# Kotstantinovskiy/SonicDiffusionBayesLab

Hardware: AMD Instinct MI355X
Metric: 512x512 images/sec at 50 DDIM steps (higher is better)
Workload: dtype bf16; 1 GPU; SD-1.5 512x512 DDIM 50 steps, CFG 7.5, batch=8/GPU (BASELINE configs[1]); global_batch=8, sample_size=64, parallelism=batch-shard x1, weights=SD-1.5-shaped synthetic seed 1234

## Files before the change

include/sd_hip.h:

```cpp
#ifndef SD_HIP_H
#define SD_HIP_H

#ifdef __cplusplus
extern "C" {
#endif

typedef struct sd_unet sd_unet;

typedef struct sd_unet_config {
    int sample_size;
    int in_channels;
    int out_channels;
    int num_levels;
    int block_out_channels[8];
    int layers_per_block;
    int attn_levels[8];
    int cross_attention_dim;
    int num_heads;
    int norm_num_groups;
    float norm_eps;
    int context_len;
    int weight_dtype;
    float fp8_act_scale_norm;
    float fp8_act_scale_ff;
// ... 277 lines not shown
int sd_op_softmax_rows(void* stream, void* S, long long rows, int cols, float scale);
int sd_op_conv3x3_upsample_subpixel(void* stream, const void* X, const void* W4, const float* bias, void* Y, int B, int Hin,
                                    int Win, int Cin, int Cout);
int sd_op_conv3x3_upsample_subpixel_groupnorm(void* stream, const void* X, const void* W4, const float* bias, void* Y, int B,
                                              int Hin, int Win, int Cin, int Cout, const float* gamma, const float* beta,
                                              void* Yn, int groups, float eps, int silu);
int sd_op_groupnorm(void* stream, const void* x1, int C1, const void* x2, int C2, const float* gamma,
                    const float* beta, void* y, int B, int HW, int groups, float eps, int silu);
int sd_op_conv3x3_groupnorm(void* stream, const void* X, const void* W, const float* bias, const float* bias2,
                            const void* R, void* Y, int B, int Hin, int Win, int Cin, int Cout, const float* gamma,
                            const float* beta, void* Yn, int groups, float eps, int silu);
int sd_op_conv3x3_splitk(int M, int Cout, int Cin, int Hin, int Win, int stride, int upsample);
int sd_op_layernorm(void* stream, const void* x, const float* gamma, const float* beta, void* y, int rows, int C,
                    float eps);
int sd_op_tome_match(void* stream, const void* x, const unsigned char* choice, int B, int h, int w, int C, float* node_max,
                     int* node_idx, int* tok);
int sd_op_tome_select(void* stream, const float* node_max, const int* node_idx, int B, int num_src, int r, int* kept, int* merged,
                      int* dst_idx);
int sd_op_tome_merge(void* stream, const void* x, const int* tok, const int* kept, const int* merged, const int* dst_idx, void* out,
                     long long ldo, int B, int h, int w, int C, int r);
int sd_op_tome_unmerge(void* stream, const void* y, long long ldy, const void* residual, const int* tok, const int* kept,
                       const int* merged, const int* dst_idx, void* out, int B, int h, int w, int C, int r);
int sd_op_tgate_capture(void* stream, const void* y, const void* res, void* h2, void* cache, float* rowstats, long long rows, int C,
                        int pair);
int sd_op_tgate_apply(void* stream, const void* h1, const void* cache, void* h2, float* rowstats, long long rows, int C);
int sd_op_freeu(void* stream, const void* hidden, const void* skip, void* hidden_out, void* skip_out, int B, int H, int W,
                int C_hidden, int C_skip, float b, float s);
int sd_hypertile_check(int B, int rh, int rw, int C, int nh, int nw, long long pitch);
int sd_op_hypertile_gather(void* stream, const void* x, long long pitch, void* out, int B, int rh, int rw, int C, int nh, int nw);
int sd_op_hypertile_scatter(void* stream, const void* y, void* out, long long pitch, int B, int rh, int rw, int C, int nh, int nw);
int sd_pag_identity_check(long long rows_total, long long row0, long long rows, int C, int heads, long long ldv, int tok);
int sd_op_pag_identity(void* stream, const void* V, long long ldv, int tok, void* out, long long rows_total, long long row0,
                       long long rows, int C, int heads);
int sd_sag_mass_check(int B, int heads, int N, int D, long long ld, int head_major);
int sd_op_sag_attn_mass(void* stream, const void* Q, const void* K, long long ld, float* mass, int B, int heads, int N, int D,
                        int exp2_units);
int sd_op_sag_degrade(void* stream, const float* x, const float* m, const float* mass, int mh, int mw, int pred_type,
                      const float coef[6], float* out, int LB, int H, int W);
int sd_op_attention(void* stream, const void* Q, long long ldq, const void* K, long long ldk, const void* V,
                    long long ldv, void* O, long long ldo, int B, int heads, int Nq, int Nk, int D, float scale);
int sd_op_gemm_qkv_headmajor(void* stream, const void* X, long long ldx, const void* W, void* Q, void* KV, int M, int C,
                             int tokens, int K);
int sd_op_attention_headmajor(void* stream, const void* Q, long long ldq, const void* K, const void* V, void* O,
                              long long ldo, int B, int heads, int Nq, int Nk, int D, float scale);
int sd_op_clip_attention(void* stream, const void* qkv, void* out, int B, int L, int H, int heads);
int sd_op_vit_attention(void* stream, const void* qkv, void* out, int B, int L, int H, int heads);
int sd_op_clip_embed(void* stream, const int* ids, const void* tok, const void* pos, void* out, int rows, int L, int H,
                     int vocab);
int sd_op_activation(void* stream, void* x, long long n, int kind);
int sd_op_pool_rows(void* stream, const void* src, const int* ids, int B, int L, int H, int eos_id, void* dst);
int sd_op_vit_embed(void* stream, const void* patch_rows, const float* cls, const void* pos, void* out, int B, int Np, int H);
int sd_op_bert_attention(void* stream, const void* q, long long ldq, const void* k, const void* v, long long ldkv,
                         const int* mask, void* out, long long ldo, int B, int heads, int Lq, int Lk);
int sd_op_reward_head(void* stream, const void* hidden, long long row_stride, const float* w, const float* bias, float mean,
                      float std, int B, int H, float* rewards, float* features);
int sd_op_clip_preprocess(void* stream, const unsigned char* images, int B, int H, int W, int S, int P, unsigned char* crop,
                          void* patches);
int sd_op_conv_in(void* stream, const float* x, int Bsrc, const float* Wt, const float* bias, void* y, int B, int H,
                  int W, int Cin, int Cout);
int sd_op_conv_in_cond(void* stream, const float* x, int Bsrc, const float* cond, int Bcond, const float* Wt,
                       const float* bias, void* y, int B, int H, int W, int Cout);
int sd_op_conv_in_add(void* stream, const float* x, int Bsrc, const void* addend, int Badd, const float* Wt, const float* bias,
                      void* y, int B, int H, int W, int Cout);
int sd_op_residual_add(void* stream, void* x, const long long* dst_off, const void* r, const long long* src_off,
                       const long long* count, int nseg, float scale);
int sd_op_conv_out(void* stream, const void* x, const void* Wp, const float* bias, float* y, int B, int H, int W,
                   int Cin, int Cout);
int sd_op_time_embedding(void* stream, float t, const void* W1, const float* b1, const void* W2, const float* b2,
                         float* scratch, float* temb, int dim_in, int dim);
int sd_op_timestep_cond(void* stream, float t, const float* cond, const void* Wc, float* row, float* emb, int cond_dim,
                        int dim);

int sd_op_ln_partials(int kind, int M, int N);
int sd_op_gemm_rowstats(void* stream, const void* X, long long ldx, const void* W, const float* bias, const void* R,
                        long long ldr, void* C, long long ldc, int M, int N, int K, float* rowstats);
int sd_op_gemm_ln(void* stream, const void* X, long long ldx, const void* Wg, const float* c1, const float* c2,
                  const float* rowstats, int parts, float eps, void* C, long long ldc, int M, int N, int K, int epi);
int sd_op_gemm_plan(void* stream, const void* X, long long ldx, const void* X2, long long ldx2, int K1, const void* W,
                    const float* bias, const float* bias2, const void* R, long long ldr, void* C, long long ldc, int M, int N,
                    int K, float* rowstats, float* stats, const float* ln_rs, int ln_parts, const float* ln_c1, float ln_eps,
                    void* KV, int hm_tokens);
int sd_op_xattn_fused_rowstats(void* stream, const void* X, const void* R, void* Y, const void* At, const void* Bw,
                               const float* bias, int M, int C, int rows_per_sample, int L, float* rowstats);
int sd_op_ip_xattn(void* stream, const void* R, void* Rout, const void* A, const void* Bt, const float* gamma, const float* beta,
                   float eps, long long M, int C, int rows_per_sample, int heads, int T);
int sd_op_xattn_expand(void* stream, const void* kv, void* out, int B, int L, int C, int heads, int slots, int col_off, float scale);
int sd_op_transpose_bf16(void* stream, const void* src, void* dst, int B, int R, int Cc, int perm16);
int sd_op_retile32(void* stream, const void* src, void* dst, int B, int R, int K, int RT);
int sd_op_xattn_fold(void* stream, const void* kv, const void* wqT, const void* wo, const float* lnu, const float* ones, void* at,
                     void* bw, float* c1, float* c2, void* scratch, int UB, int L, int C, int heads, int perm);
int sd_op_ip_fold(void* stream, const void* ip_kv, const void* wqT, const void* wo, void* at, void* bt, void* scratch, int UB, int T,
                  int C, int heads, float scale);
int sd_op_xattn_fused(void* stream, const void* X, const void* R, void* Y, const void* At, const void* Bw,
                      const float* bias, int M, int C, int rows_per_sample, int L);
int sd_op_xattn_fused_ln(void* stream, const void* X, const void* R, void* Y, const void* At, const void* Bw,
                         const float* bias, int M, int C, int rows_per_sample, int L, const float* ln_rowstats, int ln_parts,
                         long long ln_rows, const float* c2, float eps, float* rowstats);
int sd_op_conv3x3_ablate(void* stream, const void* X, const void* W, void* Y, int B, int Hin, int Win, int Cin, int Cout,
                         int ablate);
int sd_op_xattn_fused_stamps(void* stream, const void* X, const void* R, void* Y, const void* At, const void* Bw,
                             const float* bias, int M, int C, int rows_per_sample, int L, unsigned long long* stamps);

int sd_op_gemm_fp8(void* stream, const void* X, long long ldx, const void* W, const float* wscale, float xscale,
                   const float* bias, const void* R, long long ldr, void* C, long long ldc, int M, int N, int K, int epi,
                   int out_fp8, float oscale);
int sd_op_conv3x3_fp8(void* stream, const void* X, const void* W, const float* wscale, float xscale, const float* bias,
                      const float* bias2, const void* R, void* Y, int B, int Hin, int Win, int Cin, int Cout, int stride,
                      int upsample);
int sd_op_groupnorm_fp8(void* stream, const void* x1, int C1, const void* x2, int C2, const float* gamma,
                        const float* beta, void* y, int B, int HW, int groups, float eps, int silu, int Cpad, float oscale);
int sd_op_layernorm_fp8(void* stream, const void* x, const float* gamma, const float* beta, void* y, int rows, int C,
                        int Cpad, float eps, float oscale);
int sd_op_quantize_fp8(void* stream, const void* x_bf16, void* y_fp8, long long rows, int C, int Cpad, float scale);
int sd_op_amax_e4m3(void* stream, const void* codes, long long nbytes, unsigned* out_code);

#ifdef __cplusplus
}
#endif
#endif
```

sonicdiffusionbayeslab_amd/_lib.py:

```python
from __future__ import annotations

import ctypes as C
import os
import re
from typing import Optional

HERE = os.path.dirname(os.path.abspath(__file__))
LIB_PATH = os.environ.get("SD_AMD_LIB", os.path.join(HERE, "lib", "libsdhip.so"))
HEADER_PATH = os.path.normpath(os.path.join(HERE, "..", "include", "sd_hip.h"))

ABLATE_LIB_PATH = os.path.join(HERE, "lib", "libsdhip_ablate.so")

_lib: Optional[C.CDLL] = None
_ablate: Optional[C.CDLL] = None


class SdUnetConfig(C.Structure):
    _fields_ = [
        ("sample_size", C.c_int), ("in_channels", C.c_int), ("out_channels", C.c_int),
        ("num_levels", C.c_int), ("block_out_channels", C.c_int * 8), ("layers_per_block", C.c_int),
        ("attn_levels", C.c_int * 8), ("cross_attention_dim", C.c_int), ("num_heads", C.c_int),
        ("norm_num_groups", C.c_int), ("norm_eps", C.c_float), ("context_len", C.c_int),
        ("weight_dtype", C.c_int), ("fp8_act_scale_norm", C.c_float), ("fp8_act_scale_ff", C.c_float),
        ("time_cond_proj_dim", C.c_int),
# ... 147 lines not shown
    "sd_op_conv_in_add": (_i, [_vp, _vp, _i, _vp, _i, _vp, _vp, _vp, _i, _i, _i, _i]),
    "sd_op_residual_add": (_i, [_vp, _vp, _vp, _vp, _vp, _vp, _i, _f]),
    "sd_op_conv_in_cond": (_i, [_vp, _vp, _i, _vp, _i, _vp, _vp, _vp, _i, _i, _i, _i]),
    "sd_op_gemm": (_i, [_vp, _vp, _ll, _vp, _ll, _i, _vp, _vp, _vp, _vp, _ll, _vp, _ll, _i, _i, _i, _i]),
    "sd_op_gemm_tile_rows": (_i, [_i, _i, _i]),
    "sd_op_gemm_splitk": (_i, [_i, _i, _i, _i]),
    "sd_op_gemm_batched": (_i, [_vp, _vp, _ll, _vp, _ll, _i, _vp, _vp, _ll, _vp, _ll, _i, _i, _i, _i, _i]),
    "sd_op_gemm_batched_softmax_ln": (_i, [_vp, _vp, _ll, _vp, _ll, _i, _vp, _ll, _i, _i, _i, _i, _vp, _i, _vp, _vp, _f]),
    "sd_op_conv3x3": (_i, [_vp, _vp, _vp, _vp, _vp, _vp, _vp, _i, _i, _i, _i, _i, _i, _i]),
    "sd_op_conv3x3_shortcut": (_i, [_vp, _vp, _vp, _vp, _vp, _i, _vp, _i, _vp, _vp, _i, _i, _i, _i, _i]),
    "sd_op_conv3x3_shortcut_groupnorm": (_i, [_vp, _vp, _vp, _vp, _vp, _i, _vp, _i, _vp, _vp, _i, _i, _i, _i, _i,
                                              _vp, _vp, _vp, _i, _f, _i]),
    "sd_op_conv3x3_down_asym": (_i, [_vp, _vp, _vp, _vp, _vp, _i, _i, _i, _i, _i]),
    "sd_op_conv3x3_ablate": (_i, [_vp, _vp, _vp, _vp, _i, _i, _i, _i, _i, _i]),
    "sd_op_conv3x3_upsample_subpixel": (_i, [_vp, _vp, _vp, _vp, _vp, _i, _i, _i, _i, _i]),
    "sd_op_conv3x3_upsample_subpixel_groupnorm": (_i, [_vp, _vp, _vp, _vp, _vp, _i, _i, _i, _i, _i, _vp, _vp, _vp, _i, _f, _i]),
    "sd_op_groupnorm": (_i, [_vp, _vp, _i, _vp, _i, _vp, _vp, _vp, _i, _i, _i, _f, _i]),
    "sd_op_conv3x3_groupnorm": (_i, [_vp, _vp, _vp, _vp, _vp, _vp, _vp, _i, _i, _i, _i, _i, _vp, _vp, _vp, _i, _f, _i]),
    "sd_op_conv3x3_splitk": (_i, [_i, _i, _i, _i, _i, _i, _i]),
    "sd_op_conv3x3_kernel": (_i, [_i, _i, _i, _i, _i, _i, _i, _i]),
    "sd_op_softmax_rows": (_i, [_vp, _vp, _ll, _i, _f]),
    "sd_op_layernorm": (_i, [_vp, _vp, _vp, _vp, _vp, _i, _i, _f]),
    "sd_op_attention": (_i, [_vp, _vp, _ll, _vp, _ll, _vp, _ll, _vp, _ll, _i, _i, _i, _i, _i, _f]),
    "sd_op_gemm_qkv_headmajor": (_i, [_vp, _vp, _ll, _vp, _vp, _vp, _i, _i, _i, _i]),
    "sd_op_attention_headmajor": (_i, [_vp, _vp, _ll, _vp, _vp, _vp, _ll, _i, _i, _i, _i, _i, _f]),
    "sd_op_clip_attention": (_i, [_vp, _vp, _vp, _i, _i, _i, _i]),
    "sd_op_conv_in": (_i, [_vp, _vp, _i, _vp, _vp, _vp, _i, _i, _i, _i, _i]),
    "sd_op_conv_out": (_i, [_vp, _vp, _vp, _vp, _vp, _i, _i, _i, _i, _i]),
    "sd_op_time_embedding": (_i, [_vp, _f, _vp, _vp, _vp, _vp, _vp, _vp, _i, _i]),
    "sd_op_timestep_cond": (_i, [_vp, _f, _vp, _vp, _vp, _vp, _i, _i]),
    "sd_op_ln_partials": (_i, [_i, _i, _i]),
    "sd_op_gemm_rowstats": (_i, [_vp, _vp, _ll, _vp, _vp, _vp, _ll, _vp, _ll, _i, _i, _i, _vp]),
    "sd_op_gemm_plan": (_i, [_vp, _vp, _ll, _vp, _ll, _i, _vp, _vp, _vp, _vp, _ll, _vp, _ll, _i, _i, _i, _vp, _vp, _vp, _i, _vp, _f,
                            _vp, _i]),
    "sd_op_gemm_ln": (_i, [_vp, _vp, _ll, _vp, _vp, _vp, _vp, _i, _f, _vp, _ll, _i, _i, _i, _i]),
    "sd_op_xattn_fused_rowstats": (_i, [_vp, _vp, _vp, _vp, _vp, _vp, _vp, _i, _i, _i, _i, _vp]),
    "sd_op_xattn_fused": (_i, [_vp, _vp, _vp, _vp, _vp, _vp, _vp, _i, _i, _i, _i]),
    "sd_op_xattn_fused_ln": (_i, [_vp, _vp, _vp, _vp, _vp, _vp, _vp, _i, _i, _i, _i, _vp, _i, _ll, _vp, _f, _vp]),
    "sd_op_xattn_fused_stamps": (_i, [_vp, _vp, _vp, _vp, _vp, _vp, _vp, _i, _i, _i, _i, _vp]),
    "sd_op_gemm_fp8": (_i, [_vp, _vp, _ll, _vp, _vp, _f, _vp, _vp, _ll, _vp, _ll, _i, _i, _i, _i, _i, _f]),
    "sd_op_conv3x3_fp8": (_i, [_vp, _vp, _vp, _vp, _f, _vp, _vp, _vp, _vp, _i, _i, _i, _i, _i, _i, _i]),
    "sd_op_groupnorm_fp8": (_i, [_vp, _vp, _i, _vp, _i, _vp, _vp, _vp, _i, _i, _i, _f, _i, _i, _f]),
    "sd_op_layernorm_fp8": (_i, [_vp, _vp, _vp, _vp, _vp, _i, _i, _i, _f, _f]),
    "sd_op_quantize_fp8": (_i, [_vp, _vp, _vp, _ll, _i, _i, _f]),
    "sd_op_amax_e4m3": (_i, [_vp, _vp, _ll, _vp]),
    "sd_unet_set_tome": (_i, [_vp, C.c_double, _i]),
    "sd_unet_tome_block_count_hw": (_i, [_vp, _i, _i]),
    "sd_unet_tome_block_info_hw": (_i, [_vp, _i, _i, _i, C.POINTER(_i), C.POINTER(_i), C.POINTER(_i), C.POINTER(_ll)]),
    "sd_unet_set_tome_choice_hw": (_i, [_vp, _vp, _vp, _ll, _i, _i]),
    "sd_unet_tome_matching_hw": (_i, [_vp, _vp, _i, _i, _i, _vp, _vp, _vp, _vp, _vp, C.POINTER(_i), C.POINTER(_i)]),
    "sd_op_tome_match": (_i, [_vp, _vp, _vp, _i, _i, _i, _i, _vp, _vp, _vp]),
    "sd_op_tome_select": (_i, [_vp, _vp, _vp, _i, _i, _i, _vp, _vp, _vp]),
    "sd_op_tome_merge": (_i, [_vp, _vp, _vp, _vp, _vp, _vp, _vp, _ll, _i, _i, _i, _i, _i]),
    "sd_op_tome_unmerge": (_i, [_vp, _vp, _ll, _vp, _vp, _vp, _vp, _vp, _vp, _i, _i, _i, _i, _i]),
    "sd_unet_set_freeu": (_i, [_vp, _f, _f, _f, _f]),
    "sd_unet_disable_freeu": (_i, [_vp]),
    "sd_unet_plan_count": (_i, [_vp]),
    "sd_op_freeu": (_i, [_vp, _vp, _vp, _vp, _vp, _i, _i, _i, _i, _i, _f, _f]),
    "sd_unet_tgate_bytes_hw": (_ll, [_vp, _i, _i, _i]),
    "sd_unet_tgate_block_info_hw": (_i, [_vp, _i, _i, _i, _i, C.POINTER(_ll), C.POINTER(_ll), C.POINTER(_i)]),
    "sd_unet_set_tgate_hw": (_i, [_vp, _i, _vp, _ll, _i, _i, _i]),
    "sd_op_tgate_capture": (_i, [_vp, _vp, _vp, _vp, _vp, _vp, _ll, _i, _i]),
    "sd_op_tgate_apply": (_i, [_vp, _vp, _vp, _vp, _vp, _ll, _i]),
    "sd_unet_set_hypertile": (_i, [_vp, _i, _i]),
    "sd_unet_hypertile_block_count_hw": (_i, [_vp, _i, _i]),
    "sd_unet_hypertile_block_info_hw": (_i, [_vp, _i, _i, _i, C.POINTER(_i), C.POINTER(_i), C.POINTER(_i), C.POINTER(_i)]),
    "sd_hypertile_check": (_i, [_i, _i, _i, _i, _i, _i, _ll]),
    "sd_op_hypertile_gather": (_i, [_vp, _vp, _ll, _vp, _i, _i, _i, _i, _i, _i]),
    "sd_op_hypertile_scatter": (_i, [_vp, _vp, _vp, _ll, _i, _i, _i, _i, _i, _i]),
    "sd_unet_set_pag": (_i, [_vp, _ll]),
    "sd_unet_pag_block_count": (_i, [_vp]),
    "sd_pag_identity_check": (_i, [_ll, _ll, _ll, _i, _i, _ll, _i]),
    "sd_op_pag_identity": (_i, [_vp, _vp, _ll, _i, _vp, _ll, _ll, _ll, _i, _i]),
    "sd_sched_step_pag": (_i, [_vp, _vp, _i, _f, _f] + [_vp] * 8 + [C.POINTER(_f), _ll, _vp, _ll, _vp, _vp, _vp, _f, _f, _ll]),
    "sd_sched_step_pc_pag": (_i, [_vp, _vp, _i, _f, _f] + [_vp] * 9 + [C.POINTER(_f), _ll, _vp, _ll, _vp, _vp, _vp, _f, _f, _ll]),
    "sd_cfg_rescale_factors_pag": (_i, [_vp, _vp, _i, _ll, _f, _f, _f, _vp]),
    "sd_unet_set_sag": (_i, [_vp, _i]),
    "sd_unet_set_sag_buffer": (_i, [_vp, _vp, _ll]),
    "sd_sag_mass_check": (_i, [_i, _i, _i, _i, _ll, _i]),
    "sd_op_sag_attn_mass": (_i, [_vp, _vp, _vp, _ll, _vp, _i, _i, _i, _i, _i]),
    "sd_op_sag_degrade": (_i, [_vp, _vp, _vp, _vp, _i, _i, _i, C.POINTER(_f), _vp, _i, _i, _i]),
    "sd_sched_step_sag": (_i, [_vp, _vp, _i, _f, _f] + [_vp] * 8 + [C.POINTER(_f), _ll, _vp, _ll, _vp, _vp, _vp, _f, _f, _ll]),
    "sd_sched_step_pc_sag": (_i, [_vp, _vp, _i, _f, _f] + [_vp] * 9 + [C.POINTER(_f), _ll, _vp, _ll, _vp, _vp, _vp, _f, _f, _ll]),
}


def _open(path: str, missing_message: str) -> C.CDLL:
    if not os.path.exists(path):
        raise SdHipError(missing_message)
    lib = C.CDLL(path)
    for name, (res, args) in _SIGS.items():
        fn = getattr(lib, name)
        fn.restype = res
        fn.argtypes = args
    return lib


def load() -> C.CDLL:
    global _lib
    if _lib is None:
        _lib = _open(LIB_PATH, f"{LIB_PATH} is missing: build it with `python -m sonicdiffusionbayeslab_amd.build` "
                               "(or __graft_entry__.build()).  There is no CPU/PyTorch fallback for the hot path.")
    return _lib


def load_ablate() -> C.CDLL:
    global _ablate
    if _ablate is None:
        _ablate = _open(ABLATE_LIB_PATH, f"{ABLATE_LIB_PATH} is missing: build it with `python -m sonicdiffusionbayeslab_amd.build`")
    return _ablate


def check(rc: int, what: str = "libsdhip call", lib: Optional[C.CDLL] = None) -> None:
    if rc != 0:
        msg = (lib or load()).sd_last_error()
        raise SdHipError(f"{what} failed (rc={rc}): {msg.decode() if msg else '?'}")


def ptr(t) -> Optional[int]:
    return None if t is None else t.data_ptr()


def current_stream() -> int:
    import torch
    return torch.cuda.current_stream().cuda_stream
```

sonicdiffusionbayeslab_amd/build.py:

```python
from __future__ import annotations

import os
import shutil
import subprocess
import sys
import tempfile
from concurrent.futures import ThreadPoolExecutor

HERE = os.path.dirname(os.path.abspath(__file__))
CSRC = os.path.join(HERE, "csrc")
LIB_DIR = os.path.join(HERE, "lib")
LIB_PATH = os.path.join(LIB_DIR, "libsdhip.so")
ABLATE_LIB_PATH = os.path.join(LIB_DIR, "libsdhip_ablate.so")
ABLATE_SOURCES = ("gemm_conv.hip", "conv_halo.hip")
SOURCES = ["gemm_conv.hip", "gemm_lean.hip", "conv_halo.hip", "conv64.hip", "norm.hip", "attention.hip", "xattn.hip", "ip_xattn.hip", "small.hip", "sched.hip", "clip.hip", "vit.hip", "bert.hip", "inception.hip", "unet.hip", "pack.hip", "plan.hip", "taesd.hip", "tome.hip", "freeu.hip", "tgate.hip", "hypertile.hip", "pag.hip", "sag.hip", "ops.hip"]
HEADERS = ["common.h", "kernels.h", "model.h",os.path.join("..", "..", "include", "sd_hip.h")]
FLAGS = ["--offload-arch=gfx950", "-O3", "-fPIC", "-std=c++17", "-Wall", "-Wno-unused-function"]
NO_PACKED_FP32 = ["-Xclang", "-target-feature", "-Xclang", "-packed-fp32-ops"]
EXTRA_FLAGS = {"attention.hip": ["-mllvm", "-amdgpu-mfma-vgpr-form", "-ffinite-math-only", *NO_PACKED_FP32],
               "xattn.hip": ["-mllvm", "-amdgpu-mfma-vgpr-form", "-fno-slp-vectorize"],
               "ip_xattn.hip": NO_PACKED_FP32,
               "small.hip": NO_PACKED_FP32, "sched.hip": NO_PACKED_FP32, "clip.hip": NO_PACKED_FP32, "vit.hip": NO_PACKED_FP32, "bert.hip": NO_PACKED_FP32, "norm.hip": NO_PACKED_FP32,
               "inception.hip": NO_PACKED_FP32,
               "conv64.hip": NO_PACKED_FP32,
               "tome.hip": NO_PACKED_FP32,
               "freeu.hip": NO_PACKED_FP32,
               "tgate.hip": NO_PACKED_FP32,
               "hypertile.hip": NO_PACKED_FP32,
               "pag.hip": NO_PACKED_FP32,
               "sag.hip": NO_PACKED_FP32,
               "gemm_conv.hip": ["-fno-slp-vectorize"], "gemm_lean.hip": ["-fno-slp-vectorize"]}
_HOST_NOISE = "is not a recognized feature for this target (ignoring feature)"


def _newer(a: str, b: str) -> bool:
    return (not os.path.exists(b)) or os.path.getmtime(a) > os.path.getmtime(b)


def asm_path(src: str, ablate: bool = False) -> str:
    return os.path.join(LIB_DIR, src.replace(".hip", ".ablate.s" if ablate else ".s"))


def lint_asm(path: str, unit: str, verbose: bool = True) -> None:
    from . import asm_lint
    bad = asm_lint.lint_file(path, unit, verbose=verbose)
    if bad:
        raise RuntimeError(f"{unit}: the assembly hipcc produced violates {len(bad)} rule(s) of asm_lint.py (first: {bad[0]}); "
                           "see the VIOLATION lines above and sonicdiffusionbayeslab_amd/asm_lint.py for what each rule guards")


def compile_unit(hipcc: str, src: str, obj: str, flags, verbose: bool = True) -> None:
    s = os.path.join(CSRC, src)
    tmp = tempfile.mkdtemp(prefix="sdhip_", dir=LIB_DIR)
    try:
        cmd = [hipcc, *flags, "-save-temps", "-c", s, "-o", os.path.join(tmp, "unit.o")]
        if verbose:
            print(" ".join(cmd), flush=True)
        r = subprocess.run(cmd, capture_output=True, text=True, cwd=tmp)
        err = "\n".join(l for l in r.stderr.splitlines() if _HOST_NOISE not in l and "argument unused during compilation" not in l)
        if r.returncode != 0:
            raise RuntimeError(f"hipcc failed:\n{' '.join(cmd)}\n{r.stdout}\n{err}")
        if verbose and err.strip():
            print(err, file=sys.stderr)
        dev = [f for f in os.listdir(tmp) if f.endswith("-gfx950.s")]
        if len(dev) != 1:
            raise RuntimeError(f"{src}: expected one device assembly file from -save-temps, found {dev}")
        asm = obj[:-2] + ".s"
        shutil.move(os.path.join(tmp, dev[0]), asm)
        try:
            lint_asm(asm, src.split(".")[0], verbose=verbose)
        except Exception:
            os.replace(asm, asm + ".rejected")
            raise
        shutil.move(os.path.join(tmp, "unit.o"), obj)
    finally:
        shutil.rmtree(tmp, ignore_errors=True)


def build_library(force: bool = False, verbose: bool = True) -> str:
    hipcc = os.environ.get("HIPCC", "/opt/rocm/bin/hipcc")
    if not os.path.exists(hipcc):
        hipcc = "hipcc"
    os.makedirs(LIB_DIR, exist_ok=True)
    hdrs = [os.path.normpath(os.path.join(CSRC, h)) for h in HEADERS]
    me = [os.path.abspath(__file__), os.path.join(HERE, "asm_lint.py")]
    objs, jobs = [], []
    for src in SOURCES:
        s = os.path.join(CSRC, src)
        o = os.path.join(LIB_DIR, src.replace(".hip", ".o"))
        objs.append(o)
        if force or _newer(s, o) or any(_newer(h, o) for h in hdrs + me) or not os.path.exists(o[:-2] + ".s"):
            jobs.append((src, o, [*FLAGS, *EXTRA_FLAGS.get(src, [])]))

    aobjs, ajobs = [], []
    for src in SOURCES:
        s = os.path.join(CSRC, src)
        if src in ABLATE_SOURCES:
            o = os.path.join(LIB_DIR, src.replace(".hip", ".ablate.o"))
            if force or _newer(s, o) or any(_newer(h, o) for h in hdrs + me) or not os.path.exists(o[:-2] + ".s"):
                ajobs.append((src, o, [*FLAGS, "-DSD_ABLATE", *EXTRA_FLAGS.get(src, [])]))
        else:
            o = os.path.join(LIB_DIR, src.replace(".hip", ".o"))
        aobjs.append(o)

    def run(cmd):
        if verbose:
            print(" ".join(cmd), flush=True)
        r = subprocess.run(cmd, capture_output=True, text=True)
        if r.returncode != 0:
            raise RuntimeError(f"hipcc failed:\n{' '.join(cmd)}\n{r.stdout}\n{r.stderr}")

    with ThreadPoolExecutor(max_workers=4) as ex:
        list(ex.map(lambda j: compile_unit(hipcc, j[0], j[1], j[2], verbose), jobs + ajobs))
    if force or jobs or not os.path.exists(LIB_PATH):
# ... 9 lines not shown
```

sonicdiffusionbayeslab_amd/csrc/common.h:

```cpp
#pragma once
#include <hip/hip_runtime.h>
#include <stdint.h>

typedef unsigned short bf16_t;

typedef __attribute__((ext_vector_type(8))) short bf16x8;
typedef __attribute__((ext_vector_type(4))) short bf16x4;
typedef __attribute__((ext_vector_type(4))) float f32x4;
typedef __attribute__((ext_vector_type(16))) float f32x16;
typedef __attribute__((ext_vector_type(2))) __bf16 bf16x2_t;
typedef __attribute__((ext_vector_type(2))) float f32x2_t;
typedef __attribute__((ext_vector_type(4))) unsigned u32x4;
typedef __attribute__((ext_vector_type(2))) unsigned u32x2;

typedef __attribute__((ext_vector_type(8))) int i32x8;
typedef __attribute__((ext_vector_type(8))) unsigned u32x8;
__device__ __forceinline__ i32x8 cat_u32x4(u32x4 lo, u32x4 hi) {
    const u32x8 r = __builtin_shufflevector(lo, hi, 0, 1, 2, 3, 4, 5, 6, 7);
    return __builtin_bit_cast(i32x8, r);
}

#define LDS_PTR(p) ((__attribute__((address_space(3))) void*)(p))
#define GLB_PTR(p) ((const __attribute__((address_space(1))) void*)(p))

// ... 55 lines not shown

template <int SHR>
__device__ __forceinline__ float row_shr_add(float v) {
    const int sh = __builtin_amdgcn_update_dpp(0, __builtin_bit_cast(int, v), 0x110 + SHR, 0xf, 0xf, true);
    return v + __builtin_bit_cast(float, sh);
}
template <int TN, int TM>
__device__ __forceinline__ void tile_channel_stats(const f32x4 (&acc)[TN][TM], float* __restrict__ stats, long block64, int C,
                                                   int n_base, int N, int m_base, int M, int lane, int b0 = 0, int nb = TM) {
    const int lrow = lane & 15, lq = lane >> 4;
#pragma unroll
    for (int a = 0; a < TN; ++a) {
        float sv[4] = {0.f, 0.f, 0.f, 0.f}, qv[4] = {0.f, 0.f, 0.f, 0.f};
#pragma unroll
        for (int b = 0; b < TM; ++b) {
            if (b < b0 || b >= b0 + nb) continue;
            const bool live = m_base + b * 16 + lrow < M;
            const unsigned p0 = pack2bf(acc[a][b][0], acc[a][b][1]), p1 = pack2bf(acc[a][b][2], acc[a][b][3]);
            const float v[4] = {bflo(p0), bfhi(p0), bflo(p1), bfhi(p1)};
#pragma unroll
            for (int j = 0; j < 4; ++j) {
                const float x = live ? v[j] : 0.f;
                sv[j] += x;
                qv[j] = __builtin_fmaf(x, x, qv[j]);
            }
        }
#pragma unroll
        for (int j = 0; j < 4; ++j) {
            sv[j] = row_shr_add<8>(row_shr_add<4>(row_shr_add<2>(row_shr_add<1>(sv[j]))));
            qv[j] = row_shr_add<8>(row_shr_add<4>(row_shr_add<2>(row_shr_add<1>(qv[j]))));
        }
        const int n = n_base + a * 16 + lq * 4;
        if (lrow == 15 && n < N) {
            float* o = stats + (block64 * C + n) * 2;
            *(f32x4*)o = f32x4{sv[0], qv[0], sv[1], qv[1]};
            *(f32x4*)(o + 4) = f32x4{sv[2], qv[2], sv[3], qv[3]};
        }
    }
}

template <int TN, int TM>
__device__ __forceinline__ void tile_row_stats(const f32x4 (&acc)[TN][TM], float* __restrict__ part, int n_base, int N,
                                               int m_base, int M, int lane) {
    const int lrow = lane & 15, lq = lane >> 4;
#pragma unroll
    for (int b = 0; b < TM; ++b) {
        float s = 0.f, q = 0.f;
#pragma unroll
        for (int a = 0; a < TN; ++a) {
            const bool live = n_base + a * 16 + lq * 4 < N;
            const unsigned p0 = pack2bf(acc[a][b][0], acc[a][b][1]), p1 = pack2bf(acc[a][b][2], acc[a][b][3]);
            const float v[4] = {bflo(p0), bfhi(p0), bflo(p1), bfhi(p1)};
#pragma unroll
            for (int j = 0; j < 4; ++j) {
                const float x = live ? v[j] : 0.f;
                s += x;
                q = __builtin_fmaf(x, x, q);
            }
        }
        s += __shfl_xor(s, 16); q += __shfl_xor(q, 16);
        s += __shfl_xor(s, 32); q += __shfl_xor(q, 32);
        const int m = m_base + b * 16 + lrow;
        if (lq == 0 && m < M) *(f32x2_t*)(part + (long)m * 2) = f32x2_t{s, q};
    }
}

__device__ __forceinline__ f32x2_t ln_mean_rstd(float s, float q, float inv_k, float eps) {
    const float mean = s * inv_k;
    const float var = __builtin_fmaf(q, inv_k, -(mean * mean));
    return f32x2_t{mean, __builtin_amdgcn_rsqf(fmaxf(var, 0.f) + eps)};
}
__device__ __forceinline__ f32x4 ln_fold(f32x4 acc, f32x4 c1, float mean, float rstd, f32x4 c2) {
#ifdef SD_DIAG_LN_PACKED
    const f32x4 nm = {-mean, -mean, -mean, -mean}, rs = {rstd, rstd, rstd, rstd};
    return __builtin_elementwise_fma(__builtin_elementwise_fma(c1, nm, acc), rs, c2);
#else
    f32x4 r;
#pragma unroll
    for (int j = 0; j < 4; ++j) r[j] = __builtin_fmaf(__builtin_fmaf(c1[j], -mean, acc[j]), rstd, c2[j]);
    return r;
#endif
}

__device__ __forceinline__ float wave_sum(float v) {
#pragma unroll
    for (int o = 32; o > 0; o >>= 1) v += __shfl_xor(v, o);
    return v;
}

extern "C" const char* sd_last_error(void);
void sd_set_error(const char* fmt, ...);
#define SD_CHECK_HIP(expr)                                                              \
    do {                                                                                \
        hipError_t _e = (expr);                                                         \
        if (_e != hipSuccess) {                                                         \
            sd_set_error("%s failed: %s (%s:%d)", #expr, hipGetErrorString(_e), __FILE__, __LINE__); \
            return -2;                                                                  \
        }                                                                               \
    } while (0)
#define SD_REQUIRE(cond, ...)          \
    do {                               \
        if (!(cond)) {                 \
            sd_set_error(__VA_ARGS__); \
            return -1;                 \
        }                              \
    } while (0)
```

sonicdiffusionbayeslab_amd/csrc/kernels.h:

```cpp
#pragma once
#include <vector>

#include "common.h"

struct GemmArgs {
    const bf16_t* X = nullptr;
    long ldx = 0;
    const bf16_t* X2 = nullptr;
    long ldx2 = 0;
    int K1 = 0;
    const bf16_t* W = nullptr;
    long ldw = 0;
    const float* bias = nullptr;
    const float* bias2 = nullptr;
    const bf16_t* R = nullptr;
    long ldr = 0;
    bf16_t* C = nullptr;
    long ldc = 0;
    int M = 0, N = 0, K = 0;
    int Hin = 0, Win = 0, Cin = 0, Hout = 0, Wout = 0, stride = 1, up = 0;
    int asym = 0;
    int splitk = 1;
    float* slab = nullptr;
    int defer_reduce = 0;
    const void* zero_page = nullptr;
    long w_batch_stride = 0;
    int rows_per_batch = 0;
    int sm_valid = 0;
    int tiles_m = 0, tiles_n = 0;
    int tune = 0;
    float* stats = nullptr;
    float* rowstats = nullptr;
    bf16_t* KV = nullptr;
    int hm_C = 0, hm_tok = 0;
    int subpix = 0;
    const float* ln_rs = nullptr;
    const float* ln_c1 = nullptr;
    int ln_np = 0;
    float ln_eps = 1e-5f;
    int ln_per_sample = 0;
    int dt = 0;
    const float* wscale = nullptr;
    float xscale_inv = 1.0f;
    int out_fp8 = 0;
    float oscale = 1.0f;
    const bf16_t* Xs1 = nullptr;
    const bf16_t* Xs2 = nullptr;
    const bf16_t* Wsc = nullptr;
    long ldwsc = 0;
    int Csc1 = 0, Csc2 = 0;
};

int sd_gemm_tile_rows(int M, int N, int K = 0);
int sd_gemm_splitk(int M, int N, int K, int rows = 0);
int sd_launch_gemm(const GemmArgs& a, int epi , hipStream_t stream);
int sd_launch_conv3x3(const GemmArgs& a, hipStream_t stream);
bool sd_gemm_lean_applicable(const GemmArgs& a, int epi);
int sd_launch_gemm_lean(const GemmArgs& a, int epi, int rows, hipStream_t stream);
void sd_launch_splitk_reduce(const GemmArgs& a, hipStream_t stream);
bool sd_conv_halo_applicable(const GemmArgs& a);
int sd_conv_halo_mode(const GemmArgs& a);
int sd_conv3x3_splitk(int M, int N, int Cin, int Hin, int Win, int stride, int up, int dt = 0);
bool sd_conv_halo_subpix_applicable(const GemmArgs& a);
int sd_launch_conv3x3_halo(const GemmArgs& a, hipStream_t stream);
bool sd_conv_halo_shortcut_applicable(const GemmArgs& a);

constexpr int SD_CONV64_PACKED_BYTES = 9 * 2 * 4 * 1024;
struct Conv64Args {
    const bf16_t* X = nullptr;
    const bf16_t* Wp = nullptr;
    const float* bias = nullptr;
    const bf16_t* R = nullptr;
    bf16_t* Y = nullptr;
    int B = 0, Hin = 0, Win = 0;
    int mode = 0;
    int relu = 0;
    int Hout = 0, Wout = 0, tiles_y = 0, tiles_x = 0, ntiles = 0;
    unsigned xbytes = 0;
};
int sd_conv64_out_size(int in, int mode);
void sd_conv64_pack(const float* w_oihw , bf16_t* out);
int sd_launch_conv64(const Conv64Args& a, hipStream_t stream);
int sd_launch_taesd_entry(const float* x, const float* Wt, const float* bias, bf16_t* y, int B, int H, int W, int Cin, int decoder,
                          hipStream_t stream);
int sd_launch_taesd_exit(const bf16_t* x, const bf16_t* Wp, const float* bias, float* y, int B, int H, int W, int Cout, int out_mode,
                         hipStream_t stream);

struct GroupNormArgs {
    const bf16_t* x1 = nullptr; int C1 = 0;
    const bf16_t* x2 = nullptr; int C2 = 0;
    const float* gamma = nullptr; const float* beta = nullptr;
    bf16_t* y = nullptr;
    int out_fp8 = 0, Cpad = 0;
    float oscale = 1.0f;
    const float* stats1 = nullptr; const float* stats2 = nullptr;
    const float* slab = nullptr; int splitk = 0;
    const float* sbias = nullptr; const float* sbias2 = nullptr;
    const bf16_t* sR = nullptr; long sldr = 0;
    bf16_t* x1w = nullptr;
    float* partial = nullptr;
    int B = 0, HW = 0, groups = 32, nsplit = 0;
    float eps = 1e-5f;
    int silu = 0;
};
int sd_groupnorm_nsplit(int B, int HW);
bool sd_groupnorm_uses_small(int B, int HW, int C1, int C2, int groups);
bool sd_groupnorm_slab_ok(int B, int HW, int C1, int C2, int groups);
size_t sd_groupnorm_scratch_bytes(int B, int HW, int groups);
int sd_launch_groupnorm(const GroupNormArgs& a, hipStream_t stream);

int sd_launch_softmax_rows(bf16_t* s, long rows, int cols, float scale, hipStream_t stream);
int sd_launch_softmax_rows_long(bf16_t* s, long rows, int cols, float scale, hipStream_t stream);
int sd_launch_pqconv(const float* x, const float* W, const float* bias, float* y, int B, int HW, float in_scale,
                     hipStream_t stream);

int sd_launch_layernorm(const bf16_t* x, const float* gamma, const float* beta, bf16_t* y, int rows, int C,
                        float eps, hipStream_t stream);
int sd_launch_layernorm_fp8(const bf16_t* x, const float* gamma, const float* beta, void* y, int rows, int C, int Cpad,
                            float eps, float oscale, hipStream_t stream);
int sd_launch_amax_e4m3(const void* y, long nbytes, unsigned* out, hipStream_t stream);
int sd_launch_quantize_fp8(const bf16_t* x, void* y, long rows, int C, int Cpad, float scale, hipStream_t stream);

struct AttnArgs {
    const bf16_t* Q = nullptr; long ldq = 0;
    const bf16_t* K = nullptr; long ldk = 0;
    const bf16_t* V = nullptr; long ldv = 0;
    bf16_t* O = nullptr; long ldo = 0;
    int B = 0, heads = 0, Nq = 0, Nk = 0, D = 0;
    float scale = 0.f;
    const void* consts = nullptr;
    int kv_head_major = 0;
    int q_prescaled = 0;
    int xcd_order = 1;
};
int sd_launch_attention(const AttnArgs& a, hipStream_t stream);

int sd_launch_gemv(const float* x, const bf16_t* W, const float* b, float* y, int N, int K, int silu_in,
                   hipStream_t stream);
int sd_launch_timestep_sinusoid(float t, float* out, int dim, hipStream_t stream);
int sd_launch_timestep_sinusoid_row(float t, const float* row, float* out, int dim, hipStream_t stream);
int sd_launch_f32_to_bf16(const float* src, bf16_t* dst, long n, hipStream_t stream);
int sd_launch_transpose_bf16(const bf16_t* src, bf16_t* dst, int B, int R, int Cc, hipStream_t stream, int perm16 = 0);

int sd_launch_retile32(const bf16_t* src, bf16_t* dst, int B, int R, int K, int RT, hipStream_t stream);
int sd_launch_replicate(const void* src, void* dst, long bytes, int rep, hipStream_t stream);

int sd_tome_check(int h, int w, int C, const char* who);
int sd_launch_tome_partition(const unsigned char* choice, int h, int w, int* tok, hipStream_t stream);
int sd_launch_tome_match(const bf16_t* x, const unsigned char* choice, int B, int h, int w, int C, float* node_max, int* node_idx,
                         int* tok, float* inv, hipStream_t stream);
int sd_launch_tome_select(const float* node_max, const int* node_idx, int B, int num_src, int r, int* kept, int* merged, int* dst_idx,
                          hipStream_t stream);
int sd_launch_tome_merge(const bf16_t* x, const int* tok, const int* kept, const int* merged, const int* dst_idx, bf16_t* out,
                         long ldo, int B, int h, int w, int C, int r, hipStream_t stream);
int sd_launch_tome_unmerge(const bf16_t* y, long ldy, const bf16_t* residual, const int* tok, const int* kept, const int* merged,
                           const int* dst_idx, bf16_t* out, int B, int h, int w, int C, int r, hipStream_t stream);

int sd_freeu_check(int B, int H, int W, int C_hidden, int C_skip, const char* who);
int sd_launch_freeu(const bf16_t* hidden, const bf16_t* skip, bf16_t* hidden_out, bf16_t* skip_out, int B, int H, int W, int C_hidden,
                    int C_skip, float b, float s, hipStream_t stream);

constexpr int SD_TGATE_PARTS = 2;
int sd_tgate_check(long rows, int C, const char* who);
int sd_launch_tgate_capture(const bf16_t* y, const bf16_t* res, bf16_t* h2, bf16_t* cache, float* rowstats, long rows, int C, int pair,
                            hipStream_t stream);
int sd_launch_tgate_apply(const bf16_t* h1, const bf16_t* cache, bf16_t* h2, float* rowstats, long rows, int C, hipStream_t stream);

int sd_hypertile_shape_ok(int B, int rh, int rw, int C, int nh, int nw, long pitch, const char* who);
int sd_launch_hypertile_gather(const bf16_t* x, long pitch, bf16_t* out, int B, int rh, int rw, int C, int nh, int nw, hipStream_t stream);
int sd_launch_hypertile_scatter(const bf16_t* y, bf16_t* out, long pitch, int B, int rh, int rw, int C, int nh, int nw, hipStream_t stream);

int sd_pag_identity_shape_ok(long rows_total, long row0, long rows, int C, int heads, long ldv, int tok, const char* who);
int sd_launch_pag_identity(const bf16_t* V, long ldv, int tok, bf16_t* out, long rows_total, long row0, long rows, int C, int heads,
                           hipStream_t stream);

int sd_sag_mass_shape_ok(int B, int heads, int N, int D, long ld, int head_major, const char* who);
int sd_launch_sag_attn_mass(const bf16_t* Q, const bf16_t* K, long ld, float* mass, int B, int heads, int N, int D, int exp2_units,
                            hipStream_t stream);
int sd_sag_degrade_shape_ok(int LB, int H, int W, int mh, int mw, int pred, const char* who);
int sd_launch_sag_degrade(const float* x, const float* m, const float* mass, int mh, int mw, int pred, const float coef[6], float* out,
                          int LB, int H, int W, hipStream_t stream);

struct XattnArgs {
    const bf16_t* X = nullptr;
    const bf16_t* R = nullptr;
    bf16_t* Y = nullptr;
    const bf16_t* At = nullptr;
    const bf16_t* Bw = nullptr;
    const float* bias = nullptr;
    int M = 0, C = 0, rows_per_sample = 0, L = 0;
    float* rowstats = nullptr;
    const float* ln_rs = nullptr; int ln_np = 0; long ln_rows = 0;
// ... 97 lines not shown
```

sonicdiffusionbayeslab_amd/csrc/model.h:

```cpp
#pragma once
#include "../../include/sd_hip.h"
#include "common.h"
#include "kernels.h"

#include <stdlib.h>
#include <string.h>
#include <sys/mman.h>

#include <algorithm>
#include <map>
#include <new>
#include <set>
#include <string>
#include <tuple>
#include <unordered_map>
#include <vector>

namespace sdhip {

constexpr size_t NOFF = (size_t)-1;
constexpr int T_LATENTS = -2, T_EPS = -3;
constexpr int MAX_CONTROL_RES = SD_MAX_RES_SEGMENTS;

struct ParamSpec {
    std::string name;
    std::vector<long long> shape;
    std::vector<float> data;
    bool loaded = false;
    long long numel() const {
        long long n = 1;
        for (auto s : shape) n *= s;
        return n;
    }
};

struct Wrap {
    int type;
    int block_i, layer_i;
};

enum OpKind { OP_SINUSOID, OP_GEMV, OP_CONV_IN, OP_GN, OP_CONV3, OP_GEMM, OP_LN, OP_ATTN, OP_CONV_OUT, OP_SOFTMAX, OP_PQCONV,
              OP_CLIP_EMBED, OP_CLIP_ATTN, OP_QGELU, OP_TO_F32, OP_XATTN, OP_REPLICATE,
              OP_VIT_PREP, OP_VIT_EMBED, OP_VIT_ATTN, OP_POOL, OP_CONV_IN_IMG, OP_ENC_OUT, OP_IP_XATTN, OP_RES_ADD,
              OP_BERT_ATTN, OP_REWARD_HEAD,
              OP_TOME_MATCH, OP_TOME_SELECT, OP_TOME_MERGE, OP_TOME_UNMERGE,
              OP_FREEU,
              OP_TGATE_CAPTURE, OP_TGATE_APPLY, OP_TGATE_ZERO,
              OP_HT_GATHER, OP_HT_SCATTER,
              OP_PAG_IDENTITY,
              OP_SAG_MASS };

constexpr int TGATE_OFF = 0, TGATE_CAPTURE = 1, TGATE_REUSE = 2;

constexpr int REP_TEXT_POOLED = 2;

struct Op {
    int kind = 0;
    int x1 = -1, x2 = -1, r = -1, out = -1, aux = -1, b2t = -1;
    size_t w = NOFF, b = NOFF, g = NOFF, be = NOFF;
    long b2idx = 0;
    int M = 0, N = 0, K = 0, K1 = 0, epi = 0;
    int B = 0, Hin = 0, Win = 0, Cin = 0, Hout = 0, Wout = 0, stride = 1, up = 0;
    int C1 = 0, C2 = 0, HW = 0, silu = 0, nsplit = 0;
    float eps = 0.f;
    int heads = 0, D = 0, Nq = 0, Nk = 0;
    long ldq = 0, ldk = 0, ldv = 0, ldo = 0, qoff = 0, koff = 0, voff = 0;
    int silu_in = 0, splitk = 1;
    int pool_by_ids = 0;
    int key_mask = 0;
    int defer = 0, slab_t = -1, slab_k = 0, slab_r = -1, slab_b2t = -1;
    size_t slab_b = NOFF;
    long slab_b2idx = 0;
    int wt = -1;
    size_t wx = NOFF;
    long xoff = 0, woff_el = 0, coff = 0, ldx_o = 0, ldw_o = 0, ldc_o = 0;
    float scale = 0.f;
    long wbs = 0;
    int rpb = 0, sm_valid = 0;
    int dt = 0, out_fp8 = 0, Cpad = 0, Kalg = 0;
    int sname = -1;
    int stats = -1, s1 = -1, s2 = -1;
    int subpix = 0;
    int asym = 0;
    int hm = 0;
    int qps = 0;
    int rs = -1, lnrs = -1, lnnp = 0;
    size_t c1 = NOFF;
    size_t wsc = NOFF;
    float xs = 1.f, os = 1.f;
    int scx1 = -1, scx2 = -1, scc1 = 0, scc2 = 0;
    size_t scw = NOFF;
    int nres = 0;
    int res_t[MAX_CONTROL_RES];
    int nwrap = 0;
    Wrap wraps[3];
};

struct HostBlob {
    unsigned char* p = nullptr;
    size_t n = 0, cap = 0;
    unsigned char* data() { return p; }
    const unsigned char* data() const { return p; }
    size_t size() const { return n; }
    bool empty() const { return n == 0; }
    bool reserve(size_t bytes) {
        if (bytes <= cap) return true;
        void* q = mmap(nullptr, bytes, PROT_READ | PROT_WRITE, MAP_PRIVATE | MAP_ANONYMOUS | MAP_POPULATE, -1, 0);
        if (q == MAP_FAILED) return false;
        (void)madvise(q, bytes, MADV_HUGEPAGE);
        if (p) { memcpy(q, p, n); munmap(p, cap); }
        p = (unsigned char*)q; cap = bytes;
        return true;
    }
    void resize(size_t bytes) {
        if (bytes > cap && !reserve(std::max(bytes, cap * 2))) throw std::bad_alloc();
        n = bytes;
    }
    void release() { if (p) munmap(p, cap); p = nullptr; n = cap = 0; }
    ~HostBlob() { release(); }
    HostBlob() = default;
    HostBlob(const HostBlob&) = delete;
    HostBlob& operator=(const HostBlob&) = delete;
};

struct Tn {
    size_t bytes = 0;
    int def = -1, last = -1;
    bool persistent = false;
    bool ctx = false;
    bool ctx_ip = false;
    size_t off = NOFF;
};

struct Plan {
    int UB = 0, branch = -1;
    int rep = 1;
    int lh = 0, lw = 0;
    int ip = 0;
    struct IpFold { int at, bt, C; size_t wqT, wo, wkv; int heads; };
    std::vector<IpFold> ip_fold;
    int ip_e = -1, ip_proj = -1, ip_tok = -1, ip_kv = -1;
    int cn = 0;
    std::vector<size_t> cn_off;
    std::vector<long> cn_count;
    struct TomeBlock { int tok, kept, merged, dst_idx, B, h, w, r; long choice_off; };
    std::vector<TomeBlock> tome;
    long tome_choice_bytes = 0;
    struct HtBlock { int rh, rw, nh, nw; };
    std::vector<HtBlock> hypertile;
    int pag_lb = 0, pag_blocks = 0;
    int sag = 0;
    int freeu = 0;
    int tgate = 0, tg_pair = 1, tg_batch = 0;
    std::vector<size_t> tg_off;
    std::vector<long> tg_rows;
    std::vector<int> tg_ch;
    int tg_blocks = 0;
    std::vector<Tn> tensors;
    std::vector<Op> ops;
    std::vector<char> skipped;
    std::vector<int> ctx_kv;
    std::vector<size_t> ctx_w;
    std::vector<int> ctx_c;
    int ctx_bf16 = -1;
    struct Fold { int kv, at, bw, C, heads; size_t wqT, wo; bool perm; int c2 = -1; size_t lnu = NOFF; int c1 = -1; size_t ones = NOFF; };
    std::vector<Fold> ctx_fold;
    int ctx_fold_scratch = -1;
    std::map<std::string, int> taps;
    size_t total_bytes = 0;
    ClipPrepGeom geom;
    std::vector<int> prep_tab;
    const int* dtab = nullptr;
};

}

// ... 124 lines not shown
```

sonicdiffusionbayeslab_amd/csrc/norm.hip:

```cpp
#include "common.h"
#include "kernels.h"

#include <stdlib.h>

#include <algorithm>
#include <type_traits>

namespace {

struct GnGeom {
    int nchunks, rows_par, threads, cpg, C;
};

__host__ __device__ inline GnGeom gn_geom(int C, int groups) {
    GnGeom g;
    g.C = C;
    g.nchunks = C / 8;
    g.rows_par = g.nchunks >= 256 ? 1 : 256 / g.nchunks;
    const int act = g.rows_par * g.nchunks;
    g.threads = (act + 63) / 64 * 64;
    g.cpg = C / groups;
    return g;
}

// ... 58 lines not shown
            else                        { s += v.z; q += v.w; }
        }
        float* out = a.partial + (((long)b * a.nsplit + split) * a.groups + tid) * 2;
        out[0] = s;
        out[1] = q;
    }
}

__global__ __launch_bounds__(256) void gn_finalize_kernel(const GroupNormArgs a) {
    const int lane = threadIdx.x & 63;
    const int idx = blockIdx.x * 4 + (threadIdx.x >> 6);
    if (idx >= a.B * a.groups) return;
    const int b = idx / a.groups, gi = idx - b * a.groups;
    float s = 0.f, q = 0.f;
    for (int i = lane; i < a.nsplit; i += 64) {
        const float* pp = a.partial + (((long)b * a.nsplit + i) * a.groups + gi) * 2;
        s += pp[0];
        q += pp[1];
    }
    s = wave_sum(s);
    q = wave_sum(q);
    if (lane == 0) {
        const float cnt = (float)a.HW * (float)((a.C1 + a.C2) / a.groups);
        const float mean = s / cnt;
        const float var = fmaxf(q / cnt - mean * mean, 0.f);
        float* st = a.partial + (long)a.B * a.nsplit * a.groups * 2 + (long)idx * 2;
        st[0] = mean;
        st[1] = rsqrtf(var + a.eps);
    }
}

__global__ __launch_bounds__(256) void gn_finalize_stats_kernel(const GroupNormArgs a) {
    __shared__ float red[8];
    const int tid = threadIdx.x, lane = tid & 63, wave = tid >> 6;
    const int idx = blockIdx.x;
    const int b = idx / a.groups, gi = idx - b * a.groups;
    const int C = a.C1 + a.C2, cpg = C / a.groups, nblk = a.HW >> 6;
    const int total = nblk * cpg;
    float s = 0.f, q = 0.f;
    for (int i = tid; i < total; i += 256) {
        const int blk = i / cpg, c = gi * cpg + (i - blk * cpg);
        const long gb = (long)b * nblk + blk;
        const f32x2_t v = *(const f32x2_t*)(c < a.C1 ? a.stats1 + (gb * a.C1 + c) * 2 : a.stats2 + (gb * a.C2 + (c - a.C1)) * 2);
        s += v[0];
        q += v[1];
    }
    s = wave_sum(s);
    q = wave_sum(q);
    if (lane == 0) { red[wave * 2] = s; red[wave * 2 + 1] = q; }
    __syncthreads();
    if (tid == 0) {
        s = (red[0] + red[2]) + (red[4] + red[6]);
        q = (red[1] + red[3]) + (red[5] + red[7]);
        const float cnt = (float)a.HW * (float)cpg;
        const float mean = s / cnt;
        const float var = fmaxf(q / cnt - mean * mean, 0.f);
        float* st = a.partial + (long)a.B * a.nsplit * a.groups * 2 + (long)idx * 2;
        st[0] = mean;
        st[1] = rsqrtf(var + a.eps);
    }
}

template <bool SILU, bool FP8>
__global__ void gn_apply_kernel(const GroupNormArgs a) {
    const GnGeom g = gn_geom(a.C1 + a.C2, a.groups);
    const int tid = threadIdx.x;
    const int split = blockIdx.x, b = blockIdx.y;
    const bool active = tid < g.rows_par * g.nchunks;
    if (!active) return;
    const int prow = tid / g.nchunks, ch = tid - prow * g.nchunks;
    const int c0 = ch * 8;
    const float* st = a.partial + (long)a.B * a.nsplit * a.groups * 2 + (long)b * a.groups * 2;
    const int g0 = c0 / g.cpg, g1 = (c0 + 7) / g.cpg;
    const int nb = min(8, (g0 + 1) * g.cpg - c0);
    const float m0 = st[g0 * 2], r0 = st[g0 * 2 + 1], m1 = st[g1 * 2], r1 = st[g1 * 2 + 1];
    float sc[8], sf[8];
    {
        const f32x4 ga = *(const f32x4*)(a.gamma + c0), gb = *(const f32x4*)(a.gamma + c0 + 4);
        const f32x4 ba = *(const f32x4*)(a.beta + c0), bb = *(const f32x4*)(a.beta + c0 + 4);
#pragma unroll
        for (int j = 0; j < 8; ++j) {
            const float gm = j < 4 ? ga[j & 3] : gb[j & 3], bt = j < 4 ? ba[j & 3] : bb[j & 3];
            const float mean = j < nb ? m0 : m1, rstd = j < nb ? r0 : r1;
            sc[j] = rstd * gm;
            sf[j] = bt - mean * sc[j];
        }
    }
    const int per = (a.HW + a.nsplit - 1) / a.nsplit;
    const int pbeg = split * per, pend = min(a.HW, pbeg + per);
    auto apply = [&](const u32x4 v, long pix) {
        float f[8] = {bflo(v[0]), bfhi(v[0]), bflo(v[1]), bfhi(v[1]),
                      bflo(v[2]), bfhi(v[2]), bflo(v[3]), bfhi(v[3])};
#pragma unroll
        for (int j = 0; j < 8; ++j) {
            f[j] = f[j] * sc[j] + sf[j];
            if (SILU) f[j] = silu_f(f[j]);
        }
        if (FP8) {
            char* yr = (char*)a.y + pix * a.Cpad;
            const u32x2 o = {pack4fp8(f[0] * a.oscale, f[1] * a.oscale, f[2] * a.oscale, f[3] * a.oscale),
                             pack4fp8(f[4] * a.oscale, f[5] * a.oscale, f[6] * a.oscale, f[7] * a.oscale)};
            *(u32x2*)(yr + c0) = o;
            if (ch == g.nchunks - 1)
                for (int k = g.C; k < a.Cpad; k += 16) *(u32x4*)(yr + k) = u32x4{0u, 0u, 0u, 0u};
            return;
        }
        u32x4 o = {pack2bf(f[0], f[1]), pack2bf(f[2], f[3]), pack2bf(f[4], f[5]), pack2bf(f[6], f[7])};
        *(u32x4*)(a.y + pix * g.C + c0) = o;
    };
    const long base = (long)b * a.HW;
    const int rp = g.rows_par;
    int p = pbeg + prow;
    for (; p + 3 * rp < pend; p += 4 * rp) {
        const u32x4 v0 = *(const u32x4*)gn_src(a, base + p, c0);
        const u32x4 v1 = *(const u32x4*)gn_src(a, base + p + rp, c0);
        const u32x4 v2 = *(const u32x4*)gn_src(a, base + p + 2 * rp, c0);
        const u32x4 v3 = *(const u32x4*)gn_src(a, base + p + 3 * rp, c0);
        apply(v0, base + p); apply(v1, base + p + rp); apply(v2, base + p + 2 * rp); apply(v3, base + p + 3 * rp);
    }
    for (; p < pend; p += rp) apply(*(const u32x4*)gn_src(a, base + p, c0), base + p);
}

__device__ __forceinline__ float2 gn_unit_sums(const u32x2 v) {
    const float f0 = bflo(v[0]), f1 = bfhi(v[0]), f2 = bflo(v[1]), f3 = bfhi(v[1]);
    return make_float2((f0 + f1) + (f2 + f3), (f0 * f0 + f1 * f1) + (f2 * f2 + f3 * f3));
}
__device__ __forceinline__ void gn_mean_rstd(float ts, float tq, float cnt, float eps, float& mean, float& rstd) {
    mean = ts / cnt;
    rstd = rsqrtf(fmaxf(tq / cnt - mean * mean, 0.f) + eps);
}
template <bool SILU, bool FP8>
__device__ __forceinline__ void gn_unit_store(const GroupNormArgs& a, const u32x2 v, float mean, float rstd, long pix, int c, int C) {
    const f32x4 gm = *(const f32x4*)(a.gamma + c), bt = *(const f32x4*)(a.beta + c);
    float f[4] = {bflo(v[0]), bfhi(v[0]), bflo(v[1]), bfhi(v[1])};
#pragma unroll
    for (int jj = 0; jj < 4; ++jj) {
        f[jj] = (f[jj] - mean) * rstd * gm[jj] + bt[jj];
        if (SILU) f[jj] = silu_f(f[jj]);
    }
    if (FP8) {
        *(unsigned*)((char*)a.y + pix * a.Cpad + c) = pack4fp8(f[0] * a.oscale, f[1] * a.oscale, f[2] * a.oscale, f[3] * a.oscale);
    } else {
        u32x2 o = {pack2bf(f[0], f[1]), pack2bf(f[2], f[3])};
        *(u32x2*)(a.y + pix * C + c) = o;
    }
}

template <bool SILU, bool FP8, int MAXU>
__global__ __launch_bounds__(256) void gn_small_kernel(const GroupNormArgs a) {
    __shared__ float2 red[4];
    const int C = a.C1 + a.C2, cpg = C / a.groups, upp = cpg >> 2;
    const int grp = blockIdx.x, b = blockIdx.y;
    const int tid = threadIdx.x, lane = tid & 63, wave = tid >> 6;
    const int total = a.HW * upp;
    const long base = (long)b * a.HW;
    auto src = [&](int p, int c) -> const bf16_t* {
        return c < a.C1 ? a.x1 + (base + p) * a.C1 + c : a.x2 + (base + p) * a.C2 + (c - a.C1);
    };
    const int p0 = tid / upp, k0 = tid - p0 * upp, dp = 256 / upp, dk = 256 - dp * upp;
    u32x2 vals[MAXU];
    int pj[MAXU], kj[MAXU];
    {
        int p = p0, k = k0;
#pragma unroll
        for (int j = 0; j < MAXU; ++j) {
            const bool live = tid + 256 * j < total;
            pj[j] = live ? p : 0; kj[j] = live ? k : 0;
            vals[j] = *(const u32x2*)src(pj[j], grp * cpg + kj[j] * 4);
            p += dp; k += dk;
            if (k >= upp) { k -= upp; ++p; }
        }
    }
    float s = 0.f, q = 0.f;
#pragma unroll
    for (int j = 0; j < MAXU; ++j) {
        const bool live = tid + 256 * j < total;
        const float2 u = gn_unit_sums(vals[j]);
        s += live ? u.x : 0.f;
// ... 353 lines not shown

int sd_launch_softmax_rows_long(bf16_t* s, long rows, int cols, float scale, hipStream_t stream) {
    SD_REQUIRE(s && rows > 0 && rows <= 0x7fffffffL, "softmax_rows_long: %ld rows", rows);
    SD_REQUIRE(cols % 8 == 0 && cols > 0, "softmax_rows_long: cols=%d must be a positive multiple of 8", cols);
    hipLaunchKernelGGL(softmax_rows_long_kernel, dim3((unsigned)rows), dim3(256), 0, stream, s, cols, scale);
    SD_CHECK_HIP(hipGetLastError());
    return 0;
}

int sd_launch_softmax_rows(bf16_t* s, long rows, int cols, float scale, hipStream_t stream) {
    SD_REQUIRE(s && rows > 0, "softmax_rows: empty");
    SD_REQUIRE(cols % 8 == 0 && cols > 0 && cols <= 4096, "softmax_rows: cols=%d must be a multiple of 8 and <= 4096", cols);
    hipLaunchKernelGGL(softmax_rows_kernel, dim3((unsigned)((rows + 3) / 4)), dim3(256), 0, stream, s, rows, cols, scale);
    SD_CHECK_HIP(hipGetLastError());
    return 0;
}

size_t sd_groupnorm_scratch_bytes(int B, int HW, int groups) {
    return ((size_t)B * sd_groupnorm_nsplit(B, HW) * groups * 2 + (size_t)B * groups * 2) * sizeof(float);
}

int sd_groupnorm_nsplit(int B, int HW) {
    int n = (2048 + B - 1) / B;
    if (n > HW / 8) n = HW / 8;
    if (n < 1) n = 1;
    if (n > 256) n = 256;
    return n;
}

bool sd_groupnorm_uses_small(int B, int HW, int C1, int C2, int groups) {
    static const bool no_small = getenv("SD_GN_NO_SMALL") != nullptr;
    const int C = C1 + C2;
    return !no_small && HW <= 256 && (long)HW * (C / groups) <= 10240 && (C / groups) % 4 == 0 && C1 % 4 == 0 && B <= 65535;
}

bool sd_groupnorm_slab_ok(int B, int HW, int C1, int C2, int groups) {
    if (!sd_groupnorm_uses_small(B, HW, C1, C2, groups)) return false;
    const int cpg = (C1 + C2) / groups, G = cpg >= 80 ? 1 : 80 / cpg;
    return cpg >= 20 && cpg <= 80 && groups % G == 0 && C2 % 4 == 0 && (long)B * HW * C1 < (1L << 29);
}

int sd_launch_groupnorm(const GroupNormArgs& a, hipStream_t stream) {
    const int C = a.C1 + a.C2;
    SD_REQUIRE(a.x1 && a.y && a.gamma && a.beta && a.partial, "groupnorm: null operand");
    SD_REQUIRE(!a.out_fp8 || (a.Cpad >= C && a.Cpad % 128 == 0 && C % 16 == 0 && a.oscale > 0.f),
               "groupnorm fp8 out: Cpad=%d must be a multiple of 128 >= C=%d (C a multiple of 16)", a.Cpad, C);
    SD_REQUIRE(a.C1 % 8 == 0 && a.C2 % 8 == 0 && (a.C2 == 0 || a.x2), "groupnorm: C1=%d C2=%d must be multiples of 8", a.C1, a.C2);
    SD_REQUIRE(a.groups > 0 && a.groups <= 64 && C % a.groups == 0 && (C / a.groups >= 8 || C / a.groups == 4),
               "groupnorm: C=%d groups=%d needs C/groups >= 8 (or == 4)", C, a.groups);
    SD_REQUIRE(a.nsplit >= 1 && a.nsplit <= a.HW && a.B > 0 && a.HW > 0, "groupnorm: bad split %d for HW=%d", a.nsplit, a.HW);
    const GnGeom g = gn_geom(C, a.groups);
    SD_REQUIRE(g.threads <= 1024, "groupnorm: C=%d too wide", C);
    if (a.slab) {
        const int cpg = C / a.groups, G = cpg >= 80 ? 1 : 80 / cpg, ncol = G * (cpg / 4);
        SD_REQUIRE(a.splitk > 1 && a.splitk <= 64 && a.x1w && !a.out_fp8 && (!a.sR || a.sldr >= a.C1) && (a.C2 == 0 || a.x2),
                   "groupnorm with a deferred split-K reduce: splitk=%d, bf16 output, x1w and a residual stride >= C1", a.splitk);
        SD_REQUIRE(sd_groupnorm_slab_ok(a.B, a.HW, a.C1, a.C2, a.groups), "groupnorm with a deferred split-K reduce: HW=%d C=%d+%d "
                   "is not a shape gn_slab_kernel takes", a.HW, a.C1, a.C2);
        const dim3 grid(a.groups / G, a.B), blk((32 * ncol + 63) / 64 * 64);
        const size_t smem = ((size_t)G * a.HW * (cpg / 4) + 4 * G) * sizeof(float2);
        auto go = [&](auto kern) { hipLaunchKernelGGL(kern, grid, blk, smem, stream, a); };
        auto pick = [&](auto mi, auto un) {
            constexpr int MI = decltype(mi)::value, UN = decltype(un)::value;
            if (a.silu) go(gn_slab_kernel<true, MI, UN>); else go(gn_slab_kernel<false, MI, UN>);
        };
        using std::integral_constant;
        const int iters = (a.HW + 31) / 32, k = a.splitk;
        if (iters <= 2) {
            if (k % 8 == 0) pick(integral_constant<int, 2>{}, integral_constant<int, 8>{});
            else if (k % 4 == 0) pick(integral_constant<int, 2>{}, integral_constant<int, 4>{});
            else if (k % 2 == 0) pick(integral_constant<int, 2>{}, integral_constant<int, 2>{});
            else pick(integral_constant<int, 2>{}, integral_constant<int, 1>{});
        } else if (iters <= 4) {
            if (k % 4 == 0) pick(integral_constant<int, 4>{}, integral_constant<int, 4>{});
            else if (k % 2 == 0) pick(integral_constant<int, 4>{}, integral_constant<int, 2>{});
            else pick(integral_constant<int, 4>{}, integral_constant<int, 1>{});
        } else {
            if (k % 2 == 0) pick(integral_constant<int, 8>{}, integral_constant<int, 2>{});
            else pick(integral_constant<int, 8>{}, integral_constant<int, 1>{});
        }
        SD_CHECK_HIP(hipGetLastError());
        return 0;
    }
    if (sd_groupnorm_uses_small(a.B, a.HW, a.C1, a.C2, a.groups)) {
        const int units = (a.HW * (C / a.groups / 4) + 255) / 256;
        const dim3 grid(a.groups, a.B);
        auto go = [&](auto kern) { hipLaunchKernelGGL(kern, grid, dim3(256), 0, stream, a); };
        auto pick = [&](auto mu) {
            constexpr int MU = decltype(mu)::value;
            if (a.out_fp8) { if (a.silu) go(gn_small_kernel<true, true, MU>); else go(gn_small_kernel<false, true, MU>); }
            else { if (a.silu) go(gn_small_kernel<true, false, MU>); else go(gn_small_kernel<false, false, MU>); }
        };
        if (units <= 3) pick(std::integral_constant<int, 3>{});
        else if (units <= 5) pick(std::integral_constant<int, 5>{});
        else pick(std::integral_constant<int, 10>{});
        SD_CHECK_HIP(hipGetLastError());
        return 0;
    }
    dim3 grid(a.nsplit, a.B);
    if (a.stats1 != nullptr) {
        SD_REQUIRE(a.HW % 64 == 0 && (a.C2 == 0 || a.stats2 != nullptr), "groupnorm: producer statistics need HW %% 64 == 0 and both sources");
        hipLaunchKernelGGL(gn_finalize_stats_kernel, dim3(a.B * a.groups), dim3(256), 0, stream, a);
    } else {
        hipLaunchKernelGGL(gn_stats_kernel, grid, dim3(g.threads), (g.threads + g.nchunks) * sizeof(float4), stream, a);
        hipLaunchKernelGGL(gn_finalize_kernel, dim3((a.B * a.groups + 3) / 4), dim3(256), 0, stream, a);
    }
    if (a.out_fp8) {
        if (a.silu) hipLaunchKernelGGL((gn_apply_kernel<true, true>), grid, dim3(g.threads), 0, stream, a);
        else hipLaunchKernelGGL((gn_apply_kernel<false, true>), grid, dim3(g.threads), 0, stream, a);
    } else {
        if (a.silu) hipLaunchKernelGGL((gn_apply_kernel<true, false>), grid, dim3(g.threads), 0, stream, a);
        else hipLaunchKernelGGL((gn_apply_kernel<false, false>), grid, dim3(g.threads), 0, stream, a);
    }
    SD_CHECK_HIP(hipGetLastError());
    return 0;
}

static int launch_layernorm(const bf16_t* x, const float* gamma, const float* beta, bf16_t* y, int rows, int C, float eps,
                            bool fp8, int Cpad, float oscale, hipStream_t stream) {
    SD_REQUIRE(x && y && gamma && beta, "layernorm: null operand");
    SD_REQUIRE(C % 8 == 0 && C > 0 && C <= 1536, "layernorm: C=%d must be a multiple of 8 and <= 1536", C);
    SD_REQUIRE(rows > 0, "layernorm: no rows");
    SD_REQUIRE(!fp8 || (Cpad == (C + 127) / 128 * 128 && C % 16 == 0 && oscale > 0.f && Cpad - C <= 64 * 16),
               "layernorm fp8 out: Cpad=%d must be C=%d rounded up to 128 (C a multiple of 16)", Cpad, C);
    auto grouped = [&](auto kern, int lpr) {
        const int rows_per_block = 4 * (64 / lpr);
        hipLaunchKernelGGL(kern, dim3((rows + rows_per_block - 1) / rows_per_block), dim3(256), 0, stream, x, gamma, beta, y,
                           rows, eps, oscale);
    };
    if (fp8) {
        if (C == 320) grouped(layernorm_grouped_kernel<8, true>, 8);
        else if (C == 640) grouped(layernorm_grouped_kernel<16, true>, 16);
        else if (C == 1280) grouped(layernorm_grouped_kernel<32, true>, 32);
        else
            hipLaunchKernelGGL(layernorm_kernel<true>, dim3((rows + 3) / 4), dim3(256), 0, stream, x, gamma, beta, y, rows, C,
                               eps, Cpad, oscale);
    } else {
        if (C == 320) grouped(layernorm_grouped_kernel<8, false>, 8);
        else if (C == 640) grouped(layernorm_grouped_kernel<16, false>, 16);
        else if (C == 1280) grouped(layernorm_grouped_kernel<32, false>, 32);
        else
            hipLaunchKernelGGL(layernorm_kernel<false>, dim3((rows + 3) / 4), dim3(256), 0, stream, x, gamma, beta, y, rows, C,
                               eps, C, 1.0f);
    }
    SD_CHECK_HIP(hipGetLastError());
    return 0;
}

int sd_launch_layernorm(const bf16_t* x, const float* gamma, const float* beta, bf16_t* y, int rows, int C,
                        float eps, hipStream_t stream) {
    return launch_layernorm(x, gamma, beta, y, rows, C, eps, false, C, 1.0f, stream);
}

int sd_launch_layernorm_fp8(const bf16_t* x, const float* gamma, const float* beta, void* y, int rows, int C, int Cpad,
                            float eps, float oscale, hipStream_t stream) {
    return launch_layernorm(x, gamma, beta, (bf16_t*)y, rows, C, eps, true, Cpad, oscale, stream);
}

int sd_launch_quantize_fp8(const bf16_t* x, void* y, long rows, int C, int Cpad, float scale, hipStream_t stream) {
    SD_REQUIRE(x && y && rows > 0, "quantize_fp8: null operand");
    SD_REQUIRE(C % 8 == 0 && Cpad % 8 == 0 && Cpad >= C && scale > 0.f, "quantize_fp8: C=%d Cpad=%d", C, Cpad);
    const long n = rows * (Cpad >> 3);
    hipLaunchKernelGGL(quantize_fp8_kernel, dim3((unsigned)((n + 255) / 256)), dim3(256), 0, stream, x, (char*)y, rows, C,
                       Cpad, scale);
    SD_CHECK_HIP(hipGetLastError());
    return 0;
}

int sd_launch_amax_e4m3(const void* y, long nbytes, unsigned* out, hipStream_t stream) {
    SD_REQUIRE(y && out && nbytes > 0 && nbytes % 16 == 0 && ((uintptr_t)y & 15) == 0, "amax_e4m3: %ld bytes, 16-byte granules", nbytes);
    const long n16 = nbytes / 16;
    const unsigned grid = (unsigned)std::min<long>((n16 + 255) / 256, 2048);
    hipLaunchKernelGGL(amax_e4m3_kernel, dim3(grid), dim3(256), 0, stream, (const u32x4*)y, n16, out);
    SD_CHECK_HIP(hipGetLastError());
    return 0;
}
```

sonicdiffusionbayeslab_amd/csrc/ops.hip:

```cpp
#include "model.h"

#include <stdlib.h>

namespace sdhip {

static void* g_scratch = nullptr;
static size_t g_scratch_bytes = 0;
void* op_scratch(size_t bytes) {
    if (bytes > g_scratch_bytes) {
        (void)hipDeviceSynchronize();
        if (g_scratch) (void)hipFree(g_scratch);
        g_scratch = nullptr;
        g_scratch_bytes = 0;
        if (hipMalloc(&g_scratch, bytes) != hipSuccess) return nullptr;
        g_scratch_bytes = bytes;
    }
    return g_scratch;
}

}

using namespace sdhip;

static void conv3x3_args(GemmArgs& a, const void* X, const void* W, const float* bias, const float* bias2, const void* R, void* Y,
// ... 538 lines not shown
    if (splitk_slab(a, "sd_op_gemm_fp8")) return -1;
    return sd_launch_gemm(a, epi, (hipStream_t)stream);
}

extern "C" int sd_op_conv3x3_fp8(void* stream, const void* X, const void* W, const float* wscale, float xscale,
                                 const float* bias, const float* bias2, const void* R, void* Y, int B, int Hin, int Win,
                                 int Cin, int Cout, int stride, int upsample) {
    if (ensure_zero_page()) return -2;
    SD_REQUIRE(stride == 1 || stride == 2, "conv3x3 fp8: stride %d", stride);
    SD_REQUIRE(xscale > 0.f, "conv3x3 fp8: activation scale");
    GemmArgs a;
    conv3x3_args(a, X, W, bias, bias2, R, Y, B, Hin, Win, Cin, Cout, stride, upsample ? 1 : 0);
    a.dt = 1; a.wscale = wscale; a.xscale_inv = 1.0f / xscale;
    a.splitk = sd_conv3x3_splitk(a.M, a.N, Cin, Hin, Win, stride, a.up, 1);
    if (splitk_slab(a, "sd_op_conv3x3_fp8")) return -1;
    return sd_launch_conv3x3(a, (hipStream_t)stream);
}

extern "C" int sd_op_groupnorm_fp8(void* stream, const void* x1, int C1, const void* x2, int C2, const float* gamma,
                                   const float* beta, void* y, int B, int HW, int groups, float eps, int silu, int Cpad,
                                   float oscale) {
    GroupNormArgs a;
    a.x1 = (const bf16_t*)x1; a.C1 = C1; a.x2 = (const bf16_t*)x2; a.C2 = C2; a.gamma = gamma; a.beta = beta;
    a.y = (bf16_t*)y; a.B = B; a.HW = HW; a.groups = groups; a.eps = eps; a.silu = silu;
    a.out_fp8 = 1; a.Cpad = Cpad; a.oscale = oscale;
    a.nsplit = sd_groupnorm_nsplit(B, HW);
    a.partial = (float*)op_scratch(sd_groupnorm_scratch_bytes(B, HW, groups));
    SD_REQUIRE(a.partial, "sd_op_groupnorm_fp8: cannot allocate scratch");
    return sd_launch_groupnorm(a, (hipStream_t)stream);
}

extern "C" int sd_op_layernorm_fp8(void* stream, const void* x, const float* gamma, const float* beta, void* y, int rows,
                                   int C, int Cpad, float eps, float oscale) {
    return sd_launch_layernorm_fp8((const bf16_t*)x, gamma, beta, y, rows, C, Cpad, eps, oscale, (hipStream_t)stream);
}

extern "C" int sd_op_quantize_fp8(void* stream, const void* x_bf16, void* y_fp8, long long rows, int C, int Cpad, float scale) {
    return sd_launch_quantize_fp8((const bf16_t*)x_bf16, y_fp8, (long)rows, C, Cpad, scale, (hipStream_t)stream);
}

extern "C" int sd_op_amax_e4m3(void* stream, const void* codes, long long nbytes, unsigned* out_code) {
    SD_REQUIRE(out_code, "sd_op_amax_e4m3: null output");
    SD_CHECK_HIP(hipMemsetAsync(out_code, 0, sizeof(unsigned), (hipStream_t)stream));
    return sd_launch_amax_e4m3(codes, (long)nbytes, out_code, (hipStream_t)stream);
}

extern "C" int sd_op_ln_partials(int kind, int M, int N) { return kind == 0 ? (N + 159) / 160 * 2 : 2 * sd_xattn_slices(M, N); }
extern "C" int sd_op_gemm_rowstats(void* stream, const void* X, long long ldx, const void* W, const float* bias, const void* R,
                                   long long ldr, void* C, long long ldc, int M, int N, int K, float* rowstats) {
    if (ensure_zero_page()) return -2;
    SD_REQUIRE(rowstats, "sd_op_gemm_rowstats: null partials buffer");
    GemmArgs a;
    a.X = (const bf16_t*)X; a.ldx = ldx; a.K1 = K; a.W = (const bf16_t*)W; a.bias = bias; a.R = (const bf16_t*)R; a.ldr = ldr;
    a.C = (bf16_t*)C; a.ldc = ldc; a.M = M; a.N = N; a.K = K; a.zero_page = zero_page(); a.splitk = 1; a.rowstats = rowstats;
    return sd_launch_gemm(a, 0, (hipStream_t)stream);
}
extern "C" int sd_op_gemm_plan(void* stream, const void* X, long long ldx, const void* X2, long long ldx2, int K1, const void* W,
                               const float* bias, const float* bias2, const void* R, long long ldr, void* C, long long ldc,
                               int M, int N, int K, float* rowstats, float* stats, const float* ln_rs, int ln_parts,
                               const float* ln_c1, float ln_eps, void* KV, int hm_tokens) {
    if (ensure_zero_page()) return -2;
    GemmArgs a;
    a.X = (const bf16_t*)X; a.ldx = ldx; a.X2 = (const bf16_t*)X2; a.ldx2 = ldx2; a.K1 = K1; a.W = (const bf16_t*)W;
    a.bias = bias; a.bias2 = bias2; a.R = (const bf16_t*)R; a.ldr = ldr; a.C = (bf16_t*)C; a.ldc = ldc; a.M = M; a.N = N; a.K = K;
    a.zero_page = zero_page(); a.splitk = 1; a.rowstats = rowstats; a.stats = stats;
    a.ln_rs = ln_rs; a.ln_np = ln_parts; a.ln_c1 = ln_c1; a.ln_eps = ln_eps;
    if (hm_tokens > 0) {
        SD_REQUIRE(N % 3 == 0 && KV, "sd_op_gemm_plan: head-major K / V needs N = 3 C and a KV buffer");
        a.KV = (bf16_t*)KV; a.hm_C = N / 3; a.hm_tok = hm_tokens;
    }
    return sd_launch_gemm(a, 0, (hipStream_t)stream);
}
extern "C" int sd_op_gemm_ln(void* stream, const void* X, long long ldx, const void* Wg, const float* c1, const float* c2,
                             const float* rowstats, int parts, float eps, void* C, long long ldc, int M, int N, int K, int epi) {
    if (ensure_zero_page()) return -2;
    SD_REQUIRE(epi == 0 || epi == 1, "sd_op_gemm_ln: epi %d (0 = plain, 1 = GEGLU)", epi);
    GemmArgs a;
    a.X = (const bf16_t*)X; a.ldx = ldx; a.K1 = K; a.W = (const bf16_t*)Wg; a.bias = c2;
    a.C = (bf16_t*)C; a.ldc = ldc; a.M = M; a.N = N; a.K = K; a.zero_page = zero_page(); a.splitk = 1;
    a.ln_rs = rowstats; a.ln_np = parts; a.ln_c1 = c1; a.ln_eps = eps;
    return sd_launch_gemm(a, epi, (hipStream_t)stream);
}

extern "C" int sd_op_xattn_fused_rowstats(void* stream, const void* X, const void* R, void* Y, const void* At, const void* Bw,
                                          const float* bias, int M, int C, int rows_per_sample, int L, float* rowstats) {
    SD_REQUIRE(sd_xattn_fused_applicable(rows_per_sample, C, 8, L), "sd_op_xattn_fused_rowstats: shape not supported");
    XattnArgs a = xattn_args(X, R, Y, At, Bw, bias, M, C, rows_per_sample, L);
    a.rowstats = rowstats;
    return sd_launch_xattn_fused(a, (hipStream_t)stream);
}

extern "C" int sd_op_ip_xattn(void* stream, const void* R, void* Rout, const void* A, const void* Bt, const float* gamma,
                              const float* beta, float eps, long long M, int C, int rows_per_sample, int heads, int T) {
    return sd_launch_ip_xattn((const bf16_t*)R, (bf16_t*)Rout, (const bf16_t*)A, (const bf16_t*)Bt, gamma, beta, eps, (long)M, C,
                              rows_per_sample, heads, T, (hipStream_t)stream);
}

extern "C" int sd_op_xattn_expand(void* stream, const void* kv, void* out, int B, int L, int C, int heads, int slots, int col_off,
                                  float scale) {
    SD_REQUIRE(col_off == 0 || col_off == C, "sd_op_xattn_expand: col_off %d (0 = the K half, C = the V half of a row)", col_off);
    return sd_launch_xattn_expand((const bf16_t*)kv, (bf16_t*)out, B, L, C, heads, col_off, scale, (hipStream_t)stream, slots);
}

extern "C" int sd_op_transpose_bf16(void* stream, const void* src, void* dst, int B, int R, int Cc, int perm16) {
    return sd_launch_transpose_bf16((const bf16_t*)src, (bf16_t*)dst, B, R, Cc, (hipStream_t)stream, perm16);
}

extern "C" int sd_op_retile32(void* stream, const void* src, void* dst, int B, int R, int K, int RT) {
    SD_REQUIRE(R > 0 && K > 0, "sd_op_retile32: R=%d K=%d", R, K);
    SD_REQUIRE(((((uintptr_t)src) | (uintptr_t)dst) & 15) == 0, "sd_op_retile32: operands must be 16-byte aligned");
    return sd_launch_retile32((const bf16_t*)src, (bf16_t*)dst, B, R, K, RT, (hipStream_t)stream);
}

extern "C" int sd_op_xattn_fold(void* stream, const void* kv, const void* wqT, const void* wo, const float* lnu, const float* ones,
                                void* at, void* bw, float* c1, float* c2, void* scratch, int UB, int L, int C, int heads, int perm) {
    if (ensure_zero_page()) return -2;
    return sd_launch_xattn_fold((const bf16_t*)kv, (const bf16_t*)wqT, (const bf16_t*)wo, lnu, ones, (bf16_t*)at, (bf16_t*)bw, c1, c2,
                                (bf16_t*)scratch, UB, L, C, heads, perm, (hipStream_t)stream);
}

extern "C" int sd_op_ip_fold(void* stream, const void* ip_kv, const void* wqT, const void* wo, void* at, void* bt, void* scratch,
                             int UB, int T, int C, int heads, float scale) {
    if (ensure_zero_page()) return -2;
    return sd_launch_ip_fold((const bf16_t*)ip_kv, (const bf16_t*)wqT, (const bf16_t*)wo, (bf16_t*)at, (bf16_t*)bt, (bf16_t*)scratch,
                             UB, T, C, heads, scale, (hipStream_t)stream);
}

extern "C" int sd_op_xattn_fused(void* stream, const void* X, const void* R, void* Y, const void* At, const void* Bw,
                                 const float* bias, int M, int C, int rows_per_sample, int L) {
    SD_REQUIRE(sd_xattn_fused_applicable(rows_per_sample, C, 8, L) || getenv("SD_XATTN_FUSED"),
               "sd_op_xattn_fused: shape not supported (8 heads x 80 key slots, 64 < L <= 80, C %% 32 == 0, tokens per sample %% 128 == 0)");
    return sd_launch_xattn_fused(xattn_args(X, R, Y, At, Bw, bias, M, C, rows_per_sample, L), (hipStream_t)stream);
}

extern "C" int sd_op_xattn_fused_ln(void* stream, const void* X, const void* R, void* Y, const void* At, const void* Bw,
                                    const float* bias, int M, int C, int rows_per_sample, int L, const float* ln_rowstats,
                                    int ln_parts, long long ln_rows, const float* c2, float eps, float* rowstats) {
    SD_REQUIRE(sd_xattn_fused_applicable(rows_per_sample, C, 8, L), "sd_op_xattn_fused_ln: shape not supported");
    SD_REQUIRE(ln_rowstats && c2, "sd_op_xattn_fused_ln: null operand");
    XattnArgs a = xattn_args(X, R, Y, At, Bw, bias, M, C, rows_per_sample, L);
    a.rowstats = rowstats;
    a.ln_rs = ln_rowstats; a.ln_np = ln_parts; a.ln_rows = ln_rows; a.ln_c2 = c2; a.ln_eps = eps;
    return sd_launch_xattn_fused(a, (hipStream_t)stream);
}

extern "C" int sd_op_xattn_fused_stamps(void* stream, const void* X, const void* R, void* Y, const void* At, const void* Bw,
                                        const float* bias, int M, int C, int rows_per_sample, int L, unsigned long long* stamps) {
    SD_REQUIRE(stamps, "sd_op_xattn_fused_stamps: null stamp buffer");
    SD_REQUIRE(sd_xattn_fused_applicable(rows_per_sample, C, 8, L), "sd_op_xattn_fused_stamps: shape not supported");
    XattnArgs a = xattn_args(X, R, Y, At, Bw, bias, M, C, rows_per_sample, L);
    a.stamps = stamps;
    return sd_launch_xattn_fused(a, (hipStream_t)stream);
}
```

sonicdiffusionbayeslab_amd/csrc/plan.hip:

```cpp
#include "model.h"

#include <stdlib.h>

namespace sdhip {

namespace {

struct Builder {
    sd_unet* u;
    Plan& pl;
    int UB;
    std::vector<Wrap> wrapstack;
    std::map<int, int> stats_of;
    std::map<int, float> tscale;
    static std::string stem(const std::string& key) {
        const size_t n = key.rfind(".weight");
        return n == std::string::npos ? key : key.substr(0, n);
    }
    std::string error;
    float xscale(int t) {
        auto it = tscale.find(t);
        if (it == tscale.end()) {
            if (error.empty()) error = "fp8 consumer of a tensor without a scale";
            return 1.0f;
// ... 72 lines not shown
    }
    static int pad128(int c) { return (c + 127) / 128 * 128; }
    int gn(int x1, int c1, int x2, int c2, int hw, const std::string& g, const std::string& b, float eps, int silu,
           bool fq = false) {
        Op o; o.kind = OP_GN; o.x1 = x1; o.C1 = c1; o.x2 = x2; o.C2 = c2; o.HW = hw; o.B = UB;
        o.g = W(g); o.be = W(b); o.eps = eps; o.silu = silu;
        o.nsplit = sd_groupnorm_nsplit(UB, hw);
        o.aux = tensor(sd_groupnorm_scratch_bytes(UB, hw, u->cfg.norm_num_groups));
        if (hw % 64 == 0 && !sd_groupnorm_uses_small(UB, hw, c1, c2, u->cfg.norm_num_groups) && stats_of.count(x1) &&
            (x2 < 0 || stats_of.count(x2))) {
            o.s1 = stats_of[x1];
            o.s2 = x2 >= 0 ? stats_of[x2] : -1;
        }
        if (fq) {
            o.out_fp8 = 1; o.Cpad = pad128(c1 + c2); o.sname = u->act_id(stem(g), u->s_norm); o.os = u->act_scale[o.sname];
            o.out = tensor((size_t)UB * hw * o.Cpad); tscale[o.out] = o.os;
        } else o.out = tensor((size_t)UB * hw * (c1 + c2) * 2);
        push(o);
        return o.out;
    }
    int conv3(int x, int hin, int win, int cin, int cout, int stride, int up, const std::string& w, const std::string& b,
              long b2idx, int b2t, int r, bool fq = false) {
        Op o; o.kind = OP_CONV3; o.x1 = x; o.B = UB; o.Hin = hin; o.Win = win; o.Cin = cin; o.N = cout;
        o.stride = stride; o.up = up;
        o.Hout = ((hin << up) + 2 - 3) / stride + 1;
        o.Wout = ((win << up) + 2 - 3) / stride + 1;
        o.M = UB * o.Hout * o.Wout; o.K = 9 * cin; o.Kalg = o.K;
        o.b = W(b); o.b2t = b2t; o.b2idx = b2idx; o.r = r;
        if (fq) { o.dt = 1; o.Cin = pad128(cin); o.K = 9 * o.Cin; o.w = W(w + ".fp8"); o.wsc = W(w + ".scale"); o.xs = xscale(x); }
        else o.w = W(w);
        static const bool subpix_off = getenv("SD_CONV_SUBPIXEL") && atoi(getenv("SD_CONV_SUBPIXEL")) == 0;
        if (up && !fq && !subpix_off && u->kind == 0 && stride == 1 && r < 0 && b2t < 0 && (hin * win) % 64 == 0 &&
            u->woff.count(w + ".sub")) {
            o.subpix = 1; o.K = 4 * cin; o.Kalg = 4 * cin;
            o.w = W(w + ".sub"); o.splitk = 1;
            o.out = tensor((size_t)o.M * cout * 2);
            if ((hin * win) % 128 == 0) want_stats(o, o.M, cout);
            push(o);
            return o.out;
        }
        o.splitk = sd_conv3x3_splitk(o.M, o.N, o.Cin, hin, win, stride, up, o.dt);
        if (o.splitk > 1) o.aux = tensor((size_t)o.splitk * o.M * o.N * 4);
        o.out = tensor((size_t)o.M * cout * 2);
        GemmArgs g;
        g.M = o.M; g.N = o.N; g.Cin = o.Cin; g.K = o.K; g.ldw = o.K; g.Hin = hin; g.Win = win; g.Hout = o.Hout; g.Wout = o.Wout;
        g.stride = stride; g.up = up; g.dt = o.dt;
        if (sd_conv_halo_mode(g) != 2) want_stats(o, o.M, cout);
        push(o);
        return o.out;
    }
    int gemm(int x1, int k1, int x2, int k2, int M, int N, const std::string& w, const std::string& b, int r, int epi,
             bool fq = false, const std::string& oname = "") {
        Op o; o.kind = OP_GEMM; o.x1 = x1; o.x2 = x2; o.K1 = k1; o.K = k1 + k2; o.Kalg = o.K; o.M = M; o.N = N; o.epi = epi;
        o.b = b.empty() ? NOFF : W(b); o.r = r;
        if (fq) { o.dt = 1; o.K = o.K1 = pad128(k1); o.w = W(w + ".fp8"); o.wsc = W(w + ".scale"); o.xs = xscale(x1); }
        else o.w = W(w);
        o.splitk = epi ? 1 : sd_gemm_splitk(M, N, o.dt ? o.K / 2 : o.K, o.dt ? 128 : 0);
        if (o.splitk > 1) o.aux = tensor((size_t)o.splitk * M * N * 4);
        if (!oname.empty()) {
            o.out_fp8 = 1; o.sname = u->act_id(oname, u->s_ff); o.os = u->act_scale[o.sname]; o.Cpad = pad128(N / 2);
            o.out = tensor((size_t)M * o.Cpad); tscale[o.out] = o.os;
        } else o.out = tensor((size_t)M * (epi ? N / 2 : N) * 2);
        push(o);
        return o.out;
    }
    int ln(int x, int M, int C, const std::string& g, const std::string& b, bool fq = false, float eps = 1e-5f) {
        Op o; o.kind = OP_LN; o.x1 = x; o.M = M; o.N = C; o.g = W(g); o.be = W(b); o.eps = eps;
        if (fq) {
            o.out_fp8 = 1; o.Cpad = pad128(C); o.sname = u->act_id(stem(g), u->s_norm); o.os = u->act_scale[o.sname];
            o.out = tensor((size_t)M * o.Cpad); tscale[o.out] = o.os;
        } else o.out = tensor((size_t)M * C * 2);
        push(o);
        return o.out;
    }
    int attn(int q, long qoff, long ldq, int kv, long koff, long voff, long ldkv, int nq, int nk, int C, int heads, int B) {
        Op o; o.kind = OP_ATTN; o.x1 = q; o.x2 = kv; o.qoff = qoff; o.koff = koff; o.voff = voff;
        o.ldq = ldq; o.ldk = o.ldv = ldkv; o.ldo = C; o.B = B; o.heads = heads; o.D = C / heads;
        o.Nq = nq; o.Nk = nk;
        o.out = tensor((size_t)B * nq * C * 2);
        push(o);
        return o.out;
    }
    bool shortcut_fuse = !(getenv("SD_SHORTCUT_FUSE") && atoi(getenv("SD_SHORTCUT_FUSE")) == 0);
    int resnet(const std::string& p, int x1, int c1, int x2, int c2, int cout, int rh, int rw, int tproj_t) {
        const int hw = rh * rw, cin = c1 + c2, M = UB * hw;
        const bool fq = u->fp8;
        int t1 = gn(x1, c1, x2, c2, hw, p + "norm1.weight", p + "norm1.bias", u->cfg.norm_eps, 1, fq);
        int t2 = conv3(t1, rh, rw, cin, cout, 1, 0, p + "conv1.weight", p + "conv1.bias", u->tproj_off.at(p), tproj_t, -1, fq);
        int t3 = gn(t2, cout, -1, 0, hw, p + "norm2.weight", p + "norm2.bias", u->cfg.norm_eps, 1, fq);
        int sc = x1;
        if (cin != cout) {
            GemmArgs g;
            g.M = M; g.N = cout; g.Cin = cout; g.K = 9 * cout; g.ldw = g.K; g.Hin = g.Hout = rh; g.Win = g.Wout = rw;
            g.Csc1 = c1; g.Csc2 = x2 >= 0 ? c2 : 0;
            if (shortcut_fuse && !fq && u->unet_like() && u->woff.count(p + "conv2.bias+shortcut") && sd_conv_halo_shortcut_applicable(g)) {
                const int out = conv3(t3, rh, rw, cout, cout, 1, 0, p + "conv2.weight", p + "conv2.bias+shortcut", 0, -1, -1, fq);
                Op& o = pl.ops.back();
                o.scx1 = x1; o.scc1 = c1; o.scx2 = x2; o.scc2 = g.Csc2; o.scw = W(p + "conv_shortcut.weight");
                o.Kalg += cin;
                return out;
            }
            sc = gemm(x1, c1, x2, c2, M, cout, p + "conv_shortcut.weight", p + "conv_shortcut.bias", -1, 0);
        }
        return conv3(t3, rh, rw, cout, cout, 1, 0, p + "conv2.weight", p + "conv2.bias", 0, -1, sc, fq);
    }
    int tome_r(int rh, int rw, int C) {
        if (u->kind != 0 || u->fp8 || !(u->tome_ratio > 0.0) || rh <= 0 || pl.lh / rh > u->tome_max_downsample) return 0;
        const int N = rh * rw;
        if (rh % 2 || rw % 2 || N > 16384 || C % 64 || C > 1536) {
            if (error.empty()) error = "Token Merging needs even token-grid sides, at most 16384 tokens and C a multiple of 64 up to 1536 on "
                                       "every merging level (" + std::to_string(rh) + "x" + std::to_string(rw) + ", C = " + std::to_string(C) + ")";
            return 0;
        }
        return std::min(N - N / 4, (int)((double)N * u->tome_ratio));
    }
    static int ht_tile_side(int r, int T) {
        for (int d = std::min(T, r); d <= r; ++d)
            if (r % d == 0) return d;
        return r;
    }
    void hypertile_tiles(int rh, int rw, int* nh, int* nw) {
        *nh = *nw = 1;
        if (u->kind != 0 || u->fp8 || u->ht_tokens <= 0 || rh <= 0 || rw <= 0 || pl.lh / rh > (1 << u->ht_max_depth)) return;
        *nh = rh / ht_tile_side(rh, u->ht_tokens);
        *nw = rw / ht_tile_side(rw, u->ht_tokens);
    }
    int n_transformers = 0;
    int transformer(const std::string& p, int x, int C, int rh, int rw) {
        const int blk = pl.pag_blocks++;
        const bool pert = pl.pag_lb > 0 && ((u->pag_mask >> blk) & 1);
        if (pert && prefix_rep > 1) {
            x = replicate(x, (size_t)UB * rh * rw * C * 2, prefix_rep);
            UB *= prefix_rep;
            prefix_rep = 1;
        }
        int ht_nh, ht_nw;
        hypertile_tiles(rh, rw, &ht_nh, &ht_nw);
        if (ht_nh * ht_nw == 1) return transformer_block(p, x, C, rh, rw, 1, pert);
        if (u->tome_ratio > 0.0) { if (error.empty()) error = "HyperTile and Token Merging together are not built"; return x; }
        if (sd_hypertile_shape_ok(UB, rh, rw, C, ht_nh, ht_nw, C, "HyperTile")) { if (error.empty()) error = sd_last_error(); return x; }
        pl.hypertile.push_back(Plan::HtBlock{rh, rw, ht_nh, ht_nw});
        int xp;
        { Op o; o.kind = OP_HT_GATHER; o.x1 = x; o.B = UB; o.Hin = rh; o.Win = rw; o.N = C; o.K = ht_nh; o.K1 = ht_nw;
          o.out = xp = tensor((size_t)UB * rh * rw * C * 2); push(o); }
        if (stats_of.count(x)) stats_of[xp] = stats_of[x];
        const int yp = transformer_block(p, xp, C, rh, rw, ht_nh * ht_nw, pert);
        Op o; o.kind = OP_HT_SCATTER; o.x1 = yp; o.B = UB; o.Hin = rh; o.Win = rw; o.N = C; o.K = ht_nh; o.K1 = ht_nw;
        o.out = tensor((size_t)UB * rh * rw * C * 2); push(o);
        if (stats_of.count(yp)) stats_of[o.out] = stats_of[yp];
        return o.out;
    }
    int transformer_block(const std::string& p, int x, int C, int rh, int rw, int nt, bool pert) {
        const int hw = rh * rw, L = u->cfg.context_len;
        const int NH = block_heads(u->cfg, p), NP = NH * 80;
        int M = UB * hw;
        const std::string t = p + "transformer_blocks.0.";
        const bool fq = u->fp8;
        int g = gn(x, C, -1, 0, hw, p + "norm.weight", p + "norm.bias", 1e-6f, 0, fq);
        int h0 = gemm(g, C, -1, 0, M, C, p + "proj_in.weight", p + "proj_in.bias", -1, 0, fq);
        const int tr = tome_r(rh, rw, C);
        const int Nm = hw - tr, Mm = UB * Nm;
        int tome_i = -1;
        int qkv, rs = -1, np = 0;
        if (tr > 0) {
            const int num_dst = hw / 4, num_src = hw - num_dst;
            Plan::TomeBlock tb;
            tb.B = UB; tb.h = rh; tb.w = rw; tb.r = tr; tb.choice_off = pl.tome_choice_bytes;
            pl.tome_choice_bytes += num_dst;
            tb.tok = tensor((size_t)hw * 4, true);
            tb.kept = tensor((size_t)UB * std::max(num_src - tr, 1) * 4, true);
            tb.merged = tensor((size_t)UB * tr * 4, true);
            tb.dst_idx = tensor((size_t)UB * tr * 4, true);
            int n1 = ln(h0, M, C, t + "norm1.weight", t + "norm1.bias");
            int nmax, nidx;
            { Op o; o.kind = OP_TOME_MATCH; o.x1 = h0; o.B = UB; o.Hin = rh; o.Win = rw; o.N = C; o.b2idx = tb.choice_off;
              o.out = nmax = tensor((size_t)UB * num_src * 4); o.aux = nidx = tensor((size_t)UB * num_src * 4);
              o.stats = tb.tok; o.rs = tensor((size_t)UB * hw * 4); push(o); }
            { Op o; o.kind = OP_TOME_SELECT; o.x1 = nmax; o.x2 = nidx; o.B = UB; o.M = num_src; o.K = tr;
              o.out = tb.kept; o.aux = tb.merged; o.stats = tb.dst_idx; push(o); }
            int m;
            { Op o; o.kind = OP_TOME_MERGE; o.x1 = n1; o.x2 = tb.tok; o.r = tb.kept; o.wt = tb.merged; o.s1 = tb.dst_idx;
              o.B = UB; o.Hin = rh; o.Win = rw; o.N = C; o.K = tr; o.out = m = tensor((size_t)Mm * C * 2); push(o); }
            tome_i = (int)pl.tome.size();
            pl.tome.push_back(tb);
            qkv = gemm(m, C, -1, 0, Mm, 3 * C, t + "attn1.qkv.weight", "", -1, 0);
        } else if (!fq && (np = want_rowstats(pl.ops.back(), M, C, rs)) > 0) {
            qkv = gemm_ln(h0, rs, np, M, 3 * C, C, t + "attn1.qkv.weight", 0);
        } else {
            int n1 = ln(h0, M, C, t + "norm1.weight", t + "norm1.bias", fq);
            qkv = gemm(n1, C, -1, 0, M, 3 * C, t + "attn1.qkv.weight", "", -1, 0, fq);
        }
        static const bool hm_off = (getenv("SD_ATTN_HEADMAJOR") && atoi(getenv("SD_ATTN_HEADMAJOR")) == 0) ||
                                   getenv("SD_ATTN_NO_PIPE") || getenv("SD_ATTN_NO_DMA") || getenv("SD_GEMM_BIG");
        const int Na = Nm / nt;
        const bool hm = !hm_off && C / NH == 40 && C % 160 == 0 && Na % 128 == 0 && Na >= 256 &&
                        sd_gemm_tile_rows(Mm, 3 * C) == 128 && pl.ops.back().splitk == 1;
        if (pert && (tr > 0 || fq || pl.pag_lb >= UB)) {
            if (error.empty()) error = "PAG with Token Merging or fp8, or a batch without unperturbed samples, is not built";
            return x;
        }
        const int Ba = (pert ? UB - pl.pag_lb : UB) * nt;
        const int qkv_op = (int)pl.ops.size() - 1;
        if (pl.sag && p == "mid_block.attentions.0.") {
            if (nt != 1) { if (error.empty()) error = "SAG with a HyperTile setting that tiles the mid block is not built"; return x; }
            if (tr > 0 || fq || pert) { if (error.empty()) error = "SAG with Token Merging, fp8 or PAG is not built"; return x; }
            if (rh < 4 || rh > 16 || rw < 4 || rw > 16) {
                if (error.empty()) error = "SAG: the mid grid is " + std::to_string(rh) + "x" + std::to_string(rw) + " (4 .. 16 tokens per side)";
                return x;
            }
            if (sd_sag_mass_shape_ok(UB, NH, hw, C / NH, 3 * C, hm ? 1 : 0, "SAG")) { if (error.empty()) error = sd_last_error(); return x; }
            Op o; o.kind = OP_SAG_MASS; o.x1 = qkv; o.B = UB; o.heads = NH; o.D = C / NH; o.Nk = hw; o.Hin = rh; o.Win = rw;
            o.koff = C; o.ldk = 3 * C;
            push(o);
        }
        int a1;
        if (hm) {
            pl.ops[qkv_op].hm = 1;
            pl.ops[qkv_op].HW = Na;
            a1 = attn(qkv, 0, C, qkv, (long)Mm * C, 2l * Mm * C, C, Na, Na, C, NH, Ba);
            pl.ops.back().hm = 1;
        } else {
            a1 = attn(qkv, 0, 3 * C, qkv, C, 2 * C, 3 * C, Na, Na, C, NH, Ba);
        }
        pl.ops.back().qps = 1;
        if (pert) {
            const long row0 = (long)(UB - pl.pag_lb) * hw, rows = (long)pl.pag_lb * hw;
            if (sd_pag_identity_shape_ok(Mm, row0, rows, C, NH, 3 * C, hm ? Na : 0, "PAG")) { if (error.empty()) error = sd_last_error(); return x; }
            pl.tensors[a1].bytes = ((size_t)Mm * C * 2 + 255) / 256 * 256;
            Op o; o.kind = OP_PAG_IDENTITY; o.x1 = qkv; o.out = a1; o.M = Mm; o.N = C; o.heads = NH; o.qoff = row0; o.koff = rows;
            o.hm = hm ? 1 : 0; o.HW = hm ? Na : 0; o.voff = hm ? 2l * Mm * C : 2 * C; o.ldv = 3 * C;
            push(o);
        }
        int h1 = gemm(a1, C, -1, 0, Mm, C, t + "attn1.to_out.0.weight", t + "attn1.to_out.0.bias", tr > 0 ? -1 : h0, 0);
        const int to_out_op = (int)pl.ops.size() - 1;
        if (tr > 0) {
            const Plan::TomeBlock& tb = pl.tome[tome_i];
            Op o; o.kind = OP_TOME_UNMERGE; o.x1 = h1; o.r = h0; o.x2 = tb.tok; o.wt = tb.kept; o.s1 = tb.merged; o.s2 = tb.dst_idx;
            o.B = UB; o.Hin = rh; o.Win = rw; o.N = C; o.K = tr; o.out = tensor((size_t)M * C * 2); push(o);
            h1 = o.out;
        }
        if (prefix_rep > 1) {
            x = replicate(x, (size_t)M * C * 2, prefix_rep);
            h1 = replicate(h1, (size_t)M * C * 2, prefix_rep);
            UB *= prefix_rep;
            M = UB * hw;
            prefix_rep = 1;
        }
// ... 464 lines not shown
                }
                h = resnet(bp + "resnets." + std::to_string(j) + ".", hin, ch, sin, sc, co, rh, rw, t_proj);
                ch = co;
                if (c.attn_levels[lev]) h = transformer(bp + "attentions." + std::to_string(j) + ".", h, co, rh, rw);
                wrapstack.pop_back();
            }
            if (i < nl - 1) {
                wrapstack.push_back(Wrap{2, rb, 0});
                const std::string up = bp + "upsamplers.0.conv.";
                h = conv3(h, rh, rw, co, co, 1, 1, up + "weight", up + "bias", 0, -1, -1);
                wrapstack.pop_back();
                rh *= 2; rw *= 2;
            }
            wrapstack.pop_back();
            pl.taps["up" + std::to_string(i)] = h;
        }
        if (pl.tgate && pl.tg_blocks != (int)pl.tg_rows.size() && error.empty()) error = "T-GATE cache layout (block count)";
        int g = gn(h, ch, -1, 0, rh * rw, "conv_norm_out.weight", "conv_norm_out.bias", c.norm_eps, 1);
        { Op o; o.kind = OP_CONV_OUT; o.x1 = g; o.out = T_EPS; o.B = UB; o.Hin = rh; o.Win = rw; o.Cin = ch; o.N = c.out_channels;
          o.w = W("conv_out.weight"); o.b = W("conv_out.bias"); push(o); }
    }
};

bool wrap_skipped(const Wrap& w, int branch) {
    const int cache_layer_id = branch % 3, cache_block_id = branch / 3;
    if (w.block_i > cache_block_id || w.type == 1) return true;
    if (w.block_i < cache_block_id) return false;
    return w.type == 0 ? w.layer_i >= cache_layer_id : w.layer_i > cache_layer_id;
}

void op_tensors(const Op& o, int ins[32], int& nin) {
    nin = 0;
    for (int t : {o.x1, o.x2, o.r, o.b2t, o.wt, o.s1, o.s2, o.lnrs, o.slab_t, o.slab_r, o.slab_b2t, o.scx1, o.scx2})
        if (t >= 0) ins[nin++] = t;
    for (int k = 0; k < o.nres; ++k) ins[nin++] = o.res_t[k];
}

void fuse_deferred_reduce(sd_unet* u, Plan& pl) {
    if (getenv("SD_GN_SLAB") && atoi(getenv("SD_GN_SLAB")) == 0) return;
    const int nops = (int)pl.ops.size();
    auto skipped = [&](const Op& o) {
        if (pl.branch < 0) return false;
        for (int k = 0; k < o.nwrap; ++k)
            if (wrap_skipped(o.wraps[k], pl.branch)) return true;
        return false;
    };
    std::vector<int> producer(pl.tensors.size(), -1);
    for (int i = 0; i < nops; ++i)
        if (pl.ops[i].out >= 0) producer[pl.ops[i].out] = i;
    for (int g = 0; g < nops; ++g) {
        Op& G = pl.ops[g];
        if (G.kind != OP_GN || G.out_fp8 || G.x1 < 0 || !sd_groupnorm_slab_ok(G.B, G.HW, G.C1, G.C2, u->cfg.norm_num_groups)) continue;
        const int p = producer[G.x1];
        if (p < 0 || p >= g) continue;
        Op& P = pl.ops[p];
        if (P.kind != OP_CONV3 && !(P.kind == OP_GEMM && P.epi == 0)) continue;
        if (P.splitk <= 1 || P.splitk > 64 || P.aux < 0 || P.dt || P.out_fp8 || P.defer || P.subpix) continue;
        if (P.kind == OP_GEMM && (P.coff || P.ldc_o || P.hm || P.rs >= 0 || P.lnrs >= 0)) continue;
        if ((long)G.B * G.HW != P.M || G.C1 != P.N || skipped(P) != skipped(G)) continue;
        bool first_reader = true;
        for (int i = p + 1; i < g && first_reader; ++i) {
            int ins[32], nin;
            op_tensors(pl.ops[i], ins, nin);
            for (int k = 0; k < nin; ++k)
                if (ins[k] == P.out) first_reader = false;
        }
        if (!first_reader) continue;
        P.defer = 1;
        G.slab_t = P.aux; G.slab_k = P.splitk; G.slab_b = P.b; G.slab_r = P.r;
        G.slab_b2t = P.kind == OP_CONV3 ? P.b2t : -1; G.slab_b2idx = P.b2idx;
    }
}

void assign_memory(sd_unet* u, Plan& pl) {
    const int nops = (int)pl.ops.size();
    pl.skipped.assign(nops, 0);
    if (pl.branch >= 0) {
        for (int i = 0; i < nops; ++i)
            for (int k = 0; k < pl.ops[i].nwrap; ++k)
                if (wrap_skipped(pl.ops[i].wraps[k], pl.branch)) pl.skipped[i] = 1;
        std::vector<int> producer(pl.tensors.size(), -1);
        for (int i = 0; i < nops; ++i) {
            if (pl.ops[i].out >= 0) producer[pl.ops[i].out] = i;
            if (pl.ops[i].stats >= 0) producer[pl.ops[i].stats] = i;
            if (pl.ops[i].rs >= 0) producer[pl.ops[i].rs] = i;
        }
        for (int i = 0; i < nops; ++i) {
            if (pl.skipped[i]) continue;
            int ins[32], nin;
            op_tensors(pl.ops[i], ins, nin);
            for (int k = 0; k < nin; ++k) {
                const int p = producer[ins[k]];
                if (p >= 0 && pl.skipped[p]) pl.tensors[ins[k]].persistent = true;
            }
        }
    }
    if (u->debug_taps)
        for (auto& kv : pl.taps) pl.tensors[kv.second].persistent = true;
    for (int i = 0; i < nops; ++i) {
        const Op& o = pl.ops[i];
        int ins[32], nin;
        op_tensors(o, ins, nin);
        for (int k = 0; k < nin; ++k) pl.tensors[ins[k]].last = std::max(pl.tensors[ins[k]].last, i);
        for (int t : {o.out, o.aux, o.stats, o.rs})
            if (t >= 0) {
                if (pl.tensors[t].def < 0) pl.tensors[t].def = i;
                pl.tensors[t].last = std::max(pl.tensors[t].last, i);
            }
    }
    size_t off = 0;
    for (auto& t : pl.tensors)
        if (t.ctx && !t.ctx_ip) { t.off = off; off += t.bytes; }
    for (auto& t : pl.tensors)
        if (t.ctx_ip) { t.off = off; off += t.bytes; }
    for (auto& t : pl.tensors)
        if (t.persistent && !t.ctx) { t.off = off; off += t.bytes; }
    const size_t arena0 = off;
    struct Live { size_t off, bytes; int last; };
    std::vector<Live> live;
    size_t high = arena0;
    std::vector<std::vector<int>> def_at(nops);
    for (int t = 0; t < (int)pl.tensors.size(); ++t)
        if (!pl.tensors[t].persistent && pl.tensors[t].def >= 0) def_at[pl.tensors[t].def].push_back(t);
    for (int i = 0; i < nops; ++i) {
        for (int t : def_at[i]) {
            std::sort(live.begin(), live.end(), [](const Live& a, const Live& b) { return a.off < b.off; });
            size_t cur = arena0;
            for (const Live& l : live) {
                if (l.off >= cur + pl.tensors[t].bytes) break;
                cur = std::max(cur, l.off + l.bytes);
            }
            pl.tensors[t].off = cur;
            live.push_back(Live{cur, pl.tensors[t].bytes, pl.tensors[t].last});
            high = std::max(high, cur + pl.tensors[t].bytes);
        }
        live.erase(std::remove_if(live.begin(), live.end(), [i](const Live& l) { return l.last <= i; }), live.end());
    }
    pl.total_bytes = high + 4096;
}

}

int transformer_block_count(const sd_unet_config& c) {
    int n = 1;
    for (int i = 0; i < c.num_levels; ++i)
        if (c.attn_levels[i]) n += 2 * c.layers_per_block + 1;
    return n;
}

int plan_rep(const sd_unet* u, int latent_batch, int unet_batch) {
    if (u->kind == 0 && u->pag_mask)
        return (latent_batch > 0 && (unet_batch == 3 * latent_batch || unet_batch == 2 * latent_batch)) ? unet_batch / latent_batch : 1;
    static const bool off = getenv("SD_CFG_DEDUP") && atoi(getenv("SD_CFG_DEDUP")) == 0;
    return (!off && u->unet_like() && u->cfg.attn_levels[0] && latent_batch > 0 && unet_batch == 2 * latent_batch) ? 2 : 1;
}

int check_latent_size(const sd_unet* u, int lh, int lw, const char* who) {
    if (u->kind == 1 || u->kind == 4) {
        SD_REQUIRE(lh >= 8 && lw >= 8 && lh <= 128 && lw <= 128 && lh % 8 == 0 && lw % 8 == 0,
                   "%s: latent %dx%d (the VAE %s takes sides that are multiples of 8 in [8, 128])", who, lh, lw,
                   u->kind == 1 ? "decoder" : "encoder");
    } else if (u->unet_like()) {
        const int d = 1 << (u->cfg.num_levels - 1);
        SD_REQUIRE(lh >= d && lw >= d && lh <= 256 && lw <= 256 && lh % d == 0 && lw % d == 0,
                   "%s: latent %dx%d (both sides must be multiples of %d, at most 256)", who, lh, lw, d);
    }
    return 0;
}

size_t control_segments(const sd_unet_config& c, int UB, int lh, int lw, std::vector<size_t>* off, std::vector<long>* count) {
    off->clear(); count->clear();
    size_t bytes = 0;
    auto seg = [&](int C, int h, int w) {
        const long n = (long)UB * h * w * C;
        off->push_back(bytes); count->push_back(n);
        bytes = (bytes + (size_t)n * 2 + 255) / 256 * 256;
    };
    int h = lh, w = lw;
    seg(c.block_out_channels[0], h, w);
    for (int i = 0; i < c.num_levels; ++i) {
        for (int j = 0; j < c.layers_per_block; ++j) seg(c.block_out_channels[i], h, w);
        if (i < c.num_levels - 1) { h /= 2; w /= 2; seg(c.block_out_channels[i], h, w); }
    }
    seg(c.block_out_channels[c.num_levels - 1], h, w);
    return bytes;
}

// ... 101 lines not shown
```

sonicdiffusionbayeslab_amd/csrc/unet.hip:

```cpp
#include "model.h"

#include <stdarg.h>
#include <stdio.h>
#include <stdlib.h>

#include <chrono>

static thread_local char g_err[1024] = "";
void sd_set_error(const char* fmt, ...) {
    va_list ap;
    va_start(ap, fmt);
    vsnprintf(g_err, sizeof(g_err), fmt, ap);
    va_end(ap);
}
extern "C" const char* sd_last_error(void) { return g_err; }
extern "C" int sd_abi_version(void) { return 3; }

static void* g_zero_page = nullptr;

namespace sdhip {

int ensure_zero_page() {
    if (g_zero_page) return 0;
    SD_CHECK_HIP(hipMalloc(&g_zero_page, 4096));
// ... 15 lines not shown
        case OP_GEMV:
            return sd_launch_gemv((const float*)T(o.x1), (const bf16_t*)(wb + o.w), (const float*)(wb + o.b),
                                  (float*)T(o.out), o.N, o.K, o.silu_in, stream);
        case OP_CONV_IN:
            if (u->kind == 0 && o.Cin == 9) {
                SD_REQUIRE(u->inpaint_b > 0, "forward: this UNet has in_channels = 9 and no inpainting condition is set "
                                             "(sd_unet_set_inpaint_cond_hw: mask and masked-image latents)");
                SD_REQUIRE(u->inpaint_h == o.Hin && u->inpaint_w == o.Win && o.B % u->inpaint_b == 0,
                           "forward: the inpainting condition was set for batch %d at %dx%d, the forward runs batch %d at %dx%d",
                           u->inpaint_b, u->inpaint_h, u->inpaint_w, o.B, o.Hin, o.Win);
                return sd_launch_conv_in_cond(latents, latent_batch, u->dinpaint, u->inpaint_b, (const float*)(wb + o.w),
                                              (const float*)(wb + o.b), (bf16_t*)T(o.out), o.B, o.Hin, o.Win, o.N, stream);
            }
            if (u->kind == 5) {
                SD_REQUIRE(u->cn_b > 0, "controlnet_forward: no conditioning image is set (sd_controlnet_set_cond_hw)");
                SD_REQUIRE(u->cn_h == o.Hin && u->cn_w == o.Win && o.B % u->cn_b == 0,
                           "controlnet_forward: the conditioning image was set for batch %d at %dx%d, the forward runs batch %d at %dx%d",
                           u->cn_b, u->cn_h, u->cn_w, o.B, o.Hin, o.Win);
                return sd_launch_conv_in_add(latents, latent_batch, u->cn_embed, u->cn_b, (const float*)(wb + o.w),
                                             (const float*)(wb + o.b), (bf16_t*)T(o.out), o.B, o.Hin, o.Win, o.N, stream);
            }
            return sd_launch_conv_in(o.x1 >= 0 ? (const float*)T(o.x1) : latents, o.x1 >= 0 ? o.B : latent_batch,
                                     (const float*)(wb + o.w), (const float*)(wb + o.b), (bf16_t*)T(o.out), o.B, o.Hin,
                                     o.Win, o.Cin, o.N, stream);
        case OP_PQCONV:
            return sd_launch_pqconv(latents, (const float*)(wb + o.w), (const float*)(wb + o.b), (float*)T(o.out), o.B,
                                    o.HW, timestep , stream);
        case OP_SOFTMAX:
            if (o.N > 4096) return sd_launch_softmax_rows_long((bf16_t*)T(o.x1), o.M, o.N, o.scale, stream);
            return sd_launch_softmax_rows((bf16_t*)T(o.x1), o.M, o.N, o.scale, stream);
        case OP_GN: {
            GroupNormArgs a;
            a.x1 = (const bf16_t*)T(o.x1); a.C1 = o.C1; a.x2 = (const bf16_t*)T(o.x2); a.C2 = o.C2;
            a.gamma = (const float*)(wb + o.g); a.beta = (const float*)(wb + o.be);
            a.y = (bf16_t*)T(o.out); a.partial = (float*)T(o.aux);
            a.B = o.B; a.HW = o.HW; a.groups = u->cfg.norm_num_groups; a.nsplit = o.nsplit; a.eps = o.eps; a.silu = o.silu;
            a.out_fp8 = o.out_fp8; a.Cpad = o.Cpad; a.oscale = o.os;
            a.stats1 = (const float*)T(o.s1); a.stats2 = (const float*)T(o.s2);
            if (o.slab_t >= 0) {
                a.slab = (const float*)T(o.slab_t); a.splitk = o.slab_k; a.x1w = (bf16_t*)T(o.x1);
                a.sbias = o.slab_b != NOFF ? (const float*)(wb + o.slab_b) : nullptr;
                a.sbias2 = o.slab_b2t >= 0 ? (const float*)T(o.slab_b2t) + o.slab_b2idx : nullptr;
                a.sR = (const bf16_t*)T(o.slab_r); a.sldr = o.C1;
            }
            return sd_launch_groupnorm(a, stream);
        }
        case OP_CONV3: {
            GemmArgs a;
            a.X = (const bf16_t*)T(o.x1); a.W = (const bf16_t*)(wb + o.w); a.bias = (const float*)(wb + o.b);
            a.bias2 = o.b2t >= 0 ? (const float*)T(o.b2t) + o.b2idx : nullptr;
            a.R = (const bf16_t*)T(o.r); a.ldr = o.N; a.C = (bf16_t*)T(o.out); a.ldc = o.N;
            a.M = o.M; a.N = o.N; a.K = o.K; a.K1 = o.K;
            a.Hin = o.Hin; a.Win = o.Win; a.Cin = o.Cin; a.Hout = o.Hout; a.Wout = o.Wout; a.stride = o.stride; a.up = o.up;
            a.zero_page = g_zero_page; a.splitk = o.splitk; a.slab = (float*)T(o.aux); a.defer_reduce = o.defer;
            if (o.dt) { a.dt = 1; a.wscale = (const float*)(wb + o.wsc); a.xscale_inv = 1.0f / o.xs; }
            a.stats = (float*)T(o.stats);
            a.asym = o.asym;
            if (o.subpix) { a.subpix = 1; a.up = 0; a.w_batch_stride = (long)o.N * 4 * o.Cin; }
            if (o.scw != NOFF) {
                a.Xs1 = (const bf16_t*)T(o.scx1); a.Csc1 = o.scc1; a.Xs2 = (const bf16_t*)T(o.scx2); a.Csc2 = o.scc2;
                a.Wsc = (const bf16_t*)(wb + o.scw); a.ldwsc = o.scc1 + o.scc2;
            }
            return sd_launch_conv3x3(a, stream);
        }
        case OP_GEMM: {
            GemmArgs a;
            a.X = o.wx != NOFF ? (const bf16_t*)(wb + o.wx) : (const bf16_t*)T(o.x1) + o.xoff;
            a.ldx = o.ldx_o ? o.ldx_o : o.K1; a.X2 = (const bf16_t*)T(o.x2); a.ldx2 = o.K - o.K1; a.K1 = o.K1;
            a.W = o.wt >= 0 ? (const bf16_t*)T(o.wt) + o.woff_el : (const bf16_t*)(wb + o.w); a.ldw = o.ldw_o;
            a.bias = o.b != NOFF ? (const float*)(wb + o.b) : nullptr;
            a.R = (const bf16_t*)T(o.r); a.ldr = o.N; a.C = (bf16_t*)T(o.out) + o.coff;
            a.ldc = o.ldc_o ? o.ldc_o : (o.epi == 1 ? o.N / 2 : o.N);
            a.M = o.M; a.N = o.N; a.K = o.K; a.zero_page = g_zero_page; a.splitk = o.splitk; a.slab = (float*)T(o.aux);
            a.defer_reduce = o.defer;
            a.w_batch_stride = o.wbs; a.rows_per_batch = o.rpb; a.sm_valid = o.sm_valid;
            if (o.dt) { a.dt = 1; a.wscale = (const float*)(wb + o.wsc); a.xscale_inv = 1.0f / o.xs; }
            if (o.out_fp8) { a.out_fp8 = 1; a.oscale = o.os; a.ldc = o.Cpad; }
            a.stats = (float*)T(o.stats);
            a.rowstats = (float*)T(o.rs);
            if (o.hm) { a.hm_C = o.N / 3; a.hm_tok = o.HW; a.ldc = a.hm_C; a.KV = (bf16_t*)T(o.out) + (long)o.M * a.hm_C; }
            if (o.lnrs >= 0) { a.ln_rs = (const float*)T(o.lnrs); a.ln_np = o.lnnp; a.ln_c1 = (const float*)(wb + o.c1); a.ln_eps = 1e-5f; }
            if (o.lnrs >= 0 && o.s1 >= 0) { a.ln_c1 = (const float*)T(o.s1); a.bias = (const float*)T(o.s2); a.ln_per_sample = 1; }
            return sd_launch_gemm(a, o.epi, stream);
        }
        case OP_LN:
            if (o.out_fp8)
                return sd_launch_layernorm_fp8((const bf16_t*)T(o.x1), (const float*)(wb + o.g), (const float*)(wb + o.be),
                                               T(o.out), o.M, o.N, o.Cpad, o.eps, o.os, stream);
            return sd_launch_layernorm((const bf16_t*)T(o.x1), (const float*)(wb + o.g), (const float*)(wb + o.be),
                                       (bf16_t*)T(o.out), o.M, o.N, o.eps, stream);
        case OP_ATTN: {
            AttnArgs a;
            a.Q = (const bf16_t*)T(o.x1) + o.qoff; a.ldq = o.ldq;
            a.K = (const bf16_t*)T(o.x2) + o.koff; a.ldk = o.ldk;
            a.V = (const bf16_t*)T(o.x2) + o.voff; a.ldv = o.ldv;
            a.O = (bf16_t*)T(o.out); a.ldo = o.ldo;
            a.B = o.B; a.heads = o.heads; a.Nq = o.Nq; a.Nk = o.Nk; a.D = o.D;
            a.scale = 1.0f / sqrtf((float)o.D);
            a.q_prescaled = o.qps;
            a.consts = g_zero_page;
            a.kv_head_major = o.hm;
            return sd_launch_attention(a, stream);
        }
        case OP_XATTN: {
            XattnArgs a;
            a.X = (const bf16_t*)T(o.x1); a.R = (const bf16_t*)T(o.r); a.Y = (bf16_t*)T(o.out);
            a.At = (const bf16_t*)T(o.wt); a.Bw = (const bf16_t*)T(o.x2); a.bias = (const float*)(wb + o.b);
            a.M = o.M; a.C = o.N; a.rows_per_sample = o.rpb; a.L = o.sm_valid;
            a.rowstats = (float*)T(o.rs);
            if (o.lnrs >= 0) {
                a.ln_rs = (const float*)T(o.lnrs); a.ln_np = o.lnnp; a.ln_rows = o.ldx_o; a.ln_c2 = (const float*)T(o.s1); a.ln_eps = 1e-5f;
            }
            return sd_launch_xattn_fused(a, stream);
        }
        case OP_IP_XATTN:
            return sd_launch_ip_xattn((const bf16_t*)T(o.x1), (bf16_t*)T(o.out), (const bf16_t*)T(o.wt), (const bf16_t*)T(o.x2),
                                      (const float*)(wb + o.g), (const float*)(wb + o.be), o.eps, o.M, o.N, o.rpb, o.heads,
                                      u->cfg.ip_adapter_tokens, stream);
        case OP_RES_ADD: {
            SD_REQUIRE(u->ctrl_res && o.nres == (int)pl.cn_off.size() && o.nres <= MAX_CONTROL_RES, "forward: no ControlNet residuals are set");
            bf16_t* x[MAX_CONTROL_RES];
            const bf16_t* r[MAX_CONTROL_RES];
            long n[MAX_CONTROL_RES];
            for (int k = 0; k < o.nres; ++k) {
                x[k] = (bf16_t*)T(o.res_t[k]); r[k] = (const bf16_t*)(u->ctrl_res + pl.cn_off[k]); n[k] = pl.cn_count[k];
                SD_REQUIRE((size_t)n[k] * 2 <= pl.tensors[o.res_t[k]].bytes, "forward: ControlNet residual %d exceeds its tensor", k);
            }
            return sd_launch_residual_add(x, r, n, o.nres, u->ctrl_scale, stream);
        }
        case OP_FREEU:
            SD_REQUIRE(u->freeu_on && (o.epi == 0 || o.epi == 1), "forward: FreeU is off (sd_unet_set_freeu)");
            return sd_launch_freeu((const bf16_t*)T(o.x1), (const bf16_t*)T(o.x2), (bf16_t*)T(o.out), (bf16_t*)T(o.aux), o.B, o.Hin, o.Win,
                                   o.C1, o.C2, u->freeu_b[o.epi], u->freeu_s[o.epi], stream);
        case OP_TGATE_ZERO:
            SD_CHECK_HIP(hipMemsetAsync(T(o.out), 0, pl.tensors[o.out].bytes, stream));
            return 0;
        case OP_TGATE_CAPTURE:
        case OP_TGATE_APPLY: {
            SD_REQUIRE(u->tg_cache && o.b2idx >= 0 && o.b2idx < (long)pl.tg_off.size() &&
                           pl.tg_off[o.b2idx] + (size_t)pl.tg_rows[o.b2idx] * o.N * 2 <= (size_t)u->tg_bytes,
                       "forward: no T-GATE cache for block %ld (sd_unet_set_tgate_hw)", o.b2idx);
            bf16_t* slice = (bf16_t*)(u->tg_cache + pl.tg_off[o.b2idx]);
            if (o.kind == OP_TGATE_APPLY)
                return sd_launch_tgate_apply((const bf16_t*)T(o.x1), slice, (bf16_t*)T(o.out), (float*)T(o.rs), o.M, o.N, stream);
            return sd_launch_tgate_capture((const bf16_t*)T(o.x1), (const bf16_t*)T(o.r), (bf16_t*)T(o.out), slice, (float*)T(o.rs),
                                           o.M / o.K, o.N, o.K, stream);
        }
        case OP_REPLICATE:
            return sd_launch_replicate(T(o.x1), T(o.out), (long)o.M * 16, o.N, stream);
        case OP_HT_GATHER:
            return sd_launch_hypertile_gather((const bf16_t*)T(o.x1), o.N, (bf16_t*)T(o.out), o.B, o.Hin, o.Win, o.N, o.K, o.K1, stream);
        case OP_HT_SCATTER:
            return sd_launch_hypertile_scatter((const bf16_t*)T(o.x1), (bf16_t*)T(o.out), o.N, o.B, o.Hin, o.Win, o.N, o.K, o.K1, stream);
        case OP_PAG_IDENTITY:
            return sd_launch_pag_identity((const bf16_t*)T(o.x1) + o.voff, o.ldv, o.HW, (bf16_t*)T(o.out), o.M, o.qoff, o.koff, o.N, o.heads, stream);
        case OP_SAG_MASS:
            SD_REQUIRE(u->sag_mass && (long long)o.B * o.Nk <= u->sag_mass_floats, "forward: SAG capture is on and the mass buffer holds %lld "
                       "floats, batch %d at a %dx%d mid grid takes %lld (sd_unet_set_sag_buffer)", u->sag_mass ? u->sag_mass_floats : 0ll, o.B,
                       o.Hin, o.Win, (long long)o.B * o.Nk);
            return sd_launch_sag_attn_mass((const bf16_t*)T(o.x1), (const bf16_t*)T(o.x1) + o.koff, o.ldk, u->sag_mass, o.B, o.heads, o.Nk, o.D, 1, stream);
        case OP_TOME_MATCH:
            SD_REQUIRE(u->tome_choice && o.b2idx + (long)(o.Hin / 2) * (o.Win / 2) <= u->tome_choice_n, "forward: no Token Merging choice array");
            return sd_launch_tome_match((const bf16_t*)T(o.x1), u->tome_choice + o.b2idx, o.B, o.Hin, o.Win, o.N, (float*)T(o.out),
                                        (int*)T(o.aux), (int*)T(o.stats), (float*)T(o.rs), stream);
        case OP_TOME_SELECT:
            return sd_launch_tome_select((const float*)T(o.x1), (const int*)T(o.x2), o.B, o.M, o.K, (int*)T(o.out), (int*)T(o.aux),
// ... 1220 lines not shown
    if (check_workspace(*plp, "calibrate_fp8", workspace, workspace_bytes)) return -1;
    u->ip_keys.clear();
    hipStream_t st = (hipStream_t)stream;
    unsigned* dmax = (unsigned*)op_scratch(256);
    SD_REQUIRE(dmax, "calibrate_fp8: cannot allocate scratch");
    std::vector<float> eps((size_t)unet_batch * u->cfg.out_channels * u->cfg.sample_size * u->cfg.sample_size);
    float* deps = nullptr;
    SD_CHECK_HIP(hipMalloc((void**)&deps, eps.size() * 4));
    std::map<int, float> cur;
    const Plan& pl = *plp;
    auto measure = [&](const Op& o, float probe, float* amax) -> int {
        Op t = o; t.os = probe;
        int r = run_op(u, pl, t, (char*)workspace, latents, latent_batch, deps, timestep, st);
        if (r) return r;
        SD_CHECK_HIP(hipMemsetAsync(dmax, 0, 4, st));
        const Tn& tn = pl.tensors[o.out];
        const long rows = o.kind == OP_GN ? (long)o.B * o.HW : (long)o.M;
        if ((r = sd_launch_amax_e4m3((char*)workspace + tn.off, rows * o.Cpad, dmax, st))) return r;
        unsigned code = 0;
        SD_CHECK_HIP(hipMemcpyAsync(&code, dmax, 4, hipMemcpyDeviceToHost, st));
        SD_CHECK_HIP(hipStreamSynchronize(st));
        *amax = code >= 0x7e ? -1.f : e4m3_code_value(code) / probe;
        return 0;
    };
    for (size_t i = 0; i < pl.ops.size() && !rc; ++i) {
        Op o = pl.ops[i];
        if (o.dt) {
            auto it = cur.find(o.x1);
            if (it != cur.end()) o.xs = it->second;
        }
        if (o.out_fp8 && o.sname >= 0) {
            float amax = 0.f;
            rc = measure(o, 448.f / 4096.f, &amax);
            if (!rc && amax < 0.f) rc = measure(o, 448.f / 1048576.f, &amax);
            if (rc) break;
            if (amax < 0.f) amax = 1048576.f;
            float& seen = u->act_amax[o.sname];
            seen = std::max(seen, amax);
            const float want = 448.f / (margin * std::max(seen, 1e-6f));
            const float sc = ldexpf(1.f, (int)floorf(log2f(want)));
            u->act_scale[o.sname] = std::min(std::max(sc, ldexpf(1.f, -20)), ldexpf(1.f, 20));
            o.os = u->act_scale[o.sname];
            cur[o.out] = o.os;
        }
        rc = run_op(u, pl, o, (char*)workspace, latents, latent_batch, deps, timestep, st);
    }
    (void)hipStreamSynchronize(st);
    (void)hipFree(deps);
    if (rc) return rc;
    u->plans.clear();
    return 0;
}

extern "C" int sd_unet_fp8_scale_count(const sd_unet* u) { return u ? (int)u->act_names.size() : -1; }

extern "C" int sd_unet_fp8_scale_info(const sd_unet* u, int index, char* name, int name_cap, float* scale, float* amax) {
    SD_REQUIRE(u && index >= 0 && index < (int)u->act_names.size(), "fp8_scale_info: bad index %d", index);
    if (name && name_cap > 0) snprintf(name, name_cap, "%s", u->act_names[index].c_str());
    if (scale) *scale = u->act_scale[index];
    if (amax) *amax = u->act_amax[index];
    return 0;
}

extern "C" int sd_unet_set_fp8_scale(sd_unet* u, const char* name, float scale) {
    SD_REQUIRE(u && u->kind == 0 && u->fp8 && name, "set_fp8_scale: not an fp8 UNet handle");
    SD_REQUIRE(scale > 0.f && scale == scale, "set_fp8_scale: scale %g", scale);
    auto it = u->act_index.find(name);
    SD_REQUIRE(it != u->act_index.end(), "set_fp8_scale: no e4m3 activation tensor '%s' (build a plan first: sd_unet_workspace_bytes)", name);
    u->act_scale[it->second] = scale;
    u->plans.clear();
    return 0;
}

static void op_work(const Op& o, double* flops, double* bytes) {
    *flops = 0; *bytes = 0;
    switch (o.kind) {
        case OP_CONV3:
        case OP_GEMM: {
            const double K = o.Kalg ? o.Kalg : o.K, esz = o.dt ? 1.0 : 2.0;
            *flops = 2.0 * o.M * o.N * K;
            *bytes = esz * ((double)o.M * K + (double)o.N * K) + (o.out_fp8 ? 1.0 : 2.0) * (double)o.M * (o.epi == 1 ? o.N / 2 : o.N);
            break;
        }
        case OP_XATTN:
            *flops = 4.0 * o.M * (double)o.N * o.N + 4.0 * o.M * (double)o.sm_valid * o.N;
            *bytes = 3.0 * 2.0 * o.M * o.N;
            break;
        case OP_ATTN:
            *flops = 4.0 * o.B * o.heads * (double)o.Nq * o.Nk * o.D;
            *bytes = 2.0 * o.B * o.heads * o.D * (2.0 * o.Nq + 2.0 * o.Nk);
            break;
        case OP_GN:
            *bytes = 2.0 * 2.0 * o.B * (double)o.HW * (o.C1 + o.C2);
            break;
        case OP_LN:
            *bytes = 2.0 * 2.0 * (double)o.M * o.N;
            break;
        case OP_REPLICATE:
            *bytes = 16.0 * o.M * (1.0 + o.N);
            break;
        case OP_TOME_MATCH: {
            const double N = (double)o.Hin * o.Win;
            *flops = 2.0 * o.B * (0.75 * N) * (0.25 * N) * o.N;
            *bytes = 2.0 * o.B * N * o.N;
            break;
        }
        case OP_TOME_MERGE:
        case OP_TOME_UNMERGE:
            *bytes = 2.0 * o.B * (2.0 * o.Hin * o.Win - o.K) * (double)o.N;
            break;
        case OP_FREEU:
            *flops = 2.0 * 14.0 * o.B * (double)o.Hin * o.Win * o.C2;
            *bytes = 2.0 * o.B * (double)o.Hin * o.Win * (2.0 * o.C1 + 3.0 * o.C2);
            break;
        case OP_SAG_MASS:
            *flops = 2.0 * o.B * o.heads * (double)o.Nk * o.Nk * o.D;
            *bytes = 2.0 * 2.0 * o.B * (double)o.Nk * o.heads * o.D + 4.0 * o.B * o.Nk;
            break;
        case OP_PAG_IDENTITY:
            *bytes = 2.0 * 2.0 * (double)o.koff * o.N;
            break;
        case OP_HT_GATHER:
        case OP_HT_SCATTER:
            *bytes = 2.0 * 2.0 * o.B * (double)o.Hin * o.Win * o.N;
            break;
        case OP_RES_ADD:
            *bytes = 3.0 * 2.0 * (double)o.M;
            break;
        case OP_TGATE_CAPTURE:
            *bytes = 2.0 * (double)o.M * o.N * (3.0 + 1.0 / o.K);
            break;
        case OP_TGATE_APPLY:
            *bytes = 3.0 * 2.0 * (double)o.M * o.N;
            break;
        case OP_IP_XATTN:
            *flops = 4.0 * o.M * 32.0 * o.N;
            *bytes = 2.0 * 2.0 * o.M * o.N;
            break;
        default:
            break;
    }
}

static int profiled_run(sd_unet* u, void* stream, const float* latents, int latent_batch, int unet_batch, float timestep,
                        float* eps_out, void* workspace, long long workspace_bytes, int cache_mode, int cache_branch_id,
                        Plan** plan, std::vector<std::pair<int, float>>* per_op) {
    SD_REQUIRE(latents && eps_out && workspace, "forward_profiled: null argument");
    SD_REQUIRE(latent_batch > 0 && unet_batch % latent_batch == 0, "forward_profiled: bad batch");
    Plan* pl;
    const int rep = plan_rep(u, latent_batch, unet_batch);
    const int ip = u->ip_keys.empty() ? 0 : 1;
    if (ip && check_ip_set(u, "forward_profiled", unet_batch, cache_branch_id, u->cfg.sample_size, u->cfg.sample_size)) return -1;
    const int cn = u->ctrl_res ? 1 : 0;
    if (cn && check_control_set(u, "forward_profiled", unet_batch, u->cfg.sample_size, u->cfg.sample_size, cache_mode, cache_branch_id)) return -1;
    if (u->tg_mode && check_tgate_forward(u, "forward_profiled", latent_batch, unet_batch, u->cfg.sample_size, u->cfg.sample_size, cache_mode,
                                          cache_branch_id, ip, cn)) return -1;
    if (u->pag_mask && check_pag_forward(u, "forward_profiled", latent_batch, unet_batch, cache_mode, cache_branch_id, ip, cn)) return -1;
    if (u->sag_on && check_sag_forward(u, "forward_profiled", cache_mode, cache_branch_id, ip, cn)) return -1;
    u->last_rep = rep; u->last_ip = ip; u->last_cn = cn;
    u->last_h = u->last_w = u->cfg.sample_size;
    int rc = get_plan(u, unet_batch, cache_branch_id, &pl, rep, -1, -1, ip, cn);
    if (rc) return rc;
    *plan = pl;
    if ((rc = ensure_tome_choice(u, pl->tome_choice_bytes, stream))) return rc;
    SD_REQUIRE((long long)pl->total_bytes <= workspace_bytes, "forward_profiled: workspace too small");
    hipStream_t st = (hipStream_t)stream;
    std::vector<hipEvent_t> ev;
    std::vector<int> which;
    auto mark = [&]() -> int {
        hipEvent_t e;
        SD_CHECK_HIP(hipEventCreate(&e));
        SD_CHECK_HIP(hipEventRecord(e, st));
        ev.push_back(e);
        return 0;
    };
    if (mark()) return -2;
    for (size_t i = 0; i < pl->ops.size(); ++i) {
        if (cache_mode == SD_CACHE_SKIP && pl->skipped[i]) continue;
        rc = run_op(u, *pl, pl->ops[i], (char*)workspace, latents, latent_batch, eps_out, timestep, st);
        if (mark()) return -2;
        which.push_back((int)i);
        if (rc) break;
    }
    SD_CHECK_HIP(hipStreamSynchronize(st));
    if (u->tg_mode == TGATE_CAPTURE) u->tg_captured = rc == 0;
    for (size_t j = 0; j < which.size(); ++j) {
        float ms = 0.f;
        (void)hipEventElapsedTime(&ms, ev[j], ev[j + 1]);
        per_op->push_back({which[j], ms});
    }
    for (auto e : ev) (void)hipEventDestroy(e);
    return rc;
}

extern "C" int sd_unet_forward_profiled(sd_unet* u, void* stream, const float* latents, int latent_batch, int unet_batch,
                                        float timestep, float* eps_out, void* workspace, long long workspace_bytes,
                                        int cache_mode, int cache_branch_id, double kind_ms[SD_PROFILE_KINDS],
                                        long long kind_launches[SD_PROFILE_KINDS], double kind_flops[SD_PROFILE_KINDS],
                                        double kind_bytes[SD_PROFILE_KINDS]) {
    SD_REQUIRE(kind_ms && kind_launches && kind_flops && kind_bytes, "forward_profiled: null argument");
    Plan* pl = nullptr;
    std::vector<std::pair<int, float>> per_op;
    const int rc = profiled_run(u, stream, latents, latent_batch, unet_batch, timestep, eps_out, workspace, workspace_bytes,
                                cache_mode, cache_branch_id, &pl, &per_op);
    if (!pl) return rc;
    for (int k = 0; k < SD_PROFILE_KINDS; ++k) { kind_ms[k] = 0; kind_launches[k] = 0; kind_flops[k] = 0; kind_bytes[k] = 0; }
    for (auto& [i, ms] : per_op) {
        const Op& o = pl->ops[i];
        double fl, by;
        op_work(o, &fl, &by);
        bool halo4 = false;
        if (o.kind == OP_CONV3 && !o.dt && o.subpix) {
            GemmArgs a;
            a.M = o.M; a.N = o.N; a.K = o.K; a.K1 = o.K; a.Hin = o.Hin; a.Win = o.Win; a.Cin = o.Cin; a.Hout = o.Hout; a.Wout = o.Wout;
            a.stride = o.stride; a.up = 0; a.subpix = 1; a.splitk = o.splitk; a.slab = (float*)(o.aux >= 0 ? (void*)1 : nullptr);
            a.w_batch_stride = (long)o.N * 4 * o.Cin;
            halo4 = sd_conv_halo_subpix_applicable(a);
        }
        const int kd = o.kind == OP_SAG_MASS ? 12 : o.kind == OP_PAG_IDENTITY ? 11 : o.kind == OP_HT_GATHER ? 9 : o.kind == OP_HT_SCATTER ? 10 : o.kind == OP_TGATE_CAPTURE ? 24 : o.kind == OP_TGATE_APPLY ? 25 : o.kind == OP_TGATE_ZERO ? 26 : o.kind == OP_XATTN ? 18 : o.kind == OP_REPLICATE ? 19 : o.kind == OP_IP_XATTN ? 22 : o.kind == OP_RES_ADD ? 23 : halo4 ? 21 :
                       (o.kind == OP_CONV3 && !o.dt && (o.subpix || o.stride != 1)) ? 20 :
                       (o.dt ? (o.kind == OP_CONV3 ? 16 : 17) : o.kind);
        kind_ms[kd] += ms; kind_launches[kd] += 1; kind_flops[kd] += fl; kind_bytes[kd] += by;
    }
    return rc;
}

extern "C" long long sd_unet_forward_op_times(sd_unet* u, void* stream, const float* latents, int latent_batch, int unet_batch,
                                              float timestep, float* eps_out, void* workspace, long long workspace_bytes,
                                              int cache_mode, int cache_branch_id, char* text, long long cap) {
    SD_REQUIRE(text && cap > 0, "forward_op_times: null argument");
    Plan* pl = nullptr;
    std::vector<std::pair<int, float>> per_op;
    const int rc = profiled_run(u, stream, latents, latent_batch, unet_batch, timestep, eps_out, workspace, workspace_bytes,
                                cache_mode, cache_branch_id, &pl, &per_op);
    if (rc) return rc;
    long long n = 0;
    for (auto& [i, ms] : per_op) {
        const Op& o = pl->ops[i];
        double fl, by;
        op_work(o, &fl, &by);
        const int w = snprintf(text + n, (size_t)(cap - n), "%d %d %d %d %d %.5f %.3f %.3f\n", i, (int)o.kind, o.M, o.N,
                               o.kind == OP_GN ? o.slab_k : o.K, ms, fl * 1e-9, by * 1e-6);
        if (w < 0 || n + w >= cap) break;
        n += w;
    }
    return n;
}

extern "C" int sd_unet_debug_tensor(sd_unet* u, void* stream, const char* name, float* host_out, long long numel,
                                    void* workspace, int unet_batch, int cache_branch_id) {
    SD_REQUIRE(u && u->debug_taps, "debug_tensor: create the handle with SD_DEBUG_TAPS=1 in the environment");
    if (u->kind == 5 && name && !strcmp(name, "cond_embedding")) {
        SD_REQUIRE(u->cn_b > 0, "debug_tensor: no conditioning image is set");
        const size_t have = (size_t)u->cn_b * u->cn_h * u->cn_w * u->cfg.block_out_channels[0];
        SD_REQUIRE(numel >= 0 && (size_t)numel <= have, "debug_tensor: 'cond_embedding' holds %zu elements", have);
        std::vector<unsigned short> tmp(numel);
        SD_CHECK_HIP(hipStreamSynchronize((hipStream_t)stream));
        SD_CHECK_HIP(hipMemcpy(tmp.data(), u->cn_embed, (size_t)numel * 2, hipMemcpyDeviceToHost));
        for (long long i = 0; i < numel; ++i) {
            unsigned v = (unsigned)tmp[i] << 16;
            memcpy(&host_out[i], &v, 4);
        }
        return 0;
    }
    Plan* pl;
    int rc = get_plan(u, unet_batch, cache_branch_id, &pl, u->last_rep, u->last_h > 0 ? u->last_h : -1, u->last_w > 0 ? u->last_w : -1, u->last_ip, u->last_cn);
    if (rc) return rc;
    auto it = pl->taps.find(name);
    SD_REQUIRE(it != pl->taps.end(), "debug_tensor: unknown tap '%s'", name);
    const Tn& t = pl->tensors[it->second];
    SD_REQUIRE((size_t)numel * 2 <= t.bytes, "debug_tensor: '%s' holds at most %zu elements", name, t.bytes / 2);
    std::vector<unsigned short> tmp(numel);
    SD_CHECK_HIP(hipStreamSynchronize((hipStream_t)stream));
    SD_CHECK_HIP(hipMemcpy(tmp.data(), (char*)workspace + t.off, (size_t)numel * 2, hipMemcpyDeviceToHost));
    for (long long i = 0; i < numel; ++i) {
        unsigned v = (unsigned)tmp[i] << 16;
        memcpy(&host_out[i], &v, 4);
    }
    return 0;
}

extern "C" int sd_inpaint_prepare(void* stream, const float* image, const float* mask, float* masked_image, float* latent_mask,
                                  int batch, int height, int width) {
    return sd_launch_inpaint_prepare(image, mask, masked_image, latent_mask, batch, height, width, (hipStream_t)stream);
}
```

sonicdiffusionbayeslab_amd/unet.py:

```python
from __future__ import annotations

import ctypes as C
import math
from typing import Dict, Optional

import torch

from . import _lib
from .handle import ALIGN, HipHandle, Workspace, load_params as _load_params
from .weights import UNetConfig, param_shapes

CACHE_OFF, CACHE_FULL_AND_STORE, CACHE_SKIP = 0, 1, 2
LATENT_CHANNELS = 4


def _c_config(cfg: UNetConfig, weight_dtype: str = "bf16", fp8_act_scales=(0.0, 0.0)) -> _lib.SdUnetConfigFull:
    c = _lib.SdUnetConfigFull()
    if weight_dtype not in _lib.DTYPES:
        raise ValueError(f"weight_dtype {weight_dtype!r}: one of {sorted(_lib.DTYPES)}")
    c.weight_dtype = _lib.DTYPES[weight_dtype]
    c.fp8_act_scale_norm, c.fp8_act_scale_ff = float(fp8_act_scales[0]), float(fp8_act_scales[1])
    c.sample_size, c.in_channels, c.out_channels = cfg.sample_size, cfg.in_channels, cfg.out_channels
    c.num_levels = len(cfg.block_out_channels)
    for i, v in enumerate(cfg.block_out_channels):
# ... 535 lines not shown
        _lib.check(self._lib.sd_unet_set_tgate_hw(self._handle, int(mode), buf.ptr, buf.nbytes, int(latent_batch), h, w),
                   "sd_unet_set_tgate_hw")
        self._tgate = (int(mode), int(latent_batch), h, w)
        if mode == self.TGATE_CAPTURE and self._ws is not None and self._ws_key is not None and self._ws_key[2:] == (h, w):
            self._grow_workspace_for_control()

    def _tgate_workspace(self, unet_batch: int, h: int, w: int) -> Workspace:
        key = (unet_batch, h, w)
        if not self._tgate_ws.holds(key):
            self._tgate_ws.reserve(self._workspace_bytes(unet_batch, -1, h, w), key)
        return self._tgate_ws

    def plan_count(self) -> int:
        return int(self._lib.sd_unet_plan_count(self._handle))

    def forward_latents(self, latents: torch.Tensor, unet_batch: int, timestep: float,
                        out: Optional[torch.Tensor] = None, cache_mode: int = CACHE_OFF, sag_forward: bool = False) -> torch.Tensor:
        if latents.dim() != 4 or latents.shape[1] != LATENT_CHANNELS:
            raise ValueError(f"latents must be [B,{LATENT_CHANNELS},H,W], got {tuple(latents.shape)}")
        b, c, h, w = latents.shape
        if self.config.in_channels == 9 and (self._inpaint_key is None or self._inpaint_key[1:] != (h, w)
                                             or unet_batch % self._inpaint_key[0]):
            raise _lib.SdHipError(f"this UNet has in_channels = 9: set_inpaint_cond(mask, masked_latents) must be called for "
                                  f"this batch and size ({h}x{w}) first")
        gated = self._tgate is not None and self._tgate[0] == self.TGATE_REUSE
        if sag_forward:
            if self._sag or gated or cache_mode != CACHE_OFF:
                raise _lib.SdHipError("a SAG forward runs with capture off (set_sag(False)), without T-GATE and DeepCache")
            if self._sag_ctx_key != (unet_batch, h, w):
                raise _lib.SdHipError(f"set_sag_context(encoder_hidden_states, {h}, {w}) must be called for this batch and size first")
        elif not gated and (self._ctx_key is None or self._ctx_key[2:] != (unet_batch, h, w)):
            raise _lib.SdHipError(f"set_context(encoder_hidden_states, {h}, {w}) must be called for this batch and size first")
        if self._ip_on and (unet_batch, self.cache_branch_id, h, w) not in self._ip_keys:
            raise _lib.SdHipError(f"this UNet runs with an IP-Adapter image prompt: set_ip_adapter(image_embeds, scale, {h}, {w}) must "
                                  f"be called for this batch ({unet_batch}) and size after set_context (or clear_ip_adapter())")
        if self._control is not None and self._control[2:] != (unet_batch, h, w):
            raise _lib.SdHipError(f"the ControlNet residuals were set for batch {self._control[2]} at {self._control[3]}x{self._control[4]}: "
                                  f"set_control_residuals for this batch ({unet_batch}) and size ({h}x{w}), or clear_control_residuals()")
        if latents.dtype != torch.float32 or not latents.is_contiguous() or latents.device != self.device:
            latents = latents.to(self.device, torch.float32).contiguous()
        if out is None:
            out = torch.empty((unet_batch, self.config.out_channels, h, w), dtype=torch.float32, device=self.device)
        ws = self._sag_ws if sag_forward else self._tgate_workspace(unet_batch, h, w) if gated else self._reserve(unet_batch, h, w)
        _lib.check(self._lib.sd_unet_forward_hw(self._handle, _lib.current_stream(), latents.data_ptr(), b, unet_batch, h, w,
                                                float(timestep), out.data_ptr(), ws.ptr, ws.nbytes,
                                                cache_mode, self.cache_branch_id), "sd_unet_forward_hw")
        return out

    def calibrate_fp8(self, latents: torch.Tensor, unet_batch: int, timesteps, margin: float = 2.0) -> Dict[str, float]:
        if self.weight_dtype != "fp8_e4m3":
            raise _lib.SdHipError("calibrate_fp8: the handle was not created with weight_dtype='fp8'")
        if self.cache_branch_id != -1:
            raise _lib.SdHipError("calibrate_fp8: call set_deepcache(-1) and set_context(...) first (the calibration pass runs "
                                  "the plan without DeepCache)")
        s = self.config.sample_size
        if self._ctx_key is None or self._ctx_key[2:] != (unet_batch, s, s):
            raise _lib.SdHipError("set_context(encoder_hidden_states) must be called for this batch first (at sample_size)")
        latents = latents.to(self.device, torch.float32).contiguous()
        if tuple(latents.shape[1:]) != (LATENT_CHANNELS, s, s):
            raise ValueError(f"calibrate_fp8: latents must be [B,{LATENT_CHANNELS},{s},{s}] (sample_size), got {tuple(latents.shape)}")
        ws = self._reserve(unet_batch)
        for t in timesteps:
            _lib.check(self._lib.sd_unet_calibrate_fp8(self._handle, _lib.current_stream(), latents.data_ptr(), latents.shape[0],
                                                       unet_batch, float(t), float(margin), ws.ptr, ws.nbytes),
                       "sd_unet_calibrate_fp8")
        return self.fp8_scales()

    def fp8_scales(self, with_amax: bool = False) -> Dict[str, float]:
        out = {}
        name = C.create_string_buffer(256)
        sc, am = C.c_float(), C.c_float()
        for i in range(self._lib.sd_unet_fp8_scale_count(self._handle)):
            _lib.check(self._lib.sd_unet_fp8_scale_info(self._handle, i, name, 256, C.byref(sc), C.byref(am)), "sd_unet_fp8_scale_info")
            out[name.value.decode()] = (sc.value, am.value) if with_amax else sc.value
        return out

    def set_fp8_scales(self, scales: Dict[str, float]) -> None:
        if self._lib.sd_unet_workspace_bytes(self._handle, 1, -1) < 0:
            _lib.check(-1, "sd_unet_workspace_bytes")
        for k, v in scales.items():
            _lib.check(self._lib.sd_unet_set_fp8_scale(self._handle, k.encode(), float(v)), f"sd_unet_set_fp8_scale({k})")

    KIND_NAMES = {0: "sinusoid", 1: "gemv", 2: "conv_in", 3: "groupnorm", 4: "conv3x3", 5: "gemm", 6: "layernorm",
                  7: "attention", 8: "conv_out", 9: "hypertile_gather", 10: "hypertile_scatter", 11: "pag_identity", 12: "sag_mass", 16: "conv3x3_fp8", 17: "gemm_fp8", 18: "xattn_fused",
                  19: "replicate", 20: "conv3x3_gemm", 21: "conv3x3_halo_subpix", 22: "ip_xattn", 23: "residual_add",
                  24: "tgate_capture", 25: "tgate_apply", 26: "tgate_zero",
                  27: "tome_match", 28: "tome_select", 29: "tome_merge", 30: "tome_unmerge", 31: "freeu"}

    def forward_profiled(self, latents: torch.Tensor, unet_batch: int, timestep: float, cache_mode: int = CACHE_OFF):
        latents = latents.to(self.device, torch.float32).contiguous()
        s = self.config.sample_size
        if tuple(latents.shape[2:]) != (s, s):
            raise ValueError(f"forward_profiled: {s}x{s} latents only, got {tuple(latents.shape)}")
        out = torch.empty((unet_batch, self.config.out_channels, latents.shape[2], latents.shape[3]),
                          dtype=torch.float32, device=self.device)
        gated = self._tgate is not None and self._tgate[0] == self.TGATE_REUSE
        ws = self._tgate_workspace(unet_batch, s, s) if gated else self._reserve(unet_batch)
        ms, fl, by = (C.c_double * 32)(), (C.c_double * 32)(), (C.c_double * 32)()
        ln = (C.c_longlong * 32)()
        _lib.check(self._lib.sd_unet_forward_profiled(
            self._handle, _lib.current_stream(), latents.data_ptr(), latents.shape[0], unet_batch, float(timestep),
            out.data_ptr(), ws.ptr, ws.nbytes, cache_mode, self.cache_branch_id, ms, ln, fl, by),
            "sd_unet_forward_profiled")
        return {n: dict(ms=ms[i], launches=ln[i], flops=fl[i], bytes=by[i]) for i, n in self.KIND_NAMES.items()
                if ln[i] or i < 9}

    def __call__(self, sample: torch.Tensor, timestep, encoder_hidden_states: torch.Tensor = None,
                 timestep_cond=None, cross_attention_kwargs=None, added_cond_kwargs=None, return_dict: bool = False,
                 down_block_additional_residuals=None, mid_block_additional_residual=None, **kwargs):
        if (down_block_additional_residuals is None) != (mid_block_additional_residual is None):
            raise NotImplementedError("down_block_additional_residuals and mid_block_additional_residual go together (a ControlNet's "
                                      "outputs; a T2I-Adapter's down residuals alone are not built)")
        emb = None
        if added_cond_kwargs is not None:
            if self.config.ip_adapter_embed_dim is None:
                raise NotImplementedError("added_cond_kwargs is not part of the SD-1.5 hot path (this UNet has no IP-Adapter)")
            if set(added_cond_kwargs) != {"image_embeds"}:
                raise NotImplementedError(f"added_cond_kwargs {sorted(added_cond_kwargs)}: only {{'image_embeds': ...}} of one "
                                          "IP-Adapter is built")
            emb = self._call_image_embeds(added_cond_kwargs["image_embeds"], sample.shape[0])
        self._apply_timestep_cond(timestep_cond)
        h, w = sample.shape[2], sample.shape[3]
        key = (encoder_hidden_states.data_ptr(), encoder_hidden_states._version, sample.shape[0], h, w)
        if self._ctx_key != key:
            self.set_context(encoder_hidden_states, h, w)
        if emb is None:
            if self._ip_on:
                self.clear_ip_adapter()
        else:
            ip_call = (emb.data_ptr(), emb._version, float(self.ip_adapter_scale), sample.shape[0], self.cache_branch_id, h, w)
            if self._ip_call != ip_call or ip_call[3:] not in self._ip_keys:
                self.set_ip_adapter(emb, self.ip_adapter_scale, h, w)
                self._ip_call = ip_call
        t = float(timestep.item()) if torch.is_tensor(timestep) else float(timestep)
        if down_block_additional_residuals is not None:
            from .controlnet import pack_residuals
            buf = pack_residuals(down_block_additional_residuals, mid_block_additional_residual, self.config, self.device)
            self.set_control_residuals(buf, 1.0, sample.shape[0], h, w)
            try:
                eps = self.forward_latents(sample, sample.shape[0], t)
            finally:
                self.clear_control_residuals()
        else:
            eps = self.forward_latents(sample, sample.shape[0], t)
        return (eps.to(sample.dtype),)

    def _call_image_embeds(self, image_embeds, batch: int) -> torch.Tensor:
        if isinstance(image_embeds, (list, tuple)):
            if len(image_embeds) != 1:
                raise NotImplementedError(f"image_embeds: a list of {len(image_embeds)} (several IP-Adapters at once are not built)")
            image_embeds = image_embeds[0]
        e = self.config.ip_adapter_embed_dim
        if not torch.is_tensor(image_embeds):
            raise ValueError("image_embeds must be a tensor or a one-element list of tensors")
        if image_embeds.dim() == 3:
            if image_embeds.shape[1] != 1:
                raise NotImplementedError(f"image_embeds {tuple(image_embeds.shape)}: several images per sample are not built")
            image_embeds = image_embeds[:, 0]
        if image_embeds.dim() != 2 or image_embeds.shape[1] != e or image_embeds.shape[0] != batch:
            raise ValueError(f"image_embeds must be [{batch}, {e}] or [{batch}, 1, {e}], got {tuple(image_embeds.shape)}")
        return image_embeds

    ONE_ROW_RULE = "timestep_cond must be one row for the whole batch (one guidance scale per call)"

    def _apply_timestep_cond(self, timestep_cond) -> None:
        if timestep_cond is None:
            if self._cond is not None:
# ... 23 lines not shown
```

Before: 11.49 images/s.

## Chain GroupNorm, proj_in and LayerNorm-folded QKV GEMM into one transformer-entry kernel

Adds a persistent tf_entry kernel that applies GroupNorm from producer statistics, runs the proj_in GEMM, and feeds the result straight into the LN-folded QKV GEMM, writing both h0 and Q/KV. The plan uses it for C=320 transformer blocks by default (SD_TF_ENTRY defaults to 2), replacing separate groupnorm, proj_in GEMM and QKV ops. This removes the intermediate global round trips and launches, at the cost of a large hand-written kernel whose own GEMM tiling may be less efficient than the tuned generic GEMM path.

```diff
diff --git a/include/sd_hip.h b/include/sd_hip.h
--- a/include/sd_hip.h
+++ b/include/sd_hip.h
@@ -383,6 +383,12 @@
                     void* KV, int hm_tokens);
 int sd_op_xattn_fused_rowstats(void* stream, const void* X, const void* R, void* Y, const void* At, const void* Bw,
                                const float* bias, int M, int C, int rows_per_sample, int L, float* rowstats);
+int sd_op_tf_entry_applicable(int M, int hw, int C);
+int sd_op_tf_entry(void* stream, const void* x, const float* stats, const float* gamma, const float* beta, int groups, float eps,
+                   const void* Wp, const float* bp, const void* Wqkv_ln, const float* c1, const float* c2, float ln_eps, void* h0,
+                   void* Q, void* KV, int M, int hw, int C, int hm_tokens, int max_workgroups);
+int sd_op_groupnorm_stats(void* stream, const void* x, int C, const float* stats, const float* gamma, const float* beta, void* y,
+                          int B, int HW, int groups, float eps, int silu);
 int sd_op_ip_xattn(void* stream, const void* R, void* Rout, const void* A, const void* Bt, const float* gamma, const float* beta,
                    float eps, long long M, int C, int rows_per_sample, int heads, int T);
 int sd_op_xattn_expand(void* stream, const void* kv, void* out, int B, int L, int C, int heads, int slots, int col_off, float scale);
diff --git a/sonicdiffusionbayeslab_amd/_lib.py b/sonicdiffusionbayeslab_amd/_lib.py
--- a/sonicdiffusionbayeslab_amd/_lib.py
+++ b/sonicdiffusionbayeslab_amd/_lib.py
@@ -253,6 +253,9 @@
     "sd_op_sag_degrade": (_i, [_vp, _vp, _vp, _vp, _i, _i, _i, C.POINTER(_f), _vp, _i, _i, _i]),
     "sd_sched_step_sag": (_i, [_vp, _vp, _i, _f, _f] + [_vp] * 8 + [C.POINTER(_f), _ll, _vp, _ll, _vp, _vp, _vp, _f, _f, _ll]),
     "sd_sched_step_pc_sag": (_i, [_vp, _vp, _i, _f, _f] + [_vp] * 9 + [C.POINTER(_f), _ll, _vp, _ll, _vp, _vp, _vp, _f, _f, _ll]),
+    "sd_op_tf_entry_applicable": (_i, [_i, _i, _i]),
+    "sd_op_tf_entry": (_i, [_vp, _vp, _vp, _vp, _vp, _i, _f, _vp, _vp, _vp, _vp, _vp, _f, _vp, _vp, _vp, _i, _i, _i, _i, _i]),
+    "sd_op_groupnorm_stats": (_i, [_vp, _vp, _i, _vp, _vp, _vp, _vp, _i, _i, _i, _f, _i]),
 }
 
 
diff --git a/sonicdiffusionbayeslab_amd/build.py b/sonicdiffusionbayeslab_amd/build.py
--- a/sonicdiffusionbayeslab_amd/build.py
+++ b/sonicdiffusionbayeslab_amd/build.py
@@ -13,7 +13,7 @@
 LIB_PATH = os.path.join(LIB_DIR, "libsdhip.so")
 ABLATE_LIB_PATH = os.path.join(LIB_DIR, "libsdhip_ablate.so")
 ABLATE_SOURCES = ("gemm_conv.hip", "conv_halo.hip")
-SOURCES = ["gemm_conv.hip", "gemm_lean.hip", "conv_halo.hip", "conv64.hip", "norm.hip", "attention.hip", "xattn.hip", "ip_xattn.hip", "small.hip", "sched.hip", "clip.hip", "vit.hip", "bert.hip", "inception.hip", "unet.hip", "pack.hip", "plan.hip", "taesd.hip", "tome.hip", "freeu.hip", "tgate.hip", "hypertile.hip", "pag.hip", "sag.hip", "ops.hip"]
+SOURCES = ["gemm_conv.hip", "gemm_lean.hip", "tf_entry.hip", "conv_halo.hip", "conv64.hip", "norm.hip", "attention.hip", "xattn.hip", "ip_xattn.hip", "small.hip", "sched.hip", "clip.hip", "vit.hip", "bert.hip", "inception.hip", "unet.hip", "pack.hip", "plan.hip", "taesd.hip", "tome.hip", "freeu.hip", "tgate.hip", "hypertile.hip", "pag.hip", "sag.hip", "ops.hip"]
 HEADERS = ["common.h", "kernels.h", "model.h",os.path.join("..", "..", "include", "sd_hip.h")]
 FLAGS = ["--offload-arch=gfx950", "-O3", "-fPIC", "-std=c++17", "-Wall", "-Wno-unused-function"]
 NO_PACKED_FP32 = ["-Xclang", "-target-feature", "-Xclang", "-packed-fp32-ops"]
@@ -29,7 +29,8 @@
                "hypertile.hip": NO_PACKED_FP32,
                "pag.hip": NO_PACKED_FP32,
                "sag.hip": NO_PACKED_FP32,
-               "gemm_conv.hip": ["-fno-slp-vectorize"], "gemm_lean.hip": ["-fno-slp-vectorize"]}
+               "gemm_conv.hip": ["-fno-slp-vectorize"], "gemm_lean.hip": ["-fno-slp-vectorize"],
+               "tf_entry.hip": ["-fno-slp-vectorize", *NO_PACKED_FP32]}
 _HOST_NOISE = "is not a recognized feature for this target (ignoring feature)"
 
 
diff --git a/sonicdiffusionbayeslab_amd/csrc/common.h b/sonicdiffusionbayeslab_amd/csrc/common.h
--- a/sonicdiffusionbayeslab_amd/csrc/common.h
+++ b/sonicdiffusionbayeslab_amd/csrc/common.h
@@ -161,6 +161,12 @@
 #endif
 }
 
+__device__ __forceinline__ void gn_scale_shift(float mean, float rstd, float gamma, float beta, float& sc, float& sf) {
+    sc = rstd * gamma;
+    sf = beta - mean * sc;
+}
+__device__ __forceinline__ float gn_affine(float x, float sc, float sf) { return x * sc + sf; }
+
 __device__ __forceinline__ float wave_sum(float v) {
 #pragma unroll
     for (int o = 32; o > 0; o >>= 1) v += __shfl_xor(v, o);
diff --git a/sonicdiffusionbayeslab_amd/csrc/kernels.h b/sonicdiffusionbayeslab_amd/csrc/kernels.h
--- a/sonicdiffusionbayeslab_amd/csrc/kernels.h
+++ b/sonicdiffusionbayeslab_amd/csrc/kernels.h
@@ -102,12 +102,34 @@
     int B = 0, HW = 0, groups = 32, nsplit = 0;
     float eps = 1e-5f;
     int silu = 0;
+    int no_small = 0;
 };
 int sd_groupnorm_nsplit(int B, int HW);
 bool sd_groupnorm_uses_small(int B, int HW, int C1, int C2, int groups);
 bool sd_groupnorm_slab_ok(int B, int HW, int C1, int C2, int groups);
 size_t sd_groupnorm_scratch_bytes(int B, int HW, int groups);
 int sd_launch_groupnorm(const GroupNormArgs& a, hipStream_t stream);
+int sd_launch_groupnorm_finalize(const GroupNormArgs& a, hipStream_t stream);
+const float* sd_groupnorm_mean_rstd(const GroupNormArgs& a);
+
+struct TfEntryArgs {
+    const bf16_t* X = nullptr;
+    const float* gn_mr = nullptr;
+    const float* gamma = nullptr; const float* beta = nullptr;
+    int groups = 32;
+    const bf16_t* Wp = nullptr; const float* bp = nullptr;
+    const bf16_t* Wqkv = nullptr;
+    const float* c1 = nullptr; const float* c2 = nullptr;
+    float ln_eps = 1e-5f;
+    bf16_t* H0 = nullptr;
+    bf16_t* Q = nullptr;
+    bf16_t* KV = nullptr;
+    int M = 0, hw = 0, C = 0;
+    int hm_tok = 0;
+    int max_workgroups = 0;
+};
+bool sd_tf_entry_applicable(int M, int hw, int C);
+int sd_launch_tf_entry(const TfEntryArgs& a, hipStream_t stream);
 
 int sd_launch_softmax_rows(bf16_t* s, long rows, int cols, float scale, hipStream_t stream);
 int sd_launch_softmax_rows_long(bf16_t* s, long rows, int cols, float scale, hipStream_t stream);
diff --git a/sonicdiffusionbayeslab_amd/csrc/model.h b/sonicdiffusionbayeslab_amd/csrc/model.h
--- a/sonicdiffusionbayeslab_amd/csrc/model.h
+++ b/sonicdiffusionbayeslab_amd/csrc/model.h
@@ -48,7 +48,8 @@
               OP_TGATE_CAPTURE, OP_TGATE_APPLY, OP_TGATE_ZERO,
               OP_HT_GATHER, OP_HT_SCATTER,
               OP_PAG_IDENTITY,
-              OP_SAG_MASS };
+              OP_SAG_MASS,
+              OP_TF_ENTRY };
 
 constexpr int TGATE_OFF = 0, TGATE_CAPTURE = 1, TGATE_REUSE = 2;
 
@@ -92,6 +93,8 @@
     size_t scw = NOFF;
     int nres = 0;
     int res_t[MAX_CONTROL_RES];
+    int out2 = -1;
+    size_t wqkv = NOFF, c2q = NOFF;
     int nwrap = 0;
     Wrap wraps[3];
 };
diff --git a/sonicdiffusionbayeslab_amd/csrc/norm.hip b/sonicdiffusionbayeslab_amd/csrc/norm.hip
--- a/sonicdiffusionbayeslab_amd/csrc/norm.hip
+++ b/sonicdiffusionbayeslab_amd/csrc/norm.hip
@@ -164,8 +164,7 @@
         for (int j = 0; j < 8; ++j) {
             const float gm = j < 4 ? ga[j & 3] : gb[j & 3], bt = j < 4 ? ba[j & 3] : bb[j & 3];
             const float mean = j < nb ? m0 : m1, rstd = j < nb ? r0 : r1;
-            sc[j] = rstd * gm;
-            sf[j] = bt - mean * sc[j];
+            gn_scale_shift(mean, rstd, gm, bt, sc[j], sf[j]);
         }
     }
     const int per = (a.HW + a.nsplit - 1) / a.nsplit;
@@ -175,7 +174,7 @@
                       bflo(v[2]), bfhi(v[2]), bflo(v[3]), bfhi(v[3])};
 #pragma unroll
         for (int j = 0; j < 8; ++j) {
-            f[j] = f[j] * sc[j] + sf[j];
+            f[j] = gn_affine(f[j], sc[j], sf[j]);
             if (SILU) f[j] = silu_f(f[j]);
         }
         if (FP8) {
@@ -695,7 +694,7 @@
         SD_CHECK_HIP(hipGetLastError());
         return 0;
     }
-    if (sd_groupnorm_uses_small(a.B, a.HW, a.C1, a.C2, a.groups)) {
+    if (!(a.no_small && a.stats1) && sd_groupnorm_uses_small(a.B, a.HW, a.C1, a.C2, a.groups)) {
         const int units = (a.HW * (C / a.groups / 4) + 255) / 256;
         const dim3 grid(a.groups, a.B);
         auto go = [&](auto kern) { hipLaunchKernelGGL(kern, grid, dim3(256), 0, stream, a); };
@@ -725,6 +724,19 @@
         if (a.silu) hipLaunchKernelGGL((gn_apply_kernel<true, false>), grid, dim3(g.threads), 0, stream, a);
         else hipLaunchKernelGGL((gn_apply_kernel<false, false>), grid, dim3(g.threads), 0, stream, a);
     }
+    SD_CHECK_HIP(hipGetLastError());
+    return 0;
+}
+
+const float* sd_groupnorm_mean_rstd(const GroupNormArgs& a) { return a.partial + (long)a.B * a.nsplit * a.groups * 2; }
+
+int sd_launch_groupnorm_finalize(const GroupNormArgs& a, hipStream_t stream) {
+    const int C = a.C1 + a.C2;
+    SD_REQUIRE(a.partial && a.stats1 && (a.C2 == 0 || a.stats2), "groupnorm statistics: null operand");
+    SD_REQUIRE(a.groups > 0 && a.groups <= 64 && C % a.groups == 0 && a.B > 0 && a.HW > 0 && a.HW % 64 == 0 && a.nsplit >= 1,
+               "groupnorm statistics: C=%d groups=%d HW=%d (producer statistics come in 64-row blocks)", C, a.groups, a.HW);
+    SD_REQUIRE(!a.slab, "groupnorm statistics: not with a deferred split-K reduce");
+    hipLaunchKernelGGL(gn_finalize_stats_kernel, dim3(a.B * a.groups), dim3(256), 0, stream, a);
     SD_CHECK_HIP(hipGetLastError());
     return 0;
 }
diff --git a/sonicdiffusionbayeslab_amd/csrc/ops.hip b/sonicdiffusionbayeslab_amd/csrc/ops.hip
--- a/sonicdiffusionbayeslab_amd/csrc/ops.hip
+++ b/sonicdiffusionbayeslab_amd/csrc/ops.hip
@@ -644,6 +644,40 @@
     return sd_launch_gemm(a, epi, (hipStream_t)stream);
 }
 
+extern "C" int sd_op_groupnorm_stats(void* stream, const void* x, int C, const float* stats, const float* gamma, const float* beta,
+                                     void* y, int B, int HW, int groups, float eps, int silu) {
+    SD_REQUIRE(x && stats && y && B > 0 && HW > 0 && HW % 64 == 0 && groups > 0,
+               "sd_op_groupnorm_stats: %d pixels per sample, %d channels: producer statistics come in 64-pixel blocks", HW, C);
+    float* partial = (float*)op_scratch(sd_groupnorm_scratch_bytes(B, HW, groups));
+    SD_REQUIRE(partial, "sd_op_groupnorm_stats: cannot allocate scratch");
+    GroupNormArgs g = groupnorm_after_conv(x, C, gamma, beta, y, B, HW, groups, eps, silu, partial, stats);
+    g.no_small = 1;
+    return sd_launch_groupnorm(g, (hipStream_t)stream);
+}
+
+extern "C" int sd_op_tf_entry_applicable(int M, int hw, int C) { return sd_tf_entry_applicable(M, hw, C) ? 1 : 0; }
+extern "C" int sd_op_tf_entry(void* stream, const void* x, const float* stats, const float* gamma, const float* beta, int groups,
+                              float eps, const void* Wp, const float* bp, const void* Wqkv_ln, const float* c1, const float* c2,
+                              float ln_eps, void* h0, void* Q, void* KV, int M, int hw, int C, int hm_tokens, int max_workgroups) {
+    SD_REQUIRE(sd_tf_entry_applicable(M, hw, C), "sd_op_tf_entry: M=%d rows of %d per sample, C=%d is not a shape the chained kernel takes",
+               M, hw, C);
+    TfEntryArgs a;
+    a.X = (const bf16_t*)x; a.Wp = (const bf16_t*)Wp; a.bp = bp; a.Wqkv = (const bf16_t*)Wqkv_ln; a.c1 = c1; a.c2 = c2; a.ln_eps = ln_eps;
+    a.H0 = (bf16_t*)h0; a.Q = (bf16_t*)Q; a.KV = (bf16_t*)KV; a.M = M; a.hw = hw; a.C = C; a.hm_tok = hm_tokens;
+    a.max_workgroups = max_workgroups;
+    if (stats) {
+        const int B = M / hw;
+        SD_REQUIRE(gamma && beta && groups > 0 && groups <= 64 && C % groups == 0 && C / groups >= 8,
+                   "sd_op_tf_entry: GroupNorm of %d groups over %d channels (at least 8 channels per group)", groups, C);
+        float* partial = (float*)op_scratch(sd_groupnorm_scratch_bytes(B, hw, groups));
+        SD_REQUIRE(partial, "sd_op_tf_entry: cannot allocate scratch");
+        const GroupNormArgs g = groupnorm_after_conv(x, C, gamma, beta, nullptr, B, hw, groups, eps, 0, partial, stats);
+        if (int rc = sd_launch_groupnorm_finalize(g, (hipStream_t)stream)) return rc;
+        a.gn_mr = sd_groupnorm_mean_rstd(g); a.gamma = gamma; a.beta = beta; a.groups = groups;
+    }
+    return sd_launch_tf_entry(a, (hipStream_t)stream);
+}
+
 extern "C" int sd_op_xattn_fused_rowstats(void* stream, const void* X, const void* R, void* Y, const void* At, const void* Bw,
                                           const float* bias, int M, int C, int rows_per_sample, int L, float* rowstats) {
     SD_REQUIRE(sd_xattn_fused_applicable(rows_per_sample, C, 8, L), "sd_op_xattn_fused_rowstats: shape not supported");
diff --git a/sonicdiffusionbayeslab_amd/csrc/plan.hip b/sonicdiffusionbayeslab_amd/csrc/plan.hip
--- a/sonicdiffusionbayeslab_amd/csrc/plan.hip
+++ b/sonicdiffusionbayeslab_amd/csrc/plan.hip
@@ -178,6 +178,7 @@
         return o.out;
     }
     bool shortcut_fuse = !(getenv("SD_SHORTCUT_FUSE") && atoi(getenv("SD_SHORTCUT_FUSE")) == 0);
+    int tf_entry = !getenv("SD_TF_ENTRY") ? 2 : atoi(getenv("SD_TF_ENTRY")) == 0 ? 0 : atoi(getenv("SD_TF_ENTRY")) == 1 ? 1 : 2;
     int resnet(const std::string& p, int x1, int c1, int x2, int c2, int cout, int rh, int rw, int tproj_t) {
         const int hw = rh * rw, cin = c1 + c2, M = UB * hw;
         const bool fq = u->fp8;
@@ -252,13 +253,34 @@
         int M = UB * hw;
         const std::string t = p + "transformer_blocks.0.";
         const bool fq = u->fp8;
-        int g = gn(x, C, -1, 0, hw, p + "norm.weight", p + "norm.bias", 1e-6f, 0, fq);
-        int h0 = gemm(g, C, -1, 0, M, C, p + "proj_in.weight", p + "proj_in.bias", -1, 0, fq);
         const int tr = tome_r(rh, rw, C);
+        const int groups = u->cfg.norm_num_groups;
+        static const bool big_tiles = getenv("SD_GEMM_BIG") != nullptr;
+        const bool chain = tf_entry > 0 && C == 320 && !fq && u->unet_like() && tr == 0 && ln_fold && !big_tiles && sd_gemm_splitk(M, C, C) == 1 &&
+                           sd_tf_entry_applicable(M, hw, C) && u->woff.count(p + "proj_in.weight") && u->woff.count(p + "proj_in.bias") &&
+                           u->woff.count(t + "attn1.qkv.weight.ln") && u->woff.count(t + "attn1.qkv.weight.c1") &&
+                           u->woff.count(t + "attn1.qkv.weight.c2");
+        const bool chain_gn = chain && tf_entry > 1 && hw % 64 == 0 && !sd_groupnorm_uses_small(UB, hw, C, 0, groups) && stats_of.count(x) &&
+                              groups > 0 && groups <= 64 && C % groups == 0 && C / groups >= 8;
+        int g = chain_gn ? -1 : gn(x, C, -1, 0, hw, p + "norm.weight", p + "norm.bias", 1e-6f, 0, fq);
+        int h0 = chain ? -1 : gemm(g, C, -1, 0, M, C, p + "proj_in.weight", p + "proj_in.bias", -1, 0, fq);
         const int Nm = hw - tr, Mm = UB * Nm;
         int tome_i = -1;
         int qkv, rs = -1, np = 0;
-        if (tr > 0) {
+        if (chain) {
+            Op o; o.kind = OP_TF_ENTRY; o.x1 = chain_gn ? x : g; o.M = M; o.N = 3 * C; o.K1 = o.K = C; o.Kalg = C; o.rpb = hw; o.B = UB;
+            o.splitk = 1;
+            o.w = W(p + "proj_in.weight"); o.b = W(p + "proj_in.bias");
+            o.wqkv = W(t + "attn1.qkv.weight.ln"); o.c1 = W(t + "attn1.qkv.weight.c1"); o.c2q = W(t + "attn1.qkv.weight.c2");
+            if (chain_gn) {
+                o.s1 = stats_of[x]; o.g = W(p + "norm.weight"); o.be = W(p + "norm.bias"); o.eps = 1e-6f;
+                o.nsplit = sd_groupnorm_nsplit(UB, hw);
+                o.aux = tensor(sd_groupnorm_scratch_bytes(UB, hw, groups));
+            }
+            o.out2 = h0 = tensor((size_t)M * C * 2);
+            o.out = qkv = tensor((size_t)M * 3 * C * 2);
+            push(o);
+        } else if (tr > 0) {
             const int num_dst = hw / 4, num_src = hw - num_dst;
             Plan::TomeBlock tb;
             tb.B = UB; tb.h = rh; tb.w = rw; tb.r = tr; tb.choice_off = pl.tome_choice_bytes;
@@ -889,6 +911,7 @@
         std::vector<int> producer(pl.tensors.size(), -1);
         for (int i = 0; i < nops; ++i) {
             if (pl.ops[i].out >= 0) producer[pl.ops[i].out] = i;
+            if (pl.ops[i].out2 >= 0) producer[pl.ops[i].out2] = i;
             if (pl.ops[i].stats >= 0) producer[pl.ops[i].stats] = i;
             if (pl.ops[i].rs >= 0) producer[pl.ops[i].rs] = i;
         }
@@ -909,7 +932,7 @@
         int ins[32], nin;
         op_tensors(o, ins, nin);
         for (int k = 0; k < nin; ++k) pl.tensors[ins[k]].last = std::max(pl.tensors[ins[k]].last, i);
-        for (int t : {o.out, o.aux, o.stats, o.rs})
+        for (int t : {o.out, o.out2, o.aux, o.stats, o.rs})
             if (t >= 0) {
                 if (pl.tensors[t].def < 0) pl.tensors[t].def = i;
                 pl.tensors[t].last = std::max(pl.tensors[t].last, i);
diff --git a/sonicdiffusionbayeslab_amd/csrc/tf_entry.hip b/sonicdiffusionbayeslab_amd/csrc/tf_entry.hip
--- /dev/null
+++ b/sonicdiffusionbayeslab_amd/csrc/tf_entry.hip
@@ -0,0 +1,457 @@
+#include "common.h"
+#include "kernels.h"
+
+#include <stdlib.h>
+
+namespace {
+
+typedef __amdgpu_buffer_rsrc_t rsrc_t;
+
+struct TfArgs {
+    const void* X; const void* Wp; const void* Wq; void* H0; void* Q; void* KV;
+    const float* bp; const float* c1; const float* c2;
+    const float* gn_mr; const float* gamma; const float* beta;
+    unsigned x_bytes, wp_bytes, wq_bytes, h_bytes, q_bytes, kv_bytes;
+    int M, hw, items;
+    int ldqb;
+    float ln_eps, inv_c;
+    int hm_tpc, hm_tok, hm_heads, hm_samples;
+    int groups, cpg;
+};
+
+template <int N>
+__device__ __forceinline__ void wait_vmcnt() {
+    asm volatile("s_waitcnt vmcnt(%0)" ::"n"(N) : "memory");
+}
+__device__ __forceinline__ void wait_vm(int n) {
+    if (n == 3) { wait_vmcnt<3>(); return; }
+    if (n == 2) { wait_vmcnt<2>(); return; }
+    asm volatile("" : "+s"(n));
+    switch (n) {
+        case 0: wait_vmcnt<0>(); break;
+        case 1: wait_vmcnt<1>(); break;
+        case 2: wait_vmcnt<2>(); break;
+        case 3: wait_vmcnt<3>(); break;
+        case 4: wait_vmcnt<4>(); break;
+        case 5: wait_vmcnt<5>(); break;
+        case 6: wait_vmcnt<6>(); break;
+        case 7: wait_vmcnt<7>(); break;
+        case 8: wait_vmcnt<8>(); break;
+        case 9: wait_vmcnt<9>(); break;
+        case 10: wait_vmcnt<10>(); break;
+        case 11: wait_vmcnt<11>(); break;
+        default: wait_vmcnt<12>(); break;
+    }
+}
+__device__ __forceinline__ void lds_barrier() {
+    asm volatile("s_waitcnt lgkmcnt(0)" ::: "memory");
+    __builtin_amdgcn_s_barrier();
+    asm volatile("" ::: "memory");
+}
+
+__device__ __forceinline__ rsrc_t make_rsrc(const void* p, unsigned bytes) {
+    return __builtin_amdgcn_make_buffer_rsrc((void*)p, 0, (int)bytes, 0x00020000);
+}
+__device__ __forceinline__ void dma16(rsrc_t r, void* lds_wave_base, int voff, int soff) {
+    __builtin_amdgcn_raw_ptr_buffer_load_lds(r, LDS_PTR(lds_wave_base), 16, voff, soff, 0, 0);
+}
+
+template <int C>
+struct TfGeom {
+    static constexpr int BM = C == 320 ? 128 : 64;
+    static constexpr int KT = C / 64;
+    static constexpr int NPJ = C / 160, NQ = 3 * C / 160;
+    static constexpr int NP = 2 * NPJ;
+    static constexpr int XS_BYTES = KT * BM * 128;
+    static constexpr int WST = 160 * 128, NS = 3;
+    static constexpr int PART_BYTES = NP * BM * 8, VEC_BYTES = 2 * 160 * 4, GNT_BYTES = 2 * C * 4;
+    static constexpr int SMEM = XS_BYTES + NS * WST + PART_BYTES + VEC_BYTES + GNT_BYTES;
+    static_assert(SMEM <= 160 * 1024, "row block + W ring do not fit the 160 KiB LDS");
+};
+
+template <int C, bool GN>
+__global__ __launch_bounds__(512) void tf_entry_kernel(const TfArgs p) {
+    using G = TfGeom<C>;
+    constexpr int BM = G::BM, KT = G::KT, NPJ = G::NPJ, NQ = G::NQ, NP = G::NP, WST = G::WST;
+    constexpr int TM = BM / 64, TN = 5, WTM = 16 * TM, WTN = 80;
+    constexpr int XPW = BM / 64;
+    constexpr int LDB = C * 2;
+    constexpr int EPI_STORES = (TN / 2 + 1) * TM;
+
+    extern __shared__ __attribute__((aligned(16))) char smem[];
+    char* xs = smem;
+    char* ring = xs + G::XS_BYTES;
+    char* part = ring + G::NS * WST;
+    char* vecs = part + G::PART_BYTES;
+    char* gnt = vecs + G::VEC_BYTES;
+
+    const int tid = threadIdx.x, lane = tid & 63;
+    const int wave = __builtin_amdgcn_readfirstlane(tid >> 6);
+    const int wm = wave & 3, wn = wave >> 2;
+    const int lrow = lane & 15, lq = lane >> 4;
+
+    const int nblk = gridDim.x;
+    int work;
+    {
+        const int q = nblk >> 3, r = nblk & 7, xcd = blockIdx.x & 7, idx = blockIdx.x >> 3;
+        work = (xcd < r ? xcd * (q + 1) : r * (q + 1) + (xcd - r) * q) + idx;
+    }
+    const int nwork = p.items;
+    if (work >= nwork) return;
+
+    const rsrc_t rX = make_rsrc(p.X, p.x_bytes), rWp = make_rsrc(p.Wp, p.wp_bytes), rWq = make_rsrc(p.Wq, p.wq_bytes);
+    const rsrc_t rH = make_rsrc(p.H0, p.h_bytes), rQ = make_rsrc(p.Q, p.q_bytes), rKV = make_rsrc(p.KV, p.kv_bytes);
+
+    const int lrow8 = lane >> 3, gch = (lane & 7) ^ lrow8;
+    const int vD = lrow8 * LDB + gch * 16;
+    const int rowl = wm * WTM + lrow;
+    const int colw = wn * WTN + (lq & 1) * 16 + (lq >> 1) * 8;
+    const int coln = wn * WTN + (TN - 1) * 16 + lq * 4;
+    const int vHw = rowl * LDB + colw * 2, vHn = rowl * LDB + coln * 2;
+    const int vQw = rowl * p.ldqb + colw * 2, vQn = rowl * p.ldqb + coln * 2;
+    int vK[TN / 2 + 1];
+#pragma unroll
+    for (int j = 0; j <= TN / 2; ++j) {
+        const int cl = j < TN / 2 ? colw + j * 32 : coln;
+        const int hl = (cl * 205) >> 13;
+        vK[j] = (hl * p.hm_tok + rowl) * 80 + (cl - hl * 40) * 2;
+    }
+    const int swz[2] = {((lq) ^ (lane & 7)) << 4, ((4 + lq) ^ (lane & 7)) << 4};
+    const int xoff = rowl * 128;
+    const int woff = (wn * WTN + lrow) * 128;
+
+    int issued = 0;
+    int e_a = 0, e_b = 0;
+    int x_end = 0;
+
+    auto dma_x = [&](int m0, int kt) {
+#pragma unroll
+        for (int i = 0; i < XPW; ++i) {
+            const int pc = wave + i * 8;
+            dma16(rX, xs + kt * (BM * 128) + pc * 1024, vD, (m0 + pc * 8) * LDB + kt * 128);
+        }
+        issued += XPW;
+    };
+    int fp = 0, fk = 0, fwork = work;
+    auto dma_w_next = [&](int slot) {
+        if (fwork >= nwork) return;
+        char* dst = ring + slot * WST;
+        const int n0 = (fp < NPJ ? fp : fp - NPJ) * 160;
+#pragma unroll
+        for (int i = 0; i < 3; ++i) {
+            const int pc = wave + i * 8;
+            if (pc < 20) {
+                const int so = (n0 + pc * 8) * LDB + fk * 128;
+                if (fp < NPJ) dma16(rWp, dst + pc * 1024, vD, so);
+                else dma16(rWq, dst + pc * 1024, vD, so);
+                issued += 1;
+            }
+        }
+        if (++fk == KT) {
+            fk = 0;
+            if (++fp == NPJ + NQ) { fp = 0; fwork += nblk; }
+        }
+    };
+
+    f32x4 acc[TN][TM];
+    bf16x8 xf0[TM], wf0[TN], xf1[TM], wf1[TN];
+    auto load_frags = [&](const char* sx, const char* sw, int ks, bf16x8* xf, bf16x8* wf) {
+#pragma unroll
+        for (int t = 0; t < TM; ++t) xf[t] = *(const bf16x8*)(sx + xoff + t * 2048 + swz[ks]);
+#pragma unroll
+        for (int t = 0; t < TN; ++t) wf[t] = *(const bf16x8*)(sw + woff + t * 2048 + swz[ks]);
+    };
+    auto mfmas = [&](const bf16x8* xf, const bf16x8* wf) {
+#pragma unroll
+        for (int a = 0; a < TN; ++a)
+#pragma unroll
+            for (int b = 0; b < TM; ++b)
+                acc[a][b] = __builtin_amdgcn_mfma_f32_16x16x32_bf16(wf[a], xf[b], acc[a][b], 0, 0, 0);
+    };
+
+    constexpr int GNC = (C + 511) / 512;
+    float gn_g[GNC], gn_b[GNC];
+    int gn_grp[GNC];
+    if (GN) {
+#pragma unroll
+        for (int i = 0; i < GNC; ++i) {
+            const int c = tid + i * 512, cc = c < C ? c : C - 1;
+            gn_g[i] = p.gamma[cc]; gn_b[i] = p.beta[cc]; gn_grp[i] = cc / p.cpg;
+        }
+    }
+
+    int m0 = work * BM;
+#pragma unroll
+    for (int kt = 0; kt < KT; ++kt) dma_x(m0, kt);
+    x_end = issued;
+    dma_w_next(0); e_a = issued;
+    dma_w_next(1); e_b = issued;
+    int slot = 0;
+
+    auto k_loop = [&](int pass, bool stream_x, int m_next) {
+#pragma unroll
+        for (int a = 0; a < TN; ++a)
+#pragma unroll
+            for (int b = 0; b < TM; ++b) acc[a][b] = f32x4{0.f, 0.f, 0.f, 0.f};
+        for (int kt = 0; kt < KT; ++kt) {
+            wait_vm(issued - e_a);
+            __builtin_amdgcn_s_barrier();
+            asm volatile("" ::: "memory");
+            const char* sx = xs + kt * (BM * 128);
+            const char* sw = ring + slot * WST;
+            load_frags(sx, sw, 0, xf0, wf0);
+            __builtin_amdgcn_sched_barrier(0);
+            if (kt == 0) {
+                if (pass < NPJ) {
+                    if (wave == 0) {
+                        if (lane < 40) glds16((const char*)p.bp + pass * 640 + lane * 16, vecs);
+                        issued += 1;
+                    }
+                } else if (wave < 2) {
+                    const char* src = (const char*)(wave == 0 ? p.c1 : p.c2) + (pass - NPJ) * 640;
+                    if (lane < 40) glds16(src + lane * 16, vecs + wave * 640);
+                    issued += 1;
+                }
+            }
+            dma_w_next(slot >= 1 ? slot - 1 : 2);
+            e_a = e_b; e_b = issued;
+            if (stream_x && kt >= 1) dma_x(m_next, kt - 1);
+            __builtin_amdgcn_sched_barrier(0);
+            load_frags(sx, sw, 1, xf1, wf1);
+            mfmas(xf0, wf0);
+            mfmas(xf1, wf1);
+            slot = slot == 2 ? 0 : slot + 1;
+        }
+        __builtin_amdgcn_sched_barrier(0);
+    };
+    f32x4 v0[TN], v1[TN];
+    auto vec_load = [&](bool two) {
+#pragma unroll
+        for (int a = 0; a < TN; ++a) {
+            v0[a] = *(const f32x4*)(vecs + (wn * WTN + a * 16 + lq * 4) * 4);
+            if (two) v1[a] = *(const f32x4*)(vecs + 640 + (wn * WTN + a * 16 + lq * 4) * 4);
+        }
+    };
+    u32x4 ow[TM][TN / 2];
+    u32x2 on[TM];
+    auto pack_tiles = [&]() {
+#pragma unroll
+        for (int b = 0; b < TM; ++b) {
+#pragma unroll
+            for (int a = 0; a + 1 < TN; a += 2) {
+                const f32x4 vx = acc[a][b], vy = acc[a + 1][b];
+                const auto s0 = __builtin_amdgcn_permlane16_swap(pack2bf(vx[0], vx[1]), pack2bf(vy[0], vy[1]), false, false);
+                const auto s1 = __builtin_amdgcn_permlane16_swap(pack2bf(vx[2], vx[3]), pack2bf(vy[2], vy[3]), false, false);
+                ow[b][a / 2] = u32x4{s0[0], s1[0], s0[1], s1[1]};
+            }
+            const f32x4 v = acc[TN - 1][b];
+            on[b] = u32x2{pack2bf(v[0], v[1]), pack2bf(v[2], v[3])};
+        }
+    };
+
+    while (true) {
+        const bool more = work + nblk < nwork;
+        const int m_next = (work + nblk) * BM;
+
+        if (GN) {
+            const int smp = m0 / p.hw;
+            const float* mr = p.gn_mr + (long)smp * p.groups * 2;
+#pragma unroll
+            for (int i = 0; i < GNC; ++i) {
+                const int c = tid + i * 512;
+                const f32x2_t st = *(const f32x2_t*)(mr + gn_grp[i] * 2);
+                float sc, sf;
+                gn_scale_shift(st[0], st[1], gn_g[i], gn_b[i], sc, sf);
+                if (c < C) {
+                    *(float*)(gnt + c * 4) = sc;
+                    *(float*)(gnt + (C + c) * 4) = sf;
+                }
+            }
+        }
+        wait_vm(issued - x_end);
+        lds_barrier();
+        if (GN) {
+            const int gchunk = (tid & 7) ^ ((tid >> 3) & 7);
+#pragma unroll
+            for (int i = 0; i < KT * BM / 64; ++i) {
+                const int kt = i / (BM / 64);
+                const int c0 = kt * 64 + gchunk * 8;
+                char* at = xs + (i * 512 + tid) * 16;
+                const u32x4 v = *(const u32x4*)at;
+                const f32x4 sa = *(const f32x4*)(gnt + c0 * 4), sb = *(const f32x4*)(gnt + c0 * 4 + 16);
+                const f32x4 fa = *(const f32x4*)(gnt + (C + c0) * 4), fb = *(const f32x4*)(gnt + (C + c0) * 4 + 16);
+                float f[8] = {bflo(v[0]), bfhi(v[0]), bflo(v[1]), bfhi(v[1]), bflo(v[2]), bfhi(v[2]), bflo(v[3]), bfhi(v[3])};
+#pragma unroll
+                for (int j = 0; j < 8; ++j) f[j] = gn_affine(f[j], j < 4 ? sa[j & 3] : sb[j & 3], j < 4 ? fa[j & 3] : fb[j & 3]);
+                *(u32x4*)at = u32x4{pack2bf(f[0], f[1]), pack2bf(f[2], f[3]), pack2bf(f[4], f[5]), pack2bf(f[6], f[7])};
+            }
+            asm volatile("s_waitcnt lgkmcnt(0)" ::: "memory");
+        }
+
+        u32x4 hw_[NPJ][TM][TN / 2];
+        u32x2 hn_[NPJ][TM];
+#pragma unroll
+        for (int pj = 0; pj < NPJ; ++pj) {
+            k_loop(pj, false, 0);
+            vec_load(false);
+#pragma unroll
+            for (int a = 0; a < TN; ++a) {
+                const f32x4 bv = v0[a] + f32x4{0.f, 0.f, 0.f, 0.f};
+#pragma unroll
+                for (int b = 0; b < TM; ++b) acc[a][b] += bv;
+            }
+#pragma unroll
+            for (int b = 0; b < TM; ++b) {
+                float s = 0.f, q = 0.f;
+#pragma unroll
+                for (int a = 0; a < TN; ++a) {
+                    const unsigned p0 = pack2bf(acc[a][b][0], acc[a][b][1]), p1 = pack2bf(acc[a][b][2], acc[a][b][3]);
+                    const float v[4] = {bflo(p0), bfhi(p0), bflo(p1), bfhi(p1)};
+#pragma unroll
+                    for (int j = 0; j < 4; ++j) { s += v[j]; q = __builtin_fmaf(v[j], v[j], q); }
+                }
+                s += __shfl_xor(s, 16); q += __shfl_xor(q, 16);
+                s += __shfl_xor(s, 32); q += __shfl_xor(q, 32);
+                if (lq == 0) *(f32x2_t*)(part + ((pj * 2 + wn) * BM + rowl + b * 16) * 8) = f32x2_t{s, q};
+            }
+            pack_tiles();
+            const int soH = m0 * LDB + pj * 320;
+#pragma unroll
+            for (int b = 0; b < TM; ++b) {
+                const int so = soH + b * 16 * LDB;
+#pragma unroll
+                for (int j = 0; j < TN / 2; ++j) {
+                    __builtin_amdgcn_raw_buffer_store_b128(ow[b][j], rH, vHw + so + j * 64, 0, 0);
+                    hw_[pj][b][j] = ow[b][j];
+                }
+                __builtin_amdgcn_raw_buffer_store_b64(on[b], rH, vHn + so, 0, 0);
+                hn_[pj][b] = on[b];
+            }
+            issued += EPI_STORES;
+        }
+        lds_barrier();
+#pragma unroll
+        for (int pj = 0; pj < NPJ; ++pj)
+#pragma unroll
+            for (int b = 0; b < TM; ++b) {
+                const int r = rowl + b * 16;
+#pragma unroll
+                for (int j = 0; j < TN / 2; ++j) {
+                    const int col = pj * 160 + colw + j * 32;
+                    *(u32x4*)(xs + (col >> 6) * (BM * 128) + r * 128 + ((((col >> 3) & 7) ^ (lane & 7)) << 4)) = hw_[pj][b][j];
+                }
+                const int col = pj * 160 + coln;
+                *(u32x2*)(xs + (col >> 6) * (BM * 128) + r * 128 + ((((col >> 3) & 7) ^ (lane & 7)) << 4) + (col & 7) * 2) = hn_[pj][b];
+            }
+        lds_barrier();
+        f32x2_t mr[TM];
+#pragma unroll
+        for (int b = 0; b < TM; ++b) {
+            float s = 0.f, q = 0.f;
+#pragma unroll
+            for (int i = 0; i < NP; ++i) {
+                const f32x2_t e = *(const f32x2_t*)(part + (i * BM + rowl + b * 16) * 8);
+                s += e[0];
+                q += e[1];
+            }
+            mr[b] = ln_mean_rstd(s, q, p.inv_c, p.ln_eps);
+        }
+
+        for (int j = 0; j < NQ; ++j) {
+            k_loop(NPJ + j, more && j == NQ - 1, m_next);
+            vec_load(true);
+#pragma unroll
+            for (int a = 0; a < TN; ++a)
+#pragma unroll
+                for (int b = 0; b < TM; ++b) acc[a][b] = ln_fold(acc[a][b], v0[a], mr[b][0], mr[b][1], v1[a]);
+            pack_tiles();
+            if (p.hm_tpc > 0 && j >= p.hm_tpc) {
+                const int which = j >= 2 * p.hm_tpc ? 1 : 0;
+                const int head0 = (j - (which + 1) * p.hm_tpc) * 4;
+                const int smp = m0 / p.hm_tok, tok0 = m0 - smp * p.hm_tok;
+                const int soC = (((which * p.hm_samples + smp) * p.hm_heads + head0) * p.hm_tok + tok0) * 80;
+#pragma unroll
+                for (int b = 0; b < TM; ++b) {
+                    const int so = soC + b * 16 * 80;
+#pragma unroll
+                    for (int t = 0; t < TN / 2; ++t) __builtin_amdgcn_raw_buffer_store_b128(ow[b][t], rKV, vK[t] + so, 0, 0);
+                    __builtin_amdgcn_raw_buffer_store_b64(on[b], rKV, vK[TN / 2] + so, 0, 0);
+                }
+            } else {
+                const int soC = m0 * p.ldqb + j * 320;
+#pragma unroll
+                for (int b = 0; b < TM; ++b) {
+                    const int so = soC + b * 16 * p.ldqb;
+#pragma unroll
+                    for (int t = 0; t < TN / 2; ++t) __builtin_amdgcn_raw_buffer_store_b128(ow[b][t], rQ, vQw + so + t * 64, 0, 0);
+                    __builtin_amdgcn_raw_buffer_store_b64(on[b], rQ, vQn + so, 0, 0);
+                }
+            }
+            issued += EPI_STORES;
+        }
+        if (!more) break;
+        __builtin_amdgcn_s_barrier();
+        asm volatile("" ::: "memory");
+        dma_x(m_next, KT - 1);
+        x_end = issued;
+        work += nblk;
+        m0 = m_next;
+    }
+}
+
+template <int C>
+int launch_tf(const TfArgs& a, bool gn, int max_wg, hipStream_t stream) {
+    constexpr int smem = TfGeom<C>::SMEM;
+    static bool attr_set = false;
+    if (!attr_set) {
+        SD_CHECK_HIP(hipFuncSetAttribute((const void*)tf_entry_kernel<C, false>, hipFuncAttributeMaxDynamicSharedMemorySize, smem));
+        SD_CHECK_HIP(hipFuncSetAttribute((const void*)tf_entry_kernel<C, true>, hipFuncAttributeMaxDynamicSharedMemorySize, smem));
+        attr_set = true;
+    }
+    int grid = a.items < 256 ? a.items : 256;
+    if (max_wg > 0 && grid > max_wg) grid = max_wg;
+    if (gn) hipLaunchKernelGGL((tf_entry_kernel<C, true>), dim3(grid), dim3(512), smem, stream, a);
+    else hipLaunchKernelGGL((tf_entry_kernel<C, false>), dim3(grid), dim3(512), smem, stream, a);
+    SD_CHECK_HIP(hipGetLastError());
+    return 0;
+}
+
+}
+
+bool sd_tf_entry_applicable(int M, int hw, int C) {
+    if (C != 320 && C != 640) return false;
+    const int rows = C == 320 ? 128 : 64;
+    if (M <= 0 || hw <= 0 || hw % rows != 0 || M % hw != 0) return false;
+    return (long)M * 3 * C * 2 < (1L << 31);
+}
+
+int sd_launch_tf_entry(const TfEntryArgs& g, hipStream_t stream) {
+    SD_REQUIRE(sd_tf_entry_applicable(g.M, g.hw, g.C), "tf_entry: M=%d, %d rows per sample, C=%d is not a shape of the chained kernel",
+               g.M, g.hw, g.C);
+    SD_REQUIRE(g.X && g.Wp && g.bp && g.Wqkv && g.c1 && g.c2 && g.H0 && g.Q && g.max_workgroups >= 0, "tf_entry: null operand");
+    SD_REQUIRE(((((uintptr_t)g.X) | (uintptr_t)g.Wp | (uintptr_t)g.Wqkv | (uintptr_t)g.H0 | (uintptr_t)g.Q | (uintptr_t)g.KV |
+                 (uintptr_t)g.bp | (uintptr_t)g.c1 | (uintptr_t)g.c2) & 15) == 0, "tf_entry: operands must be 16-byte aligned");
+    const int rows = g.C == 320 ? 128 : 64;
+    TfArgs a{};
+    a.X = g.X; a.Wp = g.Wp; a.Wq = g.Wqkv; a.H0 = g.H0; a.Q = g.Q; a.KV = g.KV; a.bp = g.bp; a.c1 = g.c1; a.c2 = g.c2;
+    a.M = g.M; a.hw = g.hw; a.items = g.M / rows;
+    a.ln_eps = g.ln_eps; a.inv_c = 1.0f / (float)g.C;
+    const long mc = (long)g.M * g.C * 2;
+    a.x_bytes = (unsigned)mc; a.h_bytes = (unsigned)mc;
+    a.wp_bytes = (unsigned)((long)g.C * g.C * 2); a.wq_bytes = 3u * a.wp_bytes;
+    if (g.hm_tok > 0) {
+        SD_REQUIRE(g.KV && g.hm_tok % 128 == 0 && g.M % g.hm_tok == 0 && g.C % 160 == 0,
+                   "tf_entry: head-major K / V needs a KV buffer and tokens per sample (%d) a multiple of 128 dividing M", g.hm_tok);
+        a.ldqb = g.C * 2; a.q_bytes = (unsigned)mc; a.kv_bytes = (unsigned)(2 * mc);
+        a.hm_tpc = g.C / 160; a.hm_tok = g.hm_tok; a.hm_heads = g.C / 40; a.hm_samples = g.M / g.hm_tok;
+    } else {
+        a.ldqb = 3 * g.C * 2; a.q_bytes = (unsigned)(3 * mc); a.kv_bytes = 0;
+    }
+    if (g.gn_mr) {
+        SD_REQUIRE(g.gamma && g.beta && g.groups > 0 && g.C % g.groups == 0 && g.C / g.groups >= 8,
+                   "tf_entry: GroupNorm of %d groups over %d channels (at least 8 channels per group)", g.groups, g.C);
+        a.gn_mr = g.gn_mr; a.gamma = g.gamma; a.beta = g.beta; a.groups = g.groups; a.cpg = g.C / g.groups;
+    }
+    return g.C == 320 ? launch_tf<320>(a, g.gn_mr != nullptr, g.max_workgroups, stream)
+                      : launch_tf<640>(a, g.gn_mr != nullptr, g.max_workgroups, stream);
+}
diff --git a/sonicdiffusionbayeslab_amd/csrc/unet.hip b/sonicdiffusionbayeslab_amd/csrc/unet.hip
--- a/sonicdiffusionbayeslab_amd/csrc/unet.hip
+++ b/sonicdiffusionbayeslab_amd/csrc/unet.hip
@@ -121,6 +121,22 @@
             if (o.lnrs >= 0) { a.ln_rs = (const float*)T(o.lnrs); a.ln_np = o.lnnp; a.ln_c1 = (const float*)(wb + o.c1); a.ln_eps = 1e-5f; }
             if (o.lnrs >= 0 && o.s1 >= 0) { a.ln_c1 = (const float*)T(o.s1); a.bias = (const float*)T(o.s2); a.ln_per_sample = 1; }
             return sd_launch_gemm(a, o.epi, stream);
+        }
+        case OP_TF_ENTRY: {
+            TfEntryArgs a;
+            a.X = (const bf16_t*)T(o.x1); a.Wp = (const bf16_t*)(wb + o.w); a.bp = (const float*)(wb + o.b);
+            a.Wqkv = (const bf16_t*)(wb + o.wqkv); a.c1 = (const float*)(wb + o.c1); a.c2 = (const float*)(wb + o.c2q); a.ln_eps = 1e-5f;
+            a.H0 = (bf16_t*)T(o.out2); a.Q = (bf16_t*)T(o.out); a.M = o.M; a.hw = o.rpb; a.C = o.K;
+            if (o.hm) { a.hm_tok = o.HW; a.KV = (bf16_t*)T(o.out) + (long)o.M * o.K; }
+            if (o.s1 >= 0) {
+                GroupNormArgs g;
+                g.x1 = a.X; g.C1 = o.K; g.gamma = (const float*)(wb + o.g); g.beta = (const float*)(wb + o.be);
+                g.partial = (float*)T(o.aux); g.B = o.B; g.HW = o.rpb; g.groups = u->cfg.norm_num_groups; g.nsplit = o.nsplit; g.eps = o.eps;
+                g.stats1 = (const float*)T(o.s1);
+                if (int rc = sd_launch_groupnorm_finalize(g, stream)) return rc;
+                a.gn_mr = sd_groupnorm_mean_rstd(g); a.gamma = g.gamma; a.beta = g.beta; a.groups = g.groups;
+            }
+            return sd_launch_tf_entry(a, stream);
         }
         case OP_LN:
             if (o.out_fp8)
@@ -1507,6 +1523,10 @@
             *bytes = esz * ((double)o.M * K + (double)o.N * K) + (o.out_fp8 ? 1.0 : 2.0) * (double)o.M * (o.epi == 1 ? o.N / 2 : o.N);
             break;
         }
+        case OP_TF_ENTRY:
+            *flops = 2.0 * o.M * (double)(o.K + o.N) * o.K;
+            *bytes = 2.0 * ((double)o.M * (2.0 * o.K + o.N) + (double)(o.K + o.N) * o.K);
+            break;
         case OP_XATTN:
             *flops = 4.0 * o.M * (double)o.N * o.N + 4.0 * o.M * (double)o.sm_valid * o.N;
             *bytes = 3.0 * 2.0 * o.M * o.N;
@@ -1642,7 +1662,7 @@
             a.w_batch_stride = (long)o.N * 4 * o.Cin;
             halo4 = sd_conv_halo_subpix_applicable(a);
         }
-        const int kd = o.kind == OP_SAG_MASS ? 12 : o.kind == OP_PAG_IDENTITY ? 11 : o.kind == OP_HT_GATHER ? 9 : o.kind == OP_HT_SCATTER ? 10 : o.kind == OP_TGATE_CAPTURE ? 24 : o.kind == OP_TGATE_APPLY ? 25 : o.kind == OP_TGATE_ZERO ? 26 : o.kind == OP_XATTN ? 18 : o.kind == OP_REPLICATE ? 19 : o.kind == OP_IP_XATTN ? 22 : o.kind == OP_RES_ADD ? 23 : halo4 ? 21 :
+        const int kd = o.kind == OP_TF_ENTRY ? 13 : o.kind == OP_SAG_MASS ? 12 : o.kind == OP_PAG_IDENTITY ? 11 : o.kind == OP_HT_GATHER ? 9 : o.kind == OP_HT_SCATTER ? 10 : o.kind == OP_TGATE_CAPTURE ? 24 : o.kind == OP_TGATE_APPLY ? 25 : o.kind == OP_TGATE_ZERO ? 26 : o.kind == OP_XATTN ? 18 : o.kind == OP_REPLICATE ? 19 : o.kind == OP_IP_XATTN ? 22 : o.kind == OP_RES_ADD ? 23 : halo4 ? 21 :
                        (o.kind == OP_CONV3 && !o.dt && (o.subpix || o.stride != 1)) ? 20 :
                        (o.dt ? (o.kind == OP_CONV3 ? 16 : 17) : o.kind);
         kind_ms[kd] += ms; kind_launches[kd] += 1; kind_flops[kd] += fl; kind_bytes[kd] += by;
diff --git a/sonicdiffusionbayeslab_amd/unet.py b/sonicdiffusionbayeslab_amd/unet.py
--- a/sonicdiffusionbayeslab_amd/unet.py
+++ b/sonicdiffusionbayeslab_amd/unet.py
@@ -641,7 +641,7 @@
             _lib.check(self._lib.sd_unet_set_fp8_scale(self._handle, k.encode(), float(v)), f"sd_unet_set_fp8_scale({k})")
 
     KIND_NAMES = {0: "sinusoid", 1: "gemv", 2: "conv_in", 3: "groupnorm", 4: "conv3x3", 5: "gemm", 6: "layernorm",
-                  7: "attention", 8: "conv_out", 9: "hypertile_gather", 10: "hypertile_scatter", 11: "pag_identity", 12: "sag_mass", 16: "conv3x3_fp8", 17: "gemm_fp8", 18: "xattn_fused",
+                  7: "attention", 8: "conv_out", 9: "hypertile_gather", 10: "hypertile_scatter", 11: "pag_identity", 12: "sag_mass", 13: "tf_entry", 16: "conv3x3_fp8", 17: "gemm_fp8", 18: "xattn_fused",
                   19: "replicate", 20: "conv3x3_gemm", 21: "conv3x3_halo_subpix", 22: "ip_xattn", 23: "residual_add",
                   24: "tgate_capture", 25: "tgate_apply", 26: "tgate_zero",
                   27: "tome_match", 28: "tome_select", 29: "tome_merge", 30: "tome_unmerge", 31: "freeu"}
```

After: 11.52 images/s, median of 5. About the same (+0.3%).
